# therealadityashankar/hey-buddy

Measured on AMD Instinct MI355X. Metric: audio clips/sec featurized+trained, 1.5 s @16 kHz, 1/2/4/8 GPU, higher is better.
Workload: dtype f32

## Files before the change

### hey-buddy_amd/csrc/hbk_augment_plan.h

```cpp
#pragma once

#include <algorithm>
#include <cmath>
#include <cstdarg>
#include <cstdint>
#include <cstdio>
#include <numeric>
#include <string>
#include <vector>

namespace hbk {
namespace {

constexpr int kPlanOk = 0, kPlanErrArg = -1, kPlanErrUnsupported = -3;

inline std::string strf(const char* fmt, ...) {
  char buf[512];
  va_list ap;
  va_start(ap, fmt);
  vsnprintf(buf, sizeof(buf), fmt, ap);
  va_end(ap);
  return buf;
}

inline int arg_fail(std::string& err, const char* what) {
  err = strf("hbk: invalid argument: %s", what);
  return kPlanErrArg;
}

inline int64_t up256(int64_t b) { return (b + 255) & ~int64_t(255); }

constexpr int kT = 23040;
constexpr int kM = kT / 2;
constexpr int kThreads = 1024;
constexpr int kN1 = 16000;
constexpr int kM1 = kN1 / 2;

constexpr int kTwLo = 128, kTwHi = kM / kTwLo;
static_assert(kTwLo * kTwHi == kM, "twiddle split");
constexpr int kTw8Lo = 100, kTw8Hi = kM1 / kTw8Lo;
static_assert(kTw8Lo * kTw8Hi == kM1, "twiddle split");

constexpr int kHRow = kM / 16 + 1;
constexpr int kHSlots = 16 * kHRow;

constexpr int kBsHalf = kT / 2;
constexpr int kBsPart = kT - kBsHalf + 1;
constexpr int kBsCirc = 512;
static_assert(2 * kBsCirc <= kThreads, "one edge sample per thread");

constexpr size_t kAugLds = (size_t(2 * kM + 32) * sizeof(float)) + (kTwHi + kTwLo) * 8;
constexpr size_t kBandStopLds = kAugLds + (5 * kBsCirc + 1) * sizeof(float);
constexpr size_t kColoredLds = (size_t(2 * kM1 + 32) * sizeof(float)) + (kTw8Hi + kTw8Lo) * 8;

constexpr int kPsFft = 250, kPsHop = 7, kPsBins = kPsFft / 2 + 1, kPsPad = kPsFft / 2;
constexpr int kPsTapMax = 144;
constexpr int kPsPhaseMax = 128;
constexpr int kPsResFrames = 32;
#ifndef HBK_PV_CLIPS
#define HBK_PV_CLIPS 2
#endif
constexpr int kPvClips = HBK_PV_CLIPS;
constexpr int kPvGroup = 8;
constexpr int kPvRows = 64;
constexpr int kPvGh = 64;
constexpr int kRsFrames = 64, kRsK = 160, kRsLd = kRsK + 8;
static_assert(kPsTapMax <= kRsK && kPsPhaseMax <= 128, "the MFMA resampler's K padding and 8 phase tiles");

struct PitchGeometry {
  int L = 0, f_in = 0, f_out = 0, l1 = 0, orig = 0, nw = 0, width = 0, target = 0;
  double rate = 0;
};

inline int pitch_geometry(int64_t L, int32_t sample_rate, int32_t num, int32_t den, PitchGeometry& a,
                          std::string& err) {
  if (sample_rate != 16000) {
    err = strf("hbk: pitch shift supports 16 kHz (n_fft 250, hop 7), got %d", sample_rate);
    return kPlanErrUnsupported;
  }
  if (num <= 0 || den <= 0) return arg_fail(err, "shift num / den must be positive");
  if (L <= kPsPad || L > (int64_t(1) << 24)) return arg_fail(err, "clip length must be in (125, 2^24]");
  a.L = static_cast<int>(L);
  a.rate = double(den) / double(num);
  a.f_in = 1 + a.L / kPsHop;
  a.f_out = static_cast<int>(std::ceil(double(a.f_in) / a.rate));
  a.l1 = kPsHop * (a.f_out - 1);
  const int64_t new_sr = int64_t(sample_rate) * den / num;
  const int64_t g = std::gcd(int64_t(sample_rate), new_sr);
  if (new_sr <= 0 || g <= 0) return arg_fail(err, "shift out of range");
  a.orig = static_cast<int>(sample_rate / g);
  a.nw = static_cast<int>(new_sr / g);
  a.width = static_cast<int>(std::ceil(6.0 * a.orig / (std::min(a.orig, a.nw) * 0.99)));
  a.target = static_cast<int>(std::ceil(double(a.nw) * a.l1 / a.orig));
  if (a.nw > kPsPhaseMax || 2 * a.width + a.orig > kPsTapMax || a.l1 <= 0 ||
      a.rate * kPvGroup + 3 > kPvRows) {
    err = strf("hbk: pitch shift %d/%d resamples %d -> %d (%d taps): the kernel holds <= %d phases of <= %d taps "
               "(torch_pitch_shift's fast shifts at 16 kHz)", num, den, a.orig, a.nw, 2 * a.width + a.orig,
               kPsPhaseMax, kPsTapMax);
    return kPlanErrUnsupported;
  }
  return kPlanOk;
}

struct PitchLayout {
  int64_t y = 0;
  int64_t taps = 0;
  int64_t yr = 0;
  int64_t sp = 0;
  int64_t key = 0;
  int64_t ord = 0;
  int64_t gord = 0;
  int64_t total = 0;
};

inline PitchLayout pitch_layout(const PitchGeometry& a, int64_t n) {
  PitchLayout w;
  w.y = 0;
  w.taps = up256(n * a.l1 * 4);
  w.yr = w.taps + up256(int64_t(kPsPhaseMax) * kPsTapMax * 4);
  w.sp = w.yr + up256(n * 8);
  w.key = w.sp + up256(n * 8);
  w.ord = w.key + up256(n * 8);
  w.gord = w.ord + up256(n * 4);
  w.total = w.gord + up256(n * 4);
  return w;
}

struct PitchKnobs {
  bool span = true;
  bool pair = true;
  bool resample_valu = false;
};

struct Grid {
  unsigned x = 1, y = 1, block = 0;
};

struct PitchLaunches {
  bool pair = false;
  int groups = 0;
  Grid taps, span, rank_clips, group, rank_groups, vocoder, resample;
  bool resample_mfma = true;
};

inline PitchLaunches pitch_launches(const PitchGeometry& a, int64_t n, const PitchKnobs& k) {
  PitchLaunches p;
  p.pair = k.span && k.pair;
  p.groups = static_cast<int>((n + kPvClips - 1) / kPvClips);
  p.taps = Grid{unsigned((a.nw * kPsTapMax + 255) / 256), 1, 256};
  p.span = Grid{unsigned((n + 3) / 4), 1, 256};
  p.rank_clips = Grid{unsigned((n + 63) / 64), 1, 1024};
  p.group = Grid{unsigned((p.groups + 255) / 256), 1, 256};
  p.rank_groups = Grid{unsigned((p.groups + 63) / 64), 1, 1024};
  p.vocoder = Grid{unsigned(p.groups), 1, unsigned(128 * kPvClips)};
  const int res_frames = (a.L + a.nw - 1) / a.nw;
  p.resample_mfma = !(k.resample_valu || a.nw > 128);
  p.resample = p.resample_mfma ? Grid{unsigned((res_frames + kRsFrames - 1) / kRsFrames), unsigned(n), 256}
                               : Grid{unsigned((res_frames + kPsResFrames - 1) / kPsResFrames), unsigned(n), 128};
  return p;
}

struct BandStopLayout {
  int64_t sums = 0;
  int64_t taps = 0;
  int64_t spectra = 0;
  int64_t scratch = 0;
  int64_t total = 0;
};

inline BandStopLayout band_stop_layout(int64_t n, int32_t n_filters, int32_t n_spectra, int64_t blocks) {
  BandStopLayout w;
  if (n <= 0) return w;
  w.taps = w.sums + up256(int64_t(n_filters) * 8);
  w.spectra = w.taps + up256(int64_t(n_filters) * (kBsCirc + 1) * 4);
  w.scratch = w.spectra + int64_t(n_spectra) * kHSlots * 8;
  w.total = w.scratch + blocks * kT * 4;
  return w;
}

struct ColoredLayout {
  int64_t groups = 0;
  int64_t gbuf = 0;
  int64_t grms = 0;
  int64_t total = 0;
};

inline ColoredLayout colored_layout(int64_t n_clips, int64_t clips_per_noise) {
  ColoredLayout w;
  w.groups = clips_per_noise > 1 && n_clips > 0 ? (n_clips + clips_per_noise - 1) / clips_per_noise : 0;
  if (!w.groups) return w;
  w.grms = w.groups * kN1 * int64_t(sizeof(float));
  w.total = w.grms + up256(w.groups * int64_t(sizeof(float)));
  return w;
}

enum ReverbTable { kTabHi, kTabLo, kTabN, kTabHi8, kTabLo8, kTabN16, kTabCount };

struct ReverbTables {
  std::vector<float> host;
  size_t off[kTabCount] = {};
  size_t pairs[kTabCount] = {};
  size_t bytes() const { return host.size() * sizeof(float); }
};

inline void twiddle_table(float* dst, int count, int step, int N, bool slotted) {
  for (int i = 0; i < count; ++i) {
    const double a = -2.0 * M_PI * (double(i) * step) / double(N);
    float* p = dst + 2 * size_t(slotted ? (i % 16) * kHRow + i / 16 : i);
    p[0] = float(cos(a));
    p[1] = float(sin(a));
  }
}

inline ReverbTables reverb_tables() {
  struct Spec {
    int count, step, N, pairs;
    bool slotted;
  };
  const Spec spec[kTabCount] = {
      {kTwHi, kTwLo, kM, kTwHi, false},        {kTwLo, 1, kM, kTwLo, false},      {kM + 1, 1, kT, kHSlots, true},
      {kTw8Hi, kTw8Lo, kM1, kTw8Hi, false},    {kTw8Lo, 1, kM1, kTw8Lo, false},   {kM1 / 2 + 1, 1, kN1, kM1 / 2 + 1, false},
  };
  ReverbTables t;
  size_t bytes = 0;
  for (int i = 0; i < kTabCount; ++i) {
    t.off[i] = bytes;
    t.pairs[i] = size_t(spec[i].pairs);
    bytes += size_t(up256(int64_t(spec[i].pairs) * 8));
  }
  t.host.assign(bytes / sizeof(float), 0.f);
  for (int i = 0; i < kTabCount; ++i)
    twiddle_table(t.host.data() + t.off[i] / sizeof(float), spec[i].count, spec[i].step, spec[i].N, spec[i].slotted);
  return t;
}

}
}
```

### hey-buddy_amd/csrc/hbk_clip_ops.hip

```cpp
#include <algorithm>

#include "hbk_aug_dev.h"

namespace hbk {
namespace {

struct TanhArgs {
  const float* x;
  int64_t x_stride;
  float* out;
  int64_t out_stride;
  int64_t n_clips;
  const float* amount;
  const int32_t* idx;
  int64_t n_entries;
  SrcView view;
};

__device__ __forceinline__ unsigned abs_bits(float v, int s) {
  return s < kT ? (__builtin_bit_cast(unsigned, v) & 0x7FFFFFFFu) : 0xFFFFFFFFu;
}

__global__ void __launch_bounds__(kThreads) __attribute__((amdgpu_waves_per_eu(8)))
tanh_distortion_kernel(TanhArgs a) {
  __shared__ unsigned hist[4096];
  __shared__ float red[32];
  __shared__ unsigned pick[2];
  constexpr int kPer = (kT + kThreads - 1) / kThreads;
  const int64_t n_iter = a.idx ? a.n_entries : a.n_clips;
  for (int64_t e = blockIdx.x; e < n_iter; e += gridDim.x) {
    const int64_t clip = a.idx ? a.idx[e] : e;
    const int tid = opaque_tid();
    const float* x = a.x + clip * a.x_stride;
    float* out = a.out + clip * a.out_stride;
    const float amt = a.amount[clip];
    if (amt != amt) {
      if (out != x) copy_clip(x, out, tid);
      continue;
    }
    float xr[kPer];
    const int pre = a.view.pre ? a.view.pre[clip] : -1, len = a.view.pre ? a.view.len[clip] : 0;
    if (pre >= 0) {
      const int n = min(len, kT);
      const float* row = n > 0 ? a.view.src + clip * a.view.stride : x;
      const int t = opaque_tid();
      const int w0 = __builtin_amdgcn_readfirstlane(t & ~63);
#pragma unroll
      for (int u = 0; u < kPer; ++u) xr[u] = load_placed_wave(row, pre, n, w0 + u * kThreads, t & 63);
    } else {
    const int t = opaque_tid();
#pragma unroll
    for (int u = 0; u < kPer; ++u) {
      const int s = t + u * kThreads;
      xr[u] = s < kT ? *reinterpret_cast<const float*>(reinterpret_cast<const char*>(x) + (static_cast<uint32_t>(s) << 2))
                     : 0.f;
    }
    }
    const double pos = (100.0 - 99.0 * static_cast<double>(amt)) / 100.0 * (kT - 1);
    const int lo = min(max(static_cast<int>(floor(pos)), 0), kT - 1);
    const double frac = pos - lo;
    unsigned prefix = 0, mask = 0, rank = static_cast<unsigned>(lo);
#pragma unroll 1
    for (int p = 0; p < 3; ++p) {
      const int shift = p == 0 ? 19 : (p == 1 ? 9 : 0), bins = p == 0 ? 4096 : (p == 1 ? 1024 : 512);
      const int per_lane = bins >> 6;
      for (int i = tid; i < bins; i += kThreads) hist[i] = 0;
      __syncthreads();
      const int t = opaque_tid();
#pragma unroll
      for (int u = 0; u < kPer; ++u) {
        const unsigned b = abs_bits(xr[u], t + u * kThreads);
        if ((b & mask) == prefix && b != 0xFFFFFFFFu) atomicAdd(&hist[(b >> shift) & (bins - 1)], 1u);
      }
      __syncthreads();
      if (tid < 64) {
        unsigned own = 0;
        for (int i = 0; i < per_lane; ++i) own += hist[per_lane * tid + i];
        unsigned inc = own;
#pragma unroll
        for (int d = 1; d < 64; d <<= 1) {
          const unsigned v = __shfl_up(inc, d, 64);
          if (tid >= d) inc += v;
        }
        const unsigned long long hit = __ballot(inc > rank);
        const int l = __ffsll(static_cast<long long>(hit)) - 1;
        if (tid == l) {
          unsigned r = rank - (inc - own), dsel = per_lane * l;
          for (int i = 0; i < per_lane - 1; ++i) {
            const unsigned h = hist[dsel];
            if (r < h) break;
            r -= h;
            ++dsel;
          }
          pick[0] = dsel;
          pick[1] = r;
        }
      }
      __syncthreads();
      prefix |= pick[0] << shift;
      mask |= static_cast<unsigned>(bins - 1) << shift;
      rank = pick[1];
    }
    float cnt = 0.f, mg = __builtin_inff();
    const int t2 = opaque_tid();
#pragma unroll
    for (int u = 0; u < kPer; ++u) {
      const unsigned b = abs_bits(xr[u], t2 + u * kThreads);
      if (b == 0xFFFFFFFFu) continue;
      if (b <= prefix) cnt += 1.f;
      else mg = fminf(mg, __builtin_bit_cast(float, b));
    }
    cnt = block_sum(cnt, red);
    {
      for (int d = 32; d >= 1; d >>= 1) mg = fminf(mg, __shfl_xor(mg, d, 64));
      __syncthreads();
      if ((tid & 63) == 0) red[tid >> 6] = mg;
      __syncthreads();
      mg = red[0];
      for (int w = 1; w < kThreads / 64; ++w) mg = fminf(mg, red[w]);
    }
    const double v_lo = __builtin_bit_cast(float, prefix);
    const double v_hi = (cnt >= lo + 2 || lo + 1 >= kT) ? v_lo : static_cast<double>(mg);
    const double d = v_hi - v_lo;
    const double th = frac >= 0.5 ? v_hi - d * (1.0 - frac) : v_lo + d * frac;
    const float g = static_cast<float>(0.5 / (th + 1e-6));
    float ex = 0.f, ey = 0.f;
#pragma unroll
    for (int u = 0; u < kPer; ++u) {
      ex += xr[u] * xr[u];
      xr[u] = 1.f - __fdividef(2.f, __expf(2.f * g * xr[u]) + 1.f);
      ey += xr[u] * xr[u];
    }
    block_sum2(ex, ey, red);
    const float rms_x = sqrtf(ex / kT);
    const float post = rms_x > 1e-9f ? rms_x / sqrtf(ey / kT) : 1.f;
    const int t3 = opaque_tid();
#pragma unroll
    for (int u = 0; u < kPer; ++u) {
      const int s = t3 + u * kThreads;
      if (s < kT) *reinterpret_cast<float*>(reinterpret_cast<char*>(out) + (static_cast<uint32_t>(s) << 2)) = xr[u] * post;
    }
    __syncthreads();
  }
}

constexpr int kPlaceSpan = 4096;
__global__ void __launch_bounds__(256) place_kernel(const float* __restrict__ src, int64_t src_stride,
                                                    const int32_t* __restrict__ src_len,
                                                    const int32_t* __restrict__ pre,
                                                    const int32_t* __restrict__ idx, float* __restrict__ out,
                                                    int64_t out_stride, int64_t n_clips, int T) {
  const int spans = (T + kPlaceSpan - 1) / kPlaceSpan;
  const int64_t items = n_clips * spans;
  constexpr int kR = kPlaceSpan / 1024;
  for (int64_t it = blockIdx.x; it < items; it += gridDim.x) {
    const int64_t e = it / spans;
    const int sp = static_cast<int>(it - e * spans);
    const int64_t clip = idx ? idx[e] : e;
    const int p = pre[clip];
    const int n = min(src_len[clip], T);
    const int last = max(n - 1, 0);
    const float* s = src + clip * src_stride;
    float* o = out + clip * out_stride;
    const int t0 = sp * kPlaceSpan + 4 * static_cast<int>(threadIdx.x);
    float v[kR][4];
#pragma unroll
    for (int r = 0; r < kR; ++r)
#pragma unroll
      for (int q = 0; q < 4; ++q) {
        const int u = t0 + r * 1024 + q - p;
        const float x = n > 0 ? s[min(max(u, 0), last)] : 0.f;
        v[r][q] = (u >= 0 && u < n) ? x : 0.f;
      }
#pragma unroll
    for (int r = 0; r < kR; ++r) {
      const int t = t0 + r * 1024;
      if (t < T) *reinterpret_cast<float4*>(o + t) = make_float4(v[r][0], v[r][1], v[r][2], v[r][3]);
    }
  }
}

constexpr int kEqTile = 64;
struct EqArgs {
  const float* x;
  int64_t x_stride;
  const double* coef;
  const int32_t* idx;
  float* out;
  int64_t out_stride;
  int64_t n;
  SrcView view;
};

constexpr int kEqClips = 8;
__global__ void __launch_bounds__(64) eq_kernel(EqArgs a) {
  constexpr int kRow = kEqTile + 4;
  __shared__ __attribute__((aligned(16))) float tin[kEqClips][kRow];
  __shared__ __attribute__((aligned(16))) float tout[kEqClips][kRow];
  const int lane = threadIdx.x, c = lane >> 3, sec = lane & 7;
  const int64_t j0 = static_cast<int64_t>(blockIdx.x) * kEqClips;
  const int64_t jc = min(j0 + c, a.n - 1);
  const double* cf0 = a.coef + jc * 35;
  const bool copy = cf0[0] != cf0[0];
  const int k = min(sec, 6);
  double b0 = cf0[5 * k], b1 = cf0[5 * k + 1], b2 = cf0[5 * k + 2], a1 = cf0[5 * k + 3], a2 = cf0[5 * k + 4];
  if (copy) b0 = 1.0, b1 = b2 = a1 = a2 = 0.0;
  double s1 = 0.0, s2 = 0.0;
  const int lc = lane >> 3, lq = lane & 7;
  const int64_t jl = min(j0 + lc, a.n - 1);
  const int64_t clip_l = a.idx ? static_cast<int64_t>(a.idx[jl]) : jl;
  const float* xl = a.x + clip_l * a.x_stride;
  float* ol = a.out + clip_l * a.out_stride;
  const bool store_l = j0 + lc < a.n;
  const int pre_l = a.view.pre ? a.view.pre[clip_l] : -1, len_l = a.view.pre ? a.view.len[clip_l] : 0;
  const int n_l = pre_l >= 0 ? min(len_l, kT) : 0;
  const float* sl = n_l > 0 ? a.view.src + clip_l * a.view.stride : xl;
  float4 p0, p1;
  auto load_tile = [&](int t) {
    const int u0 = t + 4 * lq - pre_l;
    if (pre_l >= 0 && u0 >= 0 && u0 + 35 < n_l) {
      const float* q = sl + u0;
      p0 = float4{q[0], q[1], q[2], q[3]};
      p1 = float4{q[32], q[33], q[34], q[35]};
    } else if (pre_l >= 0 && (u0 + 35 < 0 || u0 >= n_l)) {
      p0 = p1 = float4{0.f, 0.f, 0.f, 0.f};
    } else if (pre_l >= 0) {
      const int ta = t + 4 * lq, tb = ta + 32;
      p0 = float4{load_placed(sl, pre_l, n_l, ta), load_placed(sl, pre_l, n_l, ta + 1),
                  load_placed(sl, pre_l, n_l, ta + 2), load_placed(sl, pre_l, n_l, ta + 3)};
      p1 = float4{load_placed(sl, pre_l, n_l, tb), load_placed(sl, pre_l, n_l, tb + 1),
                  load_placed(sl, pre_l, n_l, tb + 2), load_placed(sl, pre_l, n_l, tb + 3)};
    } else {
      p0 = *reinterpret_cast<const float4*>(xl + t + 4 * lq);
      p1 = *reinterpret_cast<const float4*>(xl + t + 32 + 4 * lq);
    }
  };
  load_tile(0);
  float prev = 0.f;
  for (int t0 = 0; t0 <= kT; t0 += kEqTile) {
    tin[lc][4 * lq] = p0.x;
    tin[lc][4 * lq + 1] = p0.y;
    tin[lc][4 * lq + 2] = p0.z;
    tin[lc][4 * lq + 3] = p0.w;
    tin[lc][32 + 4 * lq] = p1.x;
    tin[lc][32 + 4 * lq + 1] = p1.y;
    tin[lc][32 + 4 * lq + 2] = p1.z;
    tin[lc][32 + 4 * lq + 3] = p1.w;
    __syncthreads();
    const int tn = min(t0 + kEqTile, kT - kEqTile);
    load_tile(tn);
    for (int st0 = 0; st0 < kEqTile; st0 += 8) {
      const float4 ia = *reinterpret_cast<const float4*>(&tin[c][st0]);
      const float4 ib = *reinterpret_cast<const float4*>(&tin[c][st0 + 4]);
      const float in8[8] = {ia.x, ia.y, ia.z, ia.w, ib.x, ib.y, ib.z, ib.w};
      float o8[8];
#pragma unroll
      for (int q = 0; q < 8; ++q) {
        const float u = sec == 0 ? in8[q] : prev;
        const double vd = u;
        const double y = fma(b0, vd, s1);
        s1 = fma(b1, vd, fma(-a1, y, s2));
        s2 = fma(b2, vd, -a2 * y);
        const float v = static_cast<float>(y);
        o8[q] = v;
        prev = __builtin_bit_cast(float, __builtin_amdgcn_update_dpp(__builtin_bit_cast(int, prev),
                                                                     __builtin_bit_cast(int, v), 0x111, 0xF, 0xF,
                                                                     false));
      }
      if (sec == 6) {
        *reinterpret_cast<float4*>(&tout[c][st0]) = float4{o8[0], o8[1], o8[2], o8[3]};
        *reinterpret_cast<float4*>(&tout[c][st0 + 4]) = float4{o8[4], o8[5], o8[6], o8[7]};
      }
    }
    __syncthreads();
    if (store_l) {
#pragma unroll
      for (int m = 0; m < 8; ++m) {
        const int kk = lq + 8 * m;
        const int n = t0 - 6 + kk;
        if (n >= 0 && n < kT) ol[n] = tout[lc][kk];
      }
    }
    __syncthreads();
  }
}

}
}

extern "C" {

int hbk_place_clips_idx(const float* src, int64_t n_clips, int64_t src_stride, const int32_t* src_len,
                        const int32_t* pre, const int32_t* idx, int64_t n_entries, float* out, int64_t out_stride,
                        int64_t T, void* stream) {
  using namespace hbk;
  if (n_clips < 0 || (idx && n_entries < 0)) return arg_error("negative count");
  const int64_t n_rows = idx ? n_entries : n_clips;
  if (n_rows == 0) return HBK_OK;
  if (!src || !src_len || !pre || !out) return arg_error("NULL pointer");
  if (T <= 0 || T % 4 || T > (int64_t(1) << 30)) return arg_error("T must be a positive multiple of 4");
  if (out_stride < T || out_stride % 4 || (reinterpret_cast<uintptr_t>(out) & 15))
    return arg_error("out rows must be 16-B aligned with stride >= T");
  const int64_t items = n_rows * ((T + kPlaceSpan - 1) / kPlaceSpan);
  if (items >= (int64_t(1) << 31)) return arg_error("too many clips for one launch");
  const int64_t blocks = items;
  hipLaunchKernelGGL(place_kernel, dim3(unsigned(blocks)), dim3(256), 0, as_stream(stream), src, src_stride, src_len,
                     pre, idx, out, out_stride, n_rows, int(T));
  HBK_LAUNCH_CHECK("place_kernel");
  return HBK_OK;
}

int hbk_place_clips(const float* src, int64_t n_clips, int64_t src_stride, const int32_t* src_len,
                    const int32_t* pre, float* out, int64_t out_stride, int64_t T, void* stream) {
  return hbk_place_clips_idx(src, n_clips, src_stride, src_len, pre, nullptr, 0, out, out_stride, T, stream);
}

int hbk_tanh_distortion_src(const float* x, int64_t n_clips, int64_t x_stride, const float* amount,
                            const int32_t* idx, int64_t n_entries, float* out, int64_t out_stride,
                            const float* src, int64_t src_stride, const int32_t* src_len, const int32_t* src_pre,
                            void* stream) {
  using namespace hbk;
  if (n_clips < 0) return arg_error("negative n_clips");
  if (n_clips == 0) return HBK_OK;
  if (!x || !out || !amount) return arg_error("NULL pointer");
  if (x_stride < kT || out_stride < kT) return arg_error("stride < 23040");
  TanhArgs a;
  a.x = x;
  a.x_stride = x_stride;
  a.out = out;
  a.out_stride = out_stride;
  a.n_clips = n_clips;
  a.amount = amount;
  a.idx = idx;
  a.n_entries = idx ? n_entries : n_clips;
  const int st = src_view(src, src_stride, src_len, src_pre, a.view);
  if (st != HBK_OK) return st;
  if (a.n_entries <= 0) return n_entries < 0 ? arg_error("negative n_entries") : HBK_OK;
  const int64_t blocks = std::min<int64_t>(a.n_entries, persistent_blocks(2, stream));
  hipLaunchKernelGGL(tanh_distortion_kernel, dim3(unsigned(blocks)), dim3(kThreads), 0, as_stream(stream), a);
  HBK_LAUNCH_CHECK("tanh_distortion_kernel");
  return HBK_OK;
}

int hbk_tanh_distortion(const float* x, int64_t n_clips, int64_t x_stride, const float* amount,
                        const int32_t* idx, int64_t n_entries, float* out, int64_t out_stride, void* stream) {
  return hbk_tanh_distortion_src(x, n_clips, x_stride, amount, idx, n_entries, out, out_stride, nullptr, 0, nullptr,
                                 nullptr, stream);
}

int hbk_seven_band_eq_src(const float* x, int64_t n_clips, int64_t x_stride, const double* coef, const int32_t* idx,
                          int64_t n_entries, float* out, int64_t out_stride, const float* src, int64_t src_stride,
                          const int32_t* src_len, const int32_t* src_pre, void* stream) {
  using namespace hbk;
  if (n_clips < 0 || n_entries < 0) return arg_error("negative count");
  if (!idx) n_entries = n_clips;
  if (n_entries == 0) return HBK_OK;
  if (!x || !out || !coef) return arg_error("NULL pointer");
  if (x_stride < kT || out_stride < kT) return arg_error("stride < 23040");
  if ((reinterpret_cast<uintptr_t>(x) | reinterpret_cast<uintptr_t>(out)) % 16 || x_stride % 4 || out_stride % 4)
    return arg_error("x / out rows must be 16-B aligned");
  EqArgs a;
  a.x = x;
  a.x_stride = x_stride;
  a.coef = coef;
  a.idx = idx;
  a.out = out;
  a.out_stride = out_stride;
  a.n = n_entries;
  const int st = src_view(src, src_stride, src_len, src_pre, a.view);
  if (st != HBK_OK) return st;
  hipLaunchKernelGGL(eq_kernel, dim3(unsigned((n_entries + kEqClips - 1) / kEqClips)), dim3(64), 0,
                     as_stream(stream), a);
  HBK_LAUNCH_CHECK("eq_kernel");
  return HBK_OK;
}

int hbk_seven_band_eq(const float* x, int64_t n_clips, int64_t x_stride, const double* coef, const int32_t* idx,
                      int64_t n_entries, float* out, int64_t out_stride, void* stream) {
  return hbk_seven_band_eq_src(x, n_clips, x_stride, coef, idx, n_entries, out, out_stride, nullptr, 0, nullptr,
                               nullptr, stream);
}

}
```

### hey-buddy_amd/csrc/hbk_mlp_fused.hip

```cpp
#include <hip/hip_runtime.h>

#include <algorithm>
#include <initializer_list>
#include <utility>
#include <cmath>
#include <cstdio>

#include "hbk_common.h"
#include "hbk_mlp_dev.h"
#include "hbk_mlp_gate.h"
#include "hbk_mlp_internal.h"
#include "hbk_mlp_plan.h"

namespace hbk {
namespace {

constexpr int kStats = 8;

#ifdef HBK_TRACE
constexpr int kTraceKerns = 6, kTraceWaves = 4;
static_assert(kTraceWaves * 64 >= 256, "every traced kernel runs <= 256 threads (4 waves)");
__device__ unsigned long long g_mlp_trace[kTraceKerns][kTraceWaves][128];
__device__ int g_mlp_trace_n[kTraceKerns][kTraceWaves];
#define HBK_MTB(kern, id, blk)                                                                       \
  do {                                                                                         \
    static_assert((kern) >= 0 && (kern) < kTraceKerns, "trace kernel slot out of range");     \
    if (blockIdx.x == (blk) && (threadIdx.x & 63) == 0 && (threadIdx.x >> 6) < kTraceWaves) {   \
      const int w_ = threadIdx.x >> 6;                                                          \
      const int n_ = g_mlp_trace_n[kern][w_];                                                   \
      if (n_ < 128) {                                                                           \
        g_mlp_trace[kern][w_][n_] = (static_cast<unsigned long long>(id) << 56) |               \
                                    (__builtin_amdgcn_s_memtime() & 0xFFFFFFFFFFFFFFull);       \
        g_mlp_trace_n[kern][w_] = n_ + 1;                                                       \
      }                                                                                         \
    }                                                                                           \
  } while (0)
#define HBK_MT(kern, id) HBK_MTB(kern, id, 0)
__device__ unsigned long long g_span[1024][3];
#define HBK_SPAN(slot, v)                                                               \
  do {                                                                                  \
    if (threadIdx.x == 0 && blockIdx.x < 1024) g_span[blockIdx.x][slot] = (v);           \
  } while (0)
#else
#define HBK_SPAN(slot, v) \
  do {                    \
  } while (0)
#define HBK_MT(kern, id) \
  do {                   \
  } while (0)
#define HBK_MTB(kern, id, blk) \
  do {                         \
  } while (0)
#endif

#ifdef HBK_BOUNDS
constexpr int kBMax = 16;
__device__ unsigned long long g_brange[kBMax][2];
__device__ int g_bn;
__device__ unsigned long long g_berr[4];
__device__ __attribute__((aligned(16))) char g_bsafe[1 << 16];
template <typename T>
__device__ __forceinline__ T* bck_(T* p, int nbytes, int line) {
  const unsigned long long c = reinterpret_cast<unsigned long long>(p);
  bool ok = false;
  for (int i = 0; i < kBMax; ++i) ok |= i < g_bn && c >= g_brange[i][0] && c + nbytes <= g_brange[i][1];
  if (ok) return p;
  if (atomicCAS(&g_berr[0], 0ull, static_cast<unsigned long long>(line)) == 0ull) {
    g_berr[1] = blockIdx.x;
    g_berr[2] = threadIdx.x;
    g_berr[3] = c;
  }
  return reinterpret_cast<T*>(g_bsafe);
}
#define BCK(p, n) bck_((p), (n), __LINE__)
#else
#define BCK(p, n) (p)
#endif

__device__ __forceinline__ int step_of(const float* state, int parity) {
  return state ? static_cast<int>(state[parity * 8 + 3]) : 0;
}

struct GateWords {
  const float* st;
  const float* stats;
};
struct GateSeen {
  float acc_samples, n_sel;
};
__device__ __forceinline__ GateSeen gate_load(const GateWords& g) {
  GateSeen s{0.f, kGateSamples};
  if (g.st) {
    s.acc_samples = *BCK(&g.st[0], 4);
    s.n_sel = *BCK(&g.stats[0], 4);
  }
  return s;
}
__device__ __forceinline__ bool gate_drops(const GateSeen& s) {
  return step_gate(s.acc_samples, 1.f, 0.f, s.n_sel).fire == 0.f;
}

struct K1aArgs {
  const float* pool32;
  const _Float16* pool16;
  int64_t n32, n16;
  const int32_t* idx;
  int64_t idx_stride;
  int64_t idx_steps;
  const float* state;
  int parity;
  int B;
  float drop_p;
  uint64_t seed;
  float* xhat[2];
  int64_t Bp;
  uint4* rinfo[2];
  uint32_t* mask[2];
};

struct K1bArgs {
  const float* P;
  int64_t g_in, b_in, w0;
  int B;
  const float* xhat;
  int64_t Bp;
  float* hg_part;
  float* stats;
};

constexpr int kSlabLd = 516;
template <bool kIdx, bool kV2 = false>
__device__ __forceinline__ void k1a_tile(const K1aArgs& a, int rt, int step, float* __restrict__ xout,
                                         float* slab, int dpar = 0) {
  const int tid = threadIdx.x, lane = tid & 63, wave = tid >> 6;
  const uint64_t seed = a.seed + static_cast<uint64_t>(step) +
                        (a.state ? static_cast<uint64_t>(a.state[a.parity * 8 + 4]) << 24 : 0);
  const uint32_t s0 = static_cast<uint32_t>(seed), s1 = static_cast<uint32_t>(seed >> 32) * 0x27D4EB2Fu;
  const char* fallback = a.pool32 ? reinterpret_cast<const char*>(a.pool32) : reinterpret_cast<const char*>(a.pool16);
  int ixs[4];
#pragma unroll
  for (int i = 0; i < 4; ++i) {
    ixs[i] = min(rt * kR + wave * 4 + i, a.B - 1);
    if (kIdx) ixs[i] = *BCK(&a.idx[static_cast<int64_t>(step) * a.idx_stride + ixs[i]], 4);
  }
  uint4 raw[4][6];
  bool is16[4], ok[4];
  const char* rowptr[4];
#pragma unroll
  for (int i = 0; i < 4; ++i) {
    const int r = rt * kR + wave * 4 + i;
    const int ix = __builtin_amdgcn_readfirstlane(ixs[i]);
    is16[i] = ix < 0;
    const int64_t row16 = -static_cast<int64_t>(ix) - 1;
    ok[i] = r < a.B && (is16[i] ? row16 < a.n16 : ix < a.n32);
    const char* bp = !ok[i] ? fallback
                     : is16[i] ? reinterpret_cast<const char*>(a.pool16 + row16 * kD)
                               : reinterpret_cast<const char*>(a.pool32 + static_cast<int64_t>(ix) * kD);
    rowptr[i] = bp;
#pragma unroll
    for (int u = 0; u < 6; ++u) {
      const int slot = is16[i] ? u % 3 : u;
      raw[i][u] = *BCK(reinterpret_cast<const uint4*>(bp + 16 * (lane + 64 * slot)), 16);
    }
  }
  const float keep = a.drop_p > 0.f ? 1.f / (1.f - a.drop_p) : 1.f;
  const uint32_t thr = static_cast<uint32_t>(a.drop_p * 65536.f + 0.5f);
  float xh[4][kV2 ? 1 : 24];
  unsigned char* mimg = reinterpret_cast<unsigned char*>(slab) + (wave * 4) * kD;
#pragma unroll
  for (int i = 0; i < 4; ++i) {
    const int r = rt * kR + wave * 4 + i;
    float v[24];
    int c[24];
    bool dr[24];
#pragma unroll
    for (int j = 0; j < 24; ++j) {
      const uint4 w16 = raw[i][j >> 3];
      const uint32_t word16 = (&w16.x)[(j & 7) >> 1];
      const _Float16 h = __builtin_bit_cast(_Float16, static_cast<uint16_t>((j & 1) ? word16 >> 16 : word16));
      const uint4 w32 = raw[i][j >> 2];
      const float f = __builtin_bit_cast(float, (&w32.x)[j & 3]);
      v[j] = ok[i] ? (is16[i] ? static_cast<float>(h) : f) : 0.f;
      c[j] = is16[i] ? 8 * (lane + 64 * (j >> 3)) + (j & 7) : 4 * (lane + 64 * (j >> 2)) + (j & 3);
      dr[j] = !ok[i];
    }
    if (a.drop_p > 0.f) {
      const uint32_t base = static_cast<uint32_t>(r) * (kD / 2);
#pragma unroll
      for (int j = 0; j < 24; j += 2) {
        const uint32_t hsh = drop_hash(s0, s1, base + (c[j] >> 1));
        const bool d0 = (hsh & 0xFFFFu) < thr, d1 = (hsh >> 16) < thr;
        v[j] = d0 ? 0.f : v[j] * keep;
        v[j + 1] = d1 ? 0.f : v[j + 1] * keep;
        dr[j] = dr[j] || d0;
        dr[j + 1] = dr[j + 1] || d1;
      }
    }
    float sm = 0.f;
#pragma unroll
    for (int j = 0; j < 24; ++j) sm += v[j];
    const float mu = wsum(sm) * (1.f / kD);
    float sq = 0.f;
#pragma unroll
    for (int j = 0; j < 24; ++j) sq += (v[j] - mu) * (v[j] - mu);
// ... 287 lines not shown
    acc[t] = f4{0.f, 0.f, 0.f, 0.f};
    if (t < RT) {
#pragma unroll
      for (int i = 0; i < kNI; ++i) {
        const h8 ah = *reinterpret_cast<const h8*>(&ahS[(16 * t + m) * kLdA + 32 * i + 8 * kq]);
        const h8 al = *reinterpret_cast<const h8*>(&alS[(16 * t + m) * kLdA + 32 * i + 8 * kq]);
        acc[t] = mma3(ah, al, whi[i], wlo[i], acc[t]);
      }
    }
  }
  float* out = a.hg_part + static_cast<int64_t>(ks) * a.B * kH2 + 16 * wave + m;
#pragma unroll
  for (int t = 0; t < kRTM; ++t)
    if (t < RT) {
#pragma unroll
      for (int e = 0; e < 4; ++e) {
        const int r = r0 + 16 * t + 4 * kq + e;
        if (r < a.B) *BCK(&out[static_cast<int64_t>(r) * kH2], 4) = acc[t][e] * (1.f / 16.f);
      }
    }
  HBK_MT(3, 3);
}

__device__ __forceinline__ void wsplit_store4(const WSplit& w, _Float16* __restrict__ base, int64_t i4, f4 p) {
#pragma unroll
  for (int sg = 0; sg < kMaxSeg; ++sg) {
    if (sg >= w.n) break;
    const WSeg g = w.s[sg];
    const int64_t rc = int64_t(g.rows) * g.cols, off = i4 - g.src;
    if (off < 0 || off >= rc) continue;
    uint32_t h[2], l[2];
    split_pair(16.f * p[0], 16.f * p[1], h[0], l[0]);
    split_pair(16.f * p[2], 16.f * p[3], h[1], l[1]);
    _Float16* d = base + g.dst;
    *reinterpret_cast<uint2*>(d + off) = uint2{h[0], h[1]};
    *reinterpret_cast<uint2*>(d + rc + off) = uint2{l[0], l[1]};
    const int r = static_cast<int>(off / g.cols), c = static_cast<int>(off - int64_t(r) * g.cols);
#pragma unroll
    for (int e = 0; e < 4; ++e) {
      const uint32_t he = (e & 1) ? h[e >> 1] >> 16 : h[e >> 1] & 0xFFFFu;
      const uint32_t le = (e & 1) ? l[e >> 1] >> 16 : l[e >> 1] & 0xFFFFu;
      d[2 * rc + int64_t(c + e) * g.rows + r] = __builtin_bit_cast(_Float16, static_cast<uint16_t>(he));
      d[3 * rc + int64_t(c + e) * g.rows + r] = __builtin_bit_cast(_Float16, static_cast<uint16_t>(le));
    }
  }
}
__global__ void __launch_bounds__(256) k0_wsplit_kernel(WSplit w, const float* __restrict__ P,
                                                         _Float16* __restrict__ base, int64_t n4) {
  for (int64_t q = blockIdx.x * int64_t(256) + threadIdx.x; q < n4; q += int64_t(gridDim.x) * 256) {
    int sg = 0;
#pragma unroll
    for (int t = 1; t < kMaxSeg; ++t)
      if (t < w.n && q >= w.s[t].q0) sg = t;
    const int64_t i4 = w.s[sg].src + 4 * (q - w.s[sg].q0);
    wsplit_store4(w, base, i4, *reinterpret_cast<const f4*>(P + i4));
  }
}

struct K2Args {
  const float* P;
  int B, NG, KS;
  int64_t w_hg[kMaxG], b_hg[kMaxG], w_o[kMaxG], b_o[kMaxG];
  int64_t ln_g[kMaxG], ln_b[kMaxG];
  const float* hg_part;
  const float* y;
  int64_t y_stride;
  const float* state;
  int parity;
  const float* sched;
  int sched_len;
  float neg_weight, thr, act_thr;
  float* prob;
  float* logit;
  float* G;
  float* stats;
  int64_t Bp;
  float* U;
  float* Xn;
  float* dS;
  float* dHG;
  int n_rt, prefetch;
  K1aArgs pre;
  const _Float16* wc;
  int64_t c_o[kMaxG], c_hg[kMaxG], c_oT[kMaxG], c_hgT[kMaxG];
  float* counts;
  int count_label;
  int v2;
  float* maxS;
  int pre_tiles;
};

#ifdef HBK_TRACE
#define K2_MARK(id)                                                                \
  do {                                                                             \
    if (blockIdx.x == 0 && lane == 0 && wave < kTraceWaves && trn < 48)            \
      trS[wave][trn++] = (static_cast<unsigned long long>(id) << 56) |             \
                         (__builtin_amdgcn_s_memtime() & 0xFFFFFFFFFFFFFFull);     \
  } while (0)
#else
#define K2_MARK(id) \
  do {              \
  } while (0)
#endif

#ifndef HBK_K2_ABLATE
#define HBK_K2_ABLATE 0
#endif
template <bool kTrain, int NG>
__global__ void __launch_bounds__(64 * kK2Waves) k2_rows_kernel(K2Args a) {
  constexpr int kHgF = NG * kR * kLd > kR * kSlabLd ? NG * kR * kLd : kR * kSlabLd;
  __shared__ __attribute__((aligned(16))) float hgRaw[kHgF];
  float (*hgS)[kR][kLd] = reinterpret_cast<float (*)[kR][kLd]>(hgRaw);
  __shared__ __attribute__((aligned(16))) float xhS[NG - 1][kR][kL + 4];
  __shared__ __attribute__((aligned(16))) float bX[kR][kLd];
  __shared__ __attribute__((aligned(16))) float bU[kR][kLd];
  __shared__ __attribute__((aligned(16))) float bS[kR][kLd];
  __shared__ float rsS[NG][kR];
  __shared__ float zS[kR], dzS[kR];
  __shared__ float red[kStats];
  __shared__ float sBhg[NG][kH2], sWo[kH];
#ifdef HBK_TRACE
  __shared__ unsigned long long trS[4][48];
  int trn = 0;
#endif
  if (kTrain && static_cast<int>(blockIdx.x) >= a.n_rt) {
    const int step = step_of(a.pre.state, a.pre.parity) + 1;
    if (step < a.pre.idx_steps) {
      if (a.v2) {
        for (int t = 0; t < a.pre_tiles; ++t) {
          const int rt = (blockIdx.x - a.n_rt) * a.pre_tiles + t;
          if (rt >= a.n_rt) break;
          if (t) __syncthreads();
          k1a_tile<true, true>(a.pre, rt, step, nullptr, hgRaw, a.pre.parity ^ 1);
        }
      } else {
        for (int t = 0; t < kPreTiles; ++t) {
          const int rt = (blockIdx.x - a.n_rt) * kPreTiles + t;
          if (rt >= a.n_rt) break;
          if (t) __syncthreads();
          k1a_tile<true>(a.pre, rt, step, a.pre.xhat[a.pre.parity ^ 1], hgRaw);
        }
      }
    }
    return;
  }
  const int tid = threadIdx.x, lane = tid & 63, wave = tid >> 6;
  const int m = lane & 15, kq = lane >> 4;
  const int r0 = blockIdx.x * kR;
  const int nrow = min(kR, a.B - r0);
  const float* P = a.P;
  const int64_t B = a.B;
  const int64_t Bp = a.Bp;
  K2_MARK(1);
  const int step = step_of(a.state, a.parity);
  float y_pre = 0.f, nw_pre = a.neg_weight;
  if (kTrain) {
    y_pre = *BCK(&a.y[static_cast<int64_t>(step) * a.y_stride + min(r0 + (tid & 15), a.B - 1)], 4);
    if (a.sched) nw_pre = *BCK(&a.sched[2 * min(step, a.sched_len - 1) + 1], 4);
  }
  WFrag<kH, 2> wa;
  WFrag<kL, 2> wb;
  load_wf<kH, kL, 2>(wa, a.wc + a.c_o[0], wave, lane);
  const int lc0 = 6 * (lane & 15);
  float bo0[NG], bo1[NG], lg[NG][6], lb[NG][6];
  {
    const int c2 = tid & (kH2 - 1);
    float vbhg[NG];
#pragma unroll
    for (int k = 0; k < NG; ++k) {
      vbhg[k] = P[a.b_hg[k] + c2];
      bo0[k] = P[a.b_o[k] + (k + 1 < NG ? 16 * wave + m : 0)];
      bo1[k] = P[a.b_o[k] + (k + 1 < NG ? min(16 * (wave + 4) + m, kL - 1) : 0)];
#pragma unroll
      for (int e = 0; e < 6; ++e) {
        lg[k][e] = k + 1 < NG ? P[a.ln_g[k] + lc0 + e] : 0.f;
        lb[k][e] = k + 1 < NG ? P[a.ln_b[k] + lc0 + e] : 0.f;
      }
    }
    const float vwo = P[a.w_o[NG - 1] + (tid & (kH - 1))];
#pragma unroll
    for (int k = 0; k < NG; ++k)
      if (tid < kH2) sBhg[k][tid] = vbhg[k];
    if (tid < kH) sWo[tid] = vwo;
  }
  {
    float h[4] = {0.f, 0.f, 0.f, 0.f}, g[4] = {0.f, 0.f, 0.f, 0.f};
    auto sum_slabs = [&](auto U_) {
      constexpr int U = decltype(U_)::value;
      for (int s0 = 0; s0 < a.KS; s0 += U) {
        float lh[U][4], lg[U][4];
#pragma unroll
        for (int u = 0; u < U; ++u) {
          const int sl = (HBK_K2_ABLATE & 2) ? 0 : min(s0 + u, a.KS - 1);
#pragma unroll
          for (int q = 0; q < 4; ++q) {
            const int e = tid + 256 * q, r = min(e >> 6, nrow - 1), j = e & 63;
            const float* src = a.hg_part + (sl * B + r0 + r) * kH2;
            lh[u][q] = *BCK(&src[j], 4);
            lg[u][q] = *BCK(&src[kH + j], 4);
          }
        }
#pragma unroll
        for (int u = 0; u < U; ++u) {
          const float on = s0 + u < a.KS ? 1.f : 0.f;
#pragma unroll
          for (int q = 0; q < 4; ++q) {
            h[q] += on * lh[u][q];
            g[q] += on * lg[u][q];
          }
        }
      }
    };
    if (a.KS % 12 == 0)
      sum_slabs(std::integral_constant<int, 12>{});
    else
      sum_slabs(std::integral_constant<int, 8>{});
    const float bh = P[a.b_hg[0] + (tid & 63)], bg = P[a.b_hg[0] + kH + (tid & 63)];
#pragma unroll
    for (int q = 0; q < 4; ++q) {
      const int e = tid + 256 * q, r = e >> 6, j = e & 63;
      const float hh = h[q] + bh, gg = g[q] + bg;
      hgS[0][r][j] = hh;
      hgS[0][r][kH + j] = gg;
      bU[r][j] = hh * sigm_fast(hh) * gg;
    }
  }
  __syncthreads();
  K2_MARK(2);
  auto st4 = [&](float* base, int col, int row4, f4 v) {
#pragma unroll
    for (int e = 0; e < 4; ++e)
      if (r0 + row4 + e >= a.B) v[e] = 0.f;
    *BCK(reinterpret_cast<f4*>(base + col * Bp + r0 + row4), 16) = v;
  };
  auto amax4 = [&](f4 v, int row4) {
    float x = 0.f;
#pragma unroll
    for (int e = 0; e < 4; ++e) x = fmaxf(x, r0 + row4 + e < a.B ? fabsf(v[e]) : 0.f);
    return x;
  };
  auto store_t = [&](float* base, const float* src, int ncols) {
    float mx = 0.f;
    for (int e = tid; e < 4 * ncols; e += 256) {
      const int col = e >> 2, r4 = 4 * (e & 3);
      const f4 v = f4{src[r4 * kLd + col], src[(r4 + 1) * kLd + col], src[(r4 + 2) * kLd + col],
                      src[(r4 + 3) * kLd + col]};
      mx = fmaxf(mx, amax4(v, r4));
      st4(base, col, r4, v);
    }
    return mx;
  };
  auto pub_max = [&](int mat, float mx) {
    if (a.maxS) {
      mx = wmax(mx);
      if (lane == 0) *BCK(&a.maxS[(static_cast<int64_t>(mat) * a.n_rt + blockIdx.x) * kK2Waves + wave], 4) = mx;
    }
  };
  if (kTrain) {
    const int j = tid & 63, rg = 4 * (tid >> 6);
    st4(a.U, j, rg, f4{bU[rg][j], bU[rg + 1][j], bU[rg + 2][j], bU[rg + 3][j]});
  }
#pragma unroll
  for (int k = 0; k + 1 < NG; ++k) {
    if (!(HBK_K2_ABLATE & 1) || k == 0) load_wf<kL, kH2, 2>(wb, a.wc + a.c_hg[k + 1], wave, lane);
    {
      f4 c0, c1;
      gemm2<kH>(wa, load_a<kH>(&bU[0][0], lane), c0, c1);
      const int n0 = 16 * wave + m, n1 = 16 * (wave + 4) + m;
      const float bo0_ = bo0[k], bo1_ = bo1[k];
#pragma unroll
      for (int e = 0; e < 4; ++e) bS[4 * kq + e][n0] = c0[e] + bo0_;
      if (n1 < kL) {
#pragma unroll
        for (int e = 0; e < 4; ++e) bS[4 * kq + e][n1] = c1[e] + bo1_;
      }
    }
    __syncthreads();
    K2_MARK(10 + k);
    if (!(HBK_K2_ABLATE & 1) && k + 2 < NG) load_wf<kH, kL, 2>(wa, a.wc + a.c_o[k + 1], wave, lane);
    {
      const int r = wave * 4 + (lane >> 4), c0 = 6 * (lane & 15);
      float v[6];
#pragma unroll
      for (int e = 0; e < 6; ++e) v[e] = bS[r][c0 + e];
      const float mu = rsum16(((v[0] + v[1]) + (v[2] + v[3])) + (v[4] + v[5])) * (1.f / kL);
      float sq = 0.f;
#pragma unroll
      for (int e = 0; e < 6; ++e) sq += (v[e] - mu) * (v[e] - mu);
      const float rs = __builtin_amdgcn_rsqf(rsum16(sq) * (1.f / kL) + kLnEps);
#pragma unroll
      for (int e = 0; e < 6; ++e) {
        const float x = (v[e] - mu) * rs;
        xhS[k][r][c0 + e] = x;
        bX[r][c0 + e] = x * lg[k][e] + lb[k][e];
      }
      if ((lane & 15) == 0) rsS[k][r] = rs;
    }
    __syncthreads();
    K2_MARK(20 + k);
    if (kTrain) store_t(a.Xn + (k + 1) * kL * Bp, &bX[0][0], kL);
    {
      f4 ch, cg;
      gemm2<kL>(wb, load_a<kL>(&bX[0][0], lane), ch, cg);
      const int j = 16 * wave + m;
      const float bh = sBhg[k + 1][j], bg = sBhg[k + 1][kH + j];
      f4 uo;
#pragma unroll
      for (int e = 0; e < 4; ++e) {
        const int r = 4 * kq + e;
        const float h = ch[e] + bh, g = cg[e] + bg;
        hgS[k + 1][r][j] = h;
        hgS[k + 1][r][kH + j] = g;
        const float u = h * sigm_fast(h) * g;
        bU[r][j] = u;
        uo[e] = u;
      }
      if (kTrain) st4(a.U + (k + 1) * kH * Bp, j, 4 * kq, uo);
    }
    __syncthreads();
    K2_MARK(30 + k);
  }
  WFrag<kH2, 2> fx;
  WFrag<kL, 1> fy;
  if (kTrain) {
    load_wf<kH2, kL, 2>(fx, a.wc + a.c_hgT[NG - 1], wave, lane);
    load_wf<kL, kH, 1>(fy, a.wc + a.c_oT[NG - 2], wave, lane);
  }
  {
    const float bo = bo0[NG - 1];
    const float wl = sWo[lane];
#pragma unroll
    for (int i = 0; i < 4; ++i) {
      const int r = wave * 4 + i;
      const float z = wsum(bU[r][lane] * wl) + bo;
      if (lane == 0) zS[r] = z;
    }
  }
  __syncthreads();
  K2_MARK(40);
  if (tid < kR) {
    const int r = tid;
    float loc[kStats] = {0.f, 0.f, 0.f, 0.f, 0.f, 0.f, 0.f, 0.f};
    float dz = 0.f;
    if (r < nrow) {
      const float z = zS[r], p = sigm(z);
      if (a.prob) *BCK(&a.prob[r0 + r], 4) = p;
      if (a.logit) *BCK(&a.logit[r0 + r], 4) = z;
      if (kTrain) {
        const float nw = nw_pre;
        const float yy = y_pre;
        const bool pos = yy == 1.f;
        const bool sel = pos ? (p < 1.f - a.thr) : (p >= a.thr);
        if (sel) {
          const float w = pos ? 1.f : nw;
          const float lp = fmaxf(logf(p), -100.f), l1p = fmaxf(logf(1.f - p), -100.f);
          loc[0] = 1.f;
          loc[1] = -w * (yy * lp + (1.f - yy) * l1p);
          dz = w * (p - yy) / fmaxf((1.f - p) * p, 1e-12f) * ((1.f - p) * p);
          if (pos) {
            loc[4] = 1.f;
            loc[5] = p > a.act_thr ? 1.f : 0.f;
          } else {
            loc[2] = 1.f;
            loc[3] = (yy - p <= -a.act_thr) ? 1.f : 0.f;
          }
        }
        loc[6] = 1.f;
      }
    }
    dzS[r] = dz;
    if (!kTrain && a.counts) {
      float pge = 0.f, pgt = 0.f;
      if (r < nrow) {
        const float p = sigm(zS[r]);
        pge = p >= a.act_thr ? 1.f : 0.f;
        pgt = p > a.act_thr ? 1.f : 0.f;
      }
      pge = rsum16(pge);
      pgt = rsum16(pgt);
      if (tid == 0) {
        if (pge != 0.f) atomicAdd(BCK(a.counts + 2 * a.count_label, 4), pge);
        if (pgt != 0.f) atomicAdd(BCK(a.counts + 2 * a.count_label + 1, 4), pgt);
      }
    }
    if (kTrain) {
#pragma unroll
      for (int s = 0; s < kStats; ++s) {
        const float v = rsum16(loc[s]);
        if (tid == 0) red[s] = v;
      }
    }
  }
  if constexpr (!kTrain) return;
  __syncthreads();
  K2_MARK(41);
  if (tid < kStats && red[tid] != 0.f) atomicAdd(BCK(a.stats + tid, 4), red[tid]);
  if (!HBK_K2_ABLATE && red[0] == 0.f) {
    const f4 z4 = {0.f, 0.f, 0.f, 0.f};
#pragma unroll
    for (int k = 0; k < NG; ++k) {
      for (int e = tid; e < 4 * kH2; e += 256) st4(a.dHG + k * kH2 * Bp, e >> 2, 4 * (e & 3), z4);
      if (k + 1 < NG) {
        for (int e = tid; e < 4 * kL; e += 256) st4(a.dS + k * kL * Bp, e >> 2, 4 * (e & 3), z4);
      } else if (tid < 4) {
        st4(a.dS + k * kL * Bp, 0, 4 * tid, z4);
      }
    }
    if (a.maxS && lane == 0) {
#pragma unroll
      for (int mat = 0; mat < 2 * NG; ++mat)
        *BCK(&a.maxS[(static_cast<int64_t>(mat) * a.n_rt + blockIdx.x) * kK2Waves + wave], 4) = 0.f;
    }
    return;
  }
  float* G = a.G;
  {
    const f4 dz4 = f4{dzS[4 * (tid & 3)], dzS[4 * (tid & 3) + 1], dzS[4 * (tid & 3) + 2], dzS[4 * (tid & 3) + 3]};
    if (tid < 4) st4(a.dS + (NG - 1) * kL * Bp, 0, 4 * tid, dz4);
    pub_max(2 * NG - 1, tid < 4 ? amax4(dz4, 4 * tid) : 0.f);
  }
  if (tid == 64) {
    float s = 0.f;
    for (int r = 0; r < kR; ++r) s += dzS[r];
    if (s != 0.f) atomicAdd(BCK(G + a.b_o[NG - 1], 4), s);
  }
  {
    const int k = NG - 1;
    const int j = tid & 63, rg = 4 * (tid >> 6);
    const float wj = sWo[j];
    f4 dho, dgo;
#pragma unroll
    for (int e = 0; e < 4; ++e) {
      const int r = rg + e;
      const float h = hgS[k][r][j], gg = hgS[k][r][kH + j], du = dzS[r] * wj;
      const float sg = sigm_fast(h);
      const float dh = du * gg * (sg * (1.f + h * (1.f - sg))), dg = du * h * sg;
      bX[r][j] = dh;
      bX[r][kH + j] = dg;
      dho[e] = dh;
      dgo[e] = dg;
    }
    st4(a.dHG + k * kH2 * Bp, j, rg, dho);
    st4(a.dHG + k * kH2 * Bp, kH + j, rg, dgo);
    pub_max(k, fmaxf(amax4(dho, rg), amax4(dgo, rg)));
  }
  __syncthreads();
  K2_MARK(42);
#pragma unroll
  for (int k = NG - 1; k >= 1; --k) {
    if (tid < kH2) {
      float s = 0.f;
      for (int r = 0; r < kR; ++r) s += bX[r][tid];
      atomicAdd(BCK(G + a.b_hg[k] + tid, 4), s);
    }
    {
      f4 c0, c1;
      gemm2<kH2>(fx, load_a<kH2>(&bX[0][0], lane), c0, c1);
      if (!(HBK_K2_ABLATE & 1) && k - 1 >= 1) load_wf<kH2, kL, 2>(fx, a.wc + a.c_hgT[k - 1], wave, lane);
      const int n0 = 16 * wave + m, n1 = 16 * (wave + 4) + m;
#pragma unroll
      for (int e = 0; e < 4; ++e) bU[4 * kq + e][n0] = c0[e];
      if (n1 < kL) {
#pragma unroll
        for (int e = 0; e < 4; ++e) bU[4 * kq + e][n1] = c1[e];
      }
    }
    __syncthreads();
    K2_MARK(50 + k);
    {
      const int l = k - 1;
      if (tid < kL) {
        float sg = 0.f, sb = 0.f;
        for (int r = 0; r < kR; ++r) {
          sg += bU[r][tid] * xhS[l][r][tid];
          sb += bU[r][tid];
        }
        atomicAdd(BCK(G + a.ln_g[l] + tid, 4), sg);
        atomicAdd(BCK(G + a.ln_b[l] + tid, 4), sb);
      }
      const int r = wave * 4 + (lane >> 4), c0 = 6 * (lane & 15);
      float t[6], x[6];
      float p1 = 0.f, p2 = 0.f;
#pragma unroll
      for (int e = 0; e < 6; ++e) {
        t[e] = bU[r][c0 + e] * lg[l][e];
        x[e] = xhS[l][r][c0 + e];
        p1 += t[e];
        p2 += t[e] * x[e];
      }
      const float s1 = rsum16(p1) * (1.f / kL), s2 = rsum16(p2) * (1.f / kL);
      const float rs = rsS[l][r];
#pragma unroll
      for (int e = 0; e < 6; ++e) bS[r][c0 + e] = rs * (t[e] - s1 - x[e] * s2);
    }
    __syncthreads();
    K2_MARK(60 + k);
    {
      const int kk = k - 1;
      pub_max(NG + kk, store_t(a.dS + kk * kL * Bp, &bS[0][0], kL));
      if (tid < kL) {
        float s = 0.f;
        for (int r = 0; r < kR; ++r) s += bS[r][tid];
        atomicAdd(BCK(G + a.b_o[kk] + tid, 4), s);
      }
      const f4 du = gemm1<kL>(fy, load_a<kL>(&bS[0][0], lane));
      if (!(HBK_K2_ABLATE & 1) && k - 2 >= 0) load_wf<kL, kH, 1>(fy, a.wc + a.c_oT[k - 2], wave, lane);
      const int j = 16 * wave + m;
      f4 dho, dgo;
#pragma unroll
      for (int e = 0; e < 4; ++e) {
        const int r = 4 * kq + e;
        const float h = hgS[kk][r][j], gg = hgS[kk][r][kH + j];
        const float sg = sigm_fast(h);
        const float dh = du[e] * gg * (sg * (1.f + h * (1.f - sg))), dg = du[e] * h * sg;
        bX[r][j] = dh;
        bX[r][kH + j] = dg;
        dho[e] = dh;
        dgo[e] = dg;
      }
      st4(a.dHG + kk * kH2 * Bp, j, 4 * kq, dho);
      st4(a.dHG + kk * kH2 * Bp, kH + j, 4 * kq, dgo);
      pub_max(kk, fmaxf(amax4(dho, 4 * kq), amax4(dgo, 4 * kq)));
    }
    __syncthreads();
    K2_MARK(70 + k);
  }
  if (tid < kH2) {
    float s = 0.f;
    for (int r = 0; r < kR; ++r) s += bX[r][tid];
    atomicAdd(BCK(G + a.b_hg[0] + tid, 4), s);
  }
  K2_MARK(99);
#ifdef HBK_TRACE
  if (blockIdx.x == 0 && lane == 0 && wave < kTraceWaves) {
    for (int i = 0; i < trn; ++i) g_mlp_trace[1][wave][i] = trS[wave][i];
    g_mlp_trace_n[1][wave] = trn;
  }
#endif
}

struct WJob {
  const float* X;
  const float* Y;
  int64_t c_off;
  int ldc, M, N, tn;
};
constexpr int kMaxRng = 2 + 2 * kMaxG;
struct Ranges {
// ... 1250 lines not shown
  HBK_LAUNCH_CHECK("k0_wsplit_kernel");
  return HBK_OK;
}

int mlp_fused_run(const hbk_mlp_plan& p, const float* params, const float* pool32, int64_t n32,
                  const void* pool16, int64_t n16, const int32_t* idx, int64_t idx_stride, int64_t idx_steps,
                  const float* y, int64_t y_stride, int B, const float* state, int parity, const float* sched,
                  int sched_len, float neg_weight, float thr, float act_thr, float drop_p, uint64_t seed,
                  float* bucket, float* prob, float* logit, float* ws, bool train, int flags, hipStream_t s) {
  const StepKnobs kn = read_step_knobs();
  const int64_t cus = persistent_blocks(1, s);
  const StepPlan pl = plan_step(B, static_cast<int>(p.g.size()), p.n_params, cus, kn);
  const FusedWs& w = pl.ws;
#ifdef HBK_BOUNDS
  bounds_set({{params, p.n_params * 4},
              {pool32, n32 * kD * 4},
              {pool16, n16 * kD * 2},
              {idx, (std::max<int64_t>(idx_steps, 1) * idx_stride + B) * 4},
              {y, (std::max<int64_t>(idx_steps, 1) * y_stride + B) * 4},
              {state, 64},
              {sched, int64_t(sched_len) * 8},
              {bucket, (p.n_params + kStats) * 4},
              {prob, int64_t(B) * 4},
              {logit, int64_t(B) * 4},
              {ws, w.total * 4}});
#endif
  if (kn.plan_log && train && pl.variant == 2) {
    static int64_t logged = -1;
    if (logged != pl.Bp) {
      logged = pl.Bp;
      fprintf(stderr, "hbk k3s plan: Bp %lld, CUs %lld, S0 %d x %d steps, S1 %d x %d steps\n",
              static_cast<long long>(pl.Bp), static_cast<long long>(cus), pl.S0, kK3sPairs[pl.k3s_pair][0], pl.S1,
              kK3sPairs[pl.k3s_pair][1]);
    }
  }
  const float keep = drop_p > 0.f ? 1.f / (1.f - drop_p) : 1.f;
  if (kn.gate_skip == 0) flags &= ~HBK_STEP_GATE_SKIP;
  StepRun r{p, pl, params, pool32, static_cast<const _Float16*>(pool16), y, y_stride, B, state, parity, sched,
            sched_len, neg_weight, thr, act_thr, keep, bucket, prob, logit, ws, train, flags, s, K1aArgs{},
            kn.gate_skip};
  K1aArgs& ka = r.ka;
  ka.pool32 = pool32;
  ka.pool16 = r.pool16;
  ka.n32 = pool32 ? n32 : 0;
  ka.n16 = pool16 ? n16 : 0;
  ka.idx = idx;
  ka.idx_stride = idx_stride;
  ka.idx_steps = idx ? idx_steps : 0;
  ka.state = state;
  ka.parity = parity;
  ka.B = B;
  ka.drop_p = drop_p;
  ka.seed = seed;
  ka.Bp = pl.Bp;
  for (int i = 0; i < 2; ++i) {
    ka.xhat[i] = ws + w.xhat[i];
    ka.rinfo[i] = reinterpret_cast<uint4*>(ws + w.rinfo[i]);
    ka.mask[i] = reinterpret_cast<uint32_t*>(ws + w.mask[i]);
  }
  int rc = HBK_OK;
  if (!(flags & HBK_STEP_WEIGHTS_READY)) rc = mlp_wcache_fill(p, params, ws + w.wsplit, s);
  if (rc == HBK_OK && !(flags & HBK_STEP_XHAT_READY)) rc = launch_rows(r);
  if (rc == HBK_OK) rc = launch_input_gemm(r);
  if (rc == HBK_OK) rc = launch_k2(r);
  if (rc != HBK_OK || !train) return rc;
  rc = launch_wgrad(r);
  return rc == HBK_OK ? finish_partials(r) : rc;
}

int mlp_fused_update(const hbk_mlp_plan& p, float* params, float* bucket, float* m, float* v, float* state,
                     int parity, const float* sched, int sched_len, float lr, float b1, float b2, float eps,
                     float* hist, int hist_cap, float* ws, hipStream_t s) {
  if (p.deferred_ws && p.deferred_ws != ws) {
    set_error("hbk: the previous hbk_mlp_step_fwd_bwd deferred its weight-gradient partials to its workspace: "
              "pass that workspace to hbk_mlp_step_update");
    return HBK_ERR_ARG;
  }
  K4Args k;
  k.w = make_wsplit(p);
  const FusedFixed fl = fused_fixed(static_cast<int>(p.g.size()), p.n_params);
  k.wc = ws ? reinterpret_cast<_Float16*>(ws + fl.wsplit) : nullptr;
  k.part = p.deferred_ws ? ws + fl.part : nullptr;
  k.pstride = fl.pstride;
  k.ns = p.deferred_ws ? p.deferred_ks : 0;
  if (p.n_params >= (int64_t(1) << 31) - 4) {
    set_error("hbk: hbk_mlp_step_update: parameter count >= 2^31");
    return HBK_ERR_ARG;
  }
  const Ranges rg = make_ranges(p);
  k.n_cov = rg.n;
  for (int i = 0; i < kMaxRng; ++i) {
    k.cov_lo[i] = i < rg.n ? static_cast<int32_t>(rg.lo[i]) : 0;
    k.cov_hi[i] = i < rg.n ? static_cast<int32_t>(rg.hi[i]) : 0;
  }
  k.n_skip = k.w.n;
  for (int sg = 0; sg < kMaxSeg; ++sg) {
    const int64_t lo = sg < k.w.n ? k.w.s[sg].src : 0, hi = sg < k.w.n ? lo + int64_t(k.w.s[sg].rows) * k.w.s[sg].cols : 0;
    k.skip_lo[sg] = static_cast<int32_t>((lo + 3) / 4);
    k.skip_hi[sg] = static_cast<int32_t>((hi + 3) / 4);
  }
  const bool gate_first = p.deferred_ws && k.ns > 0 && p.deferred_gate == 1;
  p.deferred_ws = nullptr;
  p.deferred_gate = 0;
  k.n_tiles = 0;
  for (int sg = 0; sg < k.w.n; ++sg)
    for (int r0 = 0; r0 < k.w.s[sg].rows && k.n_tiles < kMaxTiles; r0 += kTileR) {
      k.tile_seg[k.n_tiles] = sg;
      k.tile_r0[k.n_tiles++] = r0;
    }
  k.P = params;
  k.G = bucket;
  k.m = m;
  k.v = v;
  k.n = p.n_params;
  k.state = state;
  k.parity = parity;
  k.sched = sched;
  k.sched_len = sched_len;
  k.lr = lr;
  k.b1 = b1;
  k.b2 = b2;
  k.eps = eps;
  k.hist = hist;
  k.hist_cap = hist_cap;
  const int64_t blocks = (k.wc ? k.n_tiles : 0) + std::min<int64_t>((p.n_params / 4 + 255) / 256, 1024);
  hipLaunchKernelGGL(gate_first ? k4_update_kernel<true> : k4_update_kernel<false>, dim3(unsigned(blocks)), dim3(256),
                     0, s, k);
  HBK_LAUNCH_CHECK("k4_update_kernel");
  return HBK_OK;
}

}

#ifdef HBK_BOUNDS
extern "C" int hbk_debug_bounds(unsigned long long* out) {
  if (hipDeviceSynchronize() != hipSuccess) return -1;
  if (hipMemcpyFromSymbol(out, HIP_SYMBOL(hbk::g_berr), 4 * sizeof(unsigned long long)) != hipSuccess) return -2;
  unsigned long long z[4] = {};
  (void)hipMemcpyToSymbol(HIP_SYMBOL(hbk::g_berr), z, sizeof(z));
  return 0;
}
#endif

#ifdef HBK_TRACE
extern "C" int hbk_debug_mlp_trace(unsigned long long* out, int* counts) {
  static_assert(sizeof(hbk::g_mlp_trace) == sizeof(unsigned long long) * 6 * 4 * 128, "probe_mlp.py's buffer");
  if (hipMemcpyFromSymbol(out, HIP_SYMBOL(hbk::g_mlp_trace), sizeof(hbk::g_mlp_trace)) != hipSuccess) return -2;
  if (hipMemcpyFromSymbol(counts, HIP_SYMBOL(hbk::g_mlp_trace_n), sizeof(hbk::g_mlp_trace_n)) != hipSuccess)
    return -2;
  int z[hbk::kTraceKerns * hbk::kTraceWaves] = {};
  (void)hipMemcpyToSymbol(HIP_SYMBOL(hbk::g_mlp_trace_n), z, sizeof(z));
  return 0;
}
extern "C" int hbk_debug_spans(unsigned long long* out) {
  return hipMemcpyFromSymbol(out, HIP_SYMBOL(hbk::g_span), sizeof(hbk::g_span)) == hipSuccess ? 0 : -2;
}
#endif
```

### hey-buddy_amd/csrc/hbk_pitch.hip

```cpp
#include <atomic>
#include <cstdlib>

#include "hbk_augment_plan.h"
#include "hbk_common.h"

namespace hbk {
namespace {

static_assert(kPsTapMax == HBK_PITCH_SHIFT_MAX_TAPS, "the resampler's tap rows");
static_assert(kPlanOk == HBK_OK && kPlanErrArg == HBK_ERR_ARG && kPlanErrUnsupported == HBK_ERR_UNSUPPORTED,
              "the planner's status values");
#ifndef HBK_PV_ABLATE
#define HBK_PV_ABLATE 0
#endif
#ifndef HBK_PV_F32STATE
#define HBK_PV_F32STATE 0
#endif
#ifndef HBK_PV_RESTART
#if HBK_PV_F32STATE
#define HBK_PV_RESTART 128
#else
#define HBK_PV_RESTART 1024
#endif
#endif
constexpr int kPvRestart = HBK_PV_RESTART;
#if HBK_PV_F32STATE
typedef float pv_t;
#else
typedef double pv_t;
#endif

struct PitchArgs {
  const float* x;
  int64_t x_stride;
  const int32_t* idx;
  int n;
  float* out;
  int64_t out_stride;
  int L, f_in, f_out, l1, orig, nw, width, target;
  double rate;
  float* y;
  float* taps;
  int2* yr;
  int span;
  int2* sp;
  uint64_t* key;
  int32_t* ord;
  int32_t* gord;
};

__device__ __forceinline__ int ps_i0(const PitchArgs& a, int t, float& alpha) {
  const float ts = static_cast<float>(static_cast<double>(t) * a.rate);
  const float fl = floorf(ts);
  alpha = ts - fl;
  return static_cast<int>(fl);
}

struct PvClip {
  float d[kPvRows][8];
  float xs[256];
  float gh[2][kPvGh][8];
  int cnt0;
  int lo, hi;
};
struct PvShared {
  cf tw[256];
  double tw64[256][2];
  float4 wt[3][128];
  PvClip c[kPvClips];
};

__device__ __forceinline__ int pv_g(int b) { return (b & 3) ^ ((b & 4) ? 7 : 0); }

template <int kCtrl>
__device__ __forceinline__ float pv_dpp(float v) {
  return __builtin_bit_cast(float, __builtin_amdgcn_update_dpp(0, __builtin_bit_cast(int, v), kCtrl, 0xF, 0xF, true));
}

template <bool kSwap16>
__device__ __forceinline__ float pv_swap_add(float x, float y) {
  if (kSwap16)
    asm volatile("s_nop 1\n\tv_permlane16_swap_b32 %0, %1\n\ts_nop 1" : "+v"(x), "+v"(y));
  else
    asm volatile("s_nop 1\n\tv_permlane32_swap_b32 %0, %1\n\ts_nop 1" : "+v"(x), "+v"(y));
  return x + y;
}

__device__ __forceinline__ cf pv_cmul(cf a, cf b) {
  cf t, r;
  asm("v_pk_mul_f32 %0, %1, %2 op_sel_hi:[0,1]" : "=v"(t) : "v"(a), "v"(b));
  asm("v_pk_fma_f32 %0, %1, %2, %3 op_sel:[1,1,0] op_sel_hi:[1,0,1] neg_lo:[0,1,0]" : "=v"(r) : "v"(a), "v"(b), "v"(t));
  return r;
}
__device__ __forceinline__ cf pv_cmul_conj(cf a, cf b) {
  cf t, r;
  asm("v_pk_mul_f32 %0, %1, %2 op_sel_hi:[0,1] neg_hi:[0,1]" : "=v"(t) : "v"(a), "v"(b));
  asm("v_pk_fma_f32 %0, %1, %2, %3 op_sel:[1,1,0] op_sel_hi:[1,0,1]" : "=v"(r) : "v"(a), "v"(b), "v"(t));
  return r;
}

typedef float pv_v4 __attribute__((ext_vector_type(4)));
typedef __attribute__((address_space(3))) const pv_v4 pv_lds_v4;
__device__ __forceinline__ float4 pv_f4(pv_v4 v) { return float4{v.x, v.y, v.z, v.w}; }

__device__ __forceinline__ cf pv_inc(float4 da, float4 db, float4 w12, float4 w34, float4 w56) {
  const cf dxy = {da.x, da.y}, dzw = {da.z, da.w}, exy = {db.x, db.y}, ez = {db.z, db.w};
  const cf w1 = {w12.x, w12.y}, w2 = {w12.z, w12.w}, w3 = {w34.x, w34.y}, w4 = {w34.z, w34.w};
  const cf w5 = {w56.x, w56.y}, w6 = {w56.z, w56.w};
  cf acc;
  asm("v_pk_mul_f32 %0, %1, %2 op_sel:[1,0] op_sel_hi:[1,1]" : "=v"(acc) : "v"(dxy), "v"(w1));
  asm("v_pk_fma_f32 %0, %1, %2, %0 op_sel:[0,0,0] op_sel_hi:[0,1,1]" : "+v"(acc) : "v"(dzw), "v"(w2));
  asm("v_pk_fma_f32 %0, %1, %2, %0 op_sel:[1,0,0] op_sel_hi:[1,1,1]" : "+v"(acc) : "v"(dzw), "v"(w3));
  asm("v_pk_fma_f32 %0, %1, %2, %0 op_sel:[0,0,0] op_sel_hi:[0,1,1]" : "+v"(acc) : "v"(exy), "v"(w4));
  asm("v_pk_fma_f32 %0, %1, %2, %0 op_sel:[1,0,0] op_sel_hi:[1,1,1]" : "+v"(acc) : "v"(exy), "v"(w5));
  asm("v_pk_fma_f32 %0, %1, %2, %0 op_sel:[0,0,0] op_sel_hi:[0,1,1]" : "+v"(acc) : "v"(ez), "v"(w6));
  return acc;
}

__device__ __forceinline__ float ps_xp(const float* xr, int L, int p) {
  int i = p - kPsPad;
  i = i < 0 ? -i : i;
  i = i >= L ? 2 * (L - 1) - i : i;
  return xr[i];
}

__device__ __forceinline__ void pv_load_rows(const PitchArgs& a, PvShared& sh, const float* xr, int cl, int lane,
                                             int fb) {
  for (int q = lane; q < 2 * kPvRows; q += 128) {
    const int row = q >> 1, h = q & 1, f = fb + row;
    float* dr = sh.c[cl].d[row];
    if (f >= a.f_in) {
      for (int j = 4 * h; j < 4 * h + 4; ++j) dr[j] = 0.f;
      continue;
    }
    if (h == 0) {
      for (int j = 0; j < 4; ++j) dr[j] = ps_xp(xr, a.L, 7 * f + 243 + j) - ps_xp(xr, a.L, 7 * f - 7 + j);
    } else {
      int delta = 0;
      for (int j = 0; j < 7; ++j) {
        const float vin = ps_xp(xr, a.L, 7 * f + 243 + j), vout = ps_xp(xr, a.L, 7 * f - 7 + j);
        delta += (vin != 0.f) - (vout != 0.f);
        if (j >= 4) dr[j] = vin - vout;
      }
      dr[7] = __builtin_bit_cast(float, delta);
    }
  }
}

__device__ __forceinline__ void pv_scan_span(PvClip& C, const float* xr, int L, int lane) {
  int lo = INT_MAX, hi = -1;
  int done = 0;
  if ((reinterpret_cast<uintptr_t>(xr) & 15) == 0) {
    const float4* x4 = reinterpret_cast<const float4*>(xr);
    const int n4 = L >> 2;
    for (int q0 = 0; q0 < n4; q0 += 128 * 8) {
      float4 v[8];
#pragma unroll
      for (int j = 0; j < 8; ++j) {
        const int q = q0 + 128 * j + lane;
        v[j] = q < n4 ? x4[q] : float4{0.f, 0.f, 0.f, 0.f};
      }
#pragma unroll
      for (int j = 0; j < 8; ++j) {
        const int p = 4 * (q0 + 128 * j + lane);
        const bool b0 = v[j].x != 0.f, b1 = v[j].y != 0.f, b2 = v[j].z != 0.f, b3 = v[j].w != 0.f;
        if (b0 || b1 || b2 || b3) {
          lo = min(lo, p + (b0 ? 0 : b1 ? 1 : b2 ? 2 : 3));
          hi = max(hi, p + (b3 ? 3 : b2 ? 2 : b1 ? 1 : 0));
        }
      }
    }
    done = 4 * n4;
  }
  for (int p = done + lane; p < L; p += 128) {
    if (xr[p] != 0.f) {
      lo = min(lo, p);
      hi = max(hi, p);
    }
  }
  if (hi >= 0) {
    atomicMin(&C.lo, lo);
    atomicMax(&C.hi, hi);
  }
}

__device__ __forceinline__ void pv_frames_of(const PitchArgs& a, int lo, int hi, int& tb, int& tl) {
  const int jmax = (a.l1 + kPsPad - 1) / kPsHop;
  tb = 0;
  tl = jmax;
  float al;
  if (lo > hi) {
    tl = -1;
    return;
  }
  if (lo > 2 * kPsPad && a.rate < 2.0) {
    const int fz = (lo - kPsPad) / kPsHop - 1;
    int tg = min(static_cast<int>((fz - 2) / a.rate), a.f_out - 1) & ~(kPvGroup - 1);
    while (tg > 0 && ps_i0(a, tg - 1, al) + 2 > fz) tg -= kPvGroup;
    tb = max(tg, 0);
  }
  if (hi < a.L - 1 - 2 * kPsPad) {
    const int fn = min((hi + kPsPad) / kPsHop, a.f_in - 1);
    int t = max(min(a.f_out - 1, static_cast<int>((fn + 1) / a.rate) + 1), 0);
    while (t > 0 && ps_i0(a, t, al) > fn) --t;
    while (t + 1 < a.f_out && ps_i0(a, t + 1, al) <= fn) ++t;
    tl = min(jmax, t + 36);
  }
}

constexpr int kPsQuant = 360;

__global__ void __launch_bounds__(256) ps_span_kernel(PitchArgs a) {
  const int lane = threadIdx.x & 63, e = blockIdx.x * 4 + (threadIdx.x >> 6);
  if (e >= a.n) return;
  const float* xr = a.x + static_cast<int64_t>(a.idx[e]) * a.x_stride;
  constexpr int kChunk = 64 * 8;
  int lo = INT_MAX, hi = -1;
  for (int p0 = 0; p0 < a.L; p0 += kChunk) {
    float v[8];
#pragma unroll
    for (int j = 0; j < 8; ++j) {
      const int p = p0 + 64 * j + lane;
      v[j] = p < a.L ? xr[p] : 0.f;
    }
#pragma unroll
    for (int j = 0; j < 8; ++j)
      if (v[j] != 0.f) {
        lo = min(lo, p0 + 64 * j + lane);
        hi = max(hi, p0 + 64 * j + lane);
      }
    if (__any(hi >= 0)) break;
  }
  for (int o = 32; o >= 1; o >>= 1) {
    lo = min(lo, __shfl_xor(lo, o, 64));
    hi = max(hi, __shfl_xor(hi, o, 64));
  }
  if (hi >= 0) {
    for (int p1 = a.L; p1 > hi + 1; p1 -= kChunk) {
      float v[8];
      int h = -1;
#pragma unroll
      for (int j = 0; j < 8; ++j) {
        const int p = p1 - kChunk + 64 * j + lane;
        v[j] = (p > hi && p < a.L) ? xr[max(p, 0)] : 0.f;
      }
#pragma unroll
      for (int j = 0; j < 8; ++j)
        if (v[j] != 0.f) h = max(h, p1 - kChunk + 64 * j + lane);
      if (__any(h >= 0)) {
        for (int o = 32; o >= 1; o >>= 1) h = max(h, __shfl_xor(h, o, 64));
        hi = h;
        break;
      }
    }
  }
  if (lane == 0) {
    a.sp[e] = int2{lo, hi};
    const uint64_t q = hi < 0 ? 0 : 1 + static_cast<uint64_t>(hi / kPsQuant), f = hi < 0 ? 0 : static_cast<uint64_t>(lo);
    a.key[e] = (q << 40) | (f << 16) | static_cast<uint64_t>(e);
  }
}

__global__ void __launch_bounds__(1024) ps_rank_kernel(const uint64_t* __restrict__ key, int n,
                                                       int32_t* __restrict__ ord) {
  __shared__ int part[16][64];
  const int lane = threadIdx.x & 63, w = threadIdx.x >> 6, i = blockIdx.x * 64 + lane;
  const uint64_t mine = key[min(i, n - 1)];
  const int per = (n + 15) / 16, j0 = min(w * per, n), j1 = min(j0 + per, n);
  int below = 0;
  for (int jb = j0; jb < j1; jb += 64) {
    const uint64_t kl = jb + lane < j1 ? key[jb + lane] : ~uint64_t(0);
#pragma unroll
    for (int q = 0; q < 64; ++q) {
      const uint32_t hi = __builtin_amdgcn_readlane(static_cast<int>(kl >> 32), q);
      const uint32_t lo = __builtin_amdgcn_readlane(static_cast<int>(kl), q);
      below += ((static_cast<uint64_t>(hi) << 32) | lo) < mine;
    }
  }
  part[w][lane] = below;
  __syncthreads();
  if (w == 0 && i < n) {
    int r = 0;
#pragma unroll
    for (int q = 0; q < 16; ++q) r += part[q][lane];
    ord[r] = i;
  }
}

__global__ void __launch_bounds__(256) ps_group_kernel(PitchArgs a, int groups) {
  const int g = blockIdx.x * 256 + threadIdx.x;
  if (g >= groups) return;
  int lo = INT_MAX, hi = -1;
  for (int c = 0; c < kPvClips; ++c) {
    const int2 s = a.sp[a.ord[min(kPvClips * g + c, a.n - 1)]];
    lo = min(lo, s.x);
    hi = max(hi, s.y);
  }
  int tb, tl;
  pv_frames_of(a, lo, hi, tb, tl);
  const int steps = tl < tb ? 0 : (tl - tb) / kPvGroup + 1;
  a.key[g] = (static_cast<uint64_t>((1 << 24) - steps) << 16) | static_cast<uint64_t>(g);
}

#ifdef HBK_PHASE_TIMING
__device__ unsigned long long g_pv_phase[5];
#define HBK_PVT(i)                                    \
  do {                                                 \
    const unsigned long long t_ = __builtin_amdgcn_s_memtime(); \
    pvt[i] += t_ - pvt_t0;                             \
    pvt_t0 = t_;                                       \
  } while (0)
#else
#define HBK_PVT(i) \
  do {             \
  } while (0)
#endif

#ifndef HBK_PV_UNROLL_TAIL
#define HBK_PV_UNROLL_TAIL 1
#endif
#ifndef HBK_PV_WAVES
#define HBK_PV_WAVES 4
#endif
__global__ void __launch_bounds__(128 * kPvClips) __attribute__((amdgpu_waves_per_eu(HBK_PV_WAVES)))
ps_vocoder_kernel(PitchArgs a) {
#ifdef HBK_PHASE_TIMING
  unsigned long long pvt[5] = {0, 0, 0, 0, 0}, pvt_t0 = __builtin_amdgcn_s_memtime();
#endif
  extern __shared__ __attribute__((aligned(16))) unsigned char pv_smem[];
  PvShared& sh = *reinterpret_cast<PvShared*>(pv_smem);
  const int tid = threadIdx.x, cl = tid >> 7, lane = tid & 127;
  const int slot = (a.sp ? a.gord[blockIdx.x] : static_cast<int>(blockIdx.x)) * kPvClips + cl;
  const int e = a.sp ? a.ord[min(slot, a.n - 1)] : min(slot, a.n - 1);
  const bool live = slot < a.n;
  const float* xr = a.x + static_cast<int64_t>(a.idx[e]) * a.x_stride;
  PvClip& C = sh.c[cl];
  for (int q = tid; q < 256; q += blockDim.x) {
    double sn, cs;
    sincospi(2.0 * q / kPsFft, &sn, &cs);
    sh.tw[q] = cf{static_cast<float>(cs), static_cast<float>(sn)};
    sh.tw64[q][0] = cs;
    sh.tw64[q][1] = -sn;
  }
  if (lane == 0) C.cnt0 = 0;
  if (lane == 0) {
    const int2 s = a.sp ? a.sp[e] : int2{INT_MAX, -1};
    C.lo = s.x;
    C.hi = s.y;
  }
  __syncthreads();
  if (a.span && !a.sp) pv_scan_span(C, xr, a.L, lane);
  int nz = 0;
  for (int q = lane; q < kPsFft; q += 128) {
    const float v = ps_xp(xr, a.L, q);
    C.xs[q] = v;
    nz += v != 0.f;
  }
  if (nz) atomicAdd(&C.cnt0, nz);
  for (int q = tid; q < 3 * 128; q += blockDim.x) {
    const int j = 2 * (q / 128) + 1, kk = min(q % 128, kPsBins - 1), q1 = (kk * j) % kPsFft,
              q2 = (kk * (j + 1)) % kPsFft;
    sh.wt[q / 128][q % 128] = float4{static_cast<float>(sh.tw64[q1][0]), static_cast<float>(sh.tw64[q1][1]),
                                     static_cast<float>(sh.tw64[q2][0]), static_cast<float>(sh.tw64[q2][1])};
  }
  int fb = 1;
  pv_load_rows(a, sh, xr, cl, lane, fb);
  __syncthreads();

  const int k = min(lane, kPsBins - 1);
  const int q7 = (7 * k) % kPsFft;
  const pv_t rr = static_cast<pv_t>(sh.tw64[q7][0]), ri = static_cast<pv_t>(-sh.tw64[q7][1]);
  const float ck = lane < kPsBins ? ((lane == 0 || lane == kPsBins - 1) ? 1.f : 2.f) : 0.f;
  const int gb = pv_g(lane & 7), w = lane >> 6, ou = (lane >> 3) & 7;
  cf esr[4], esi[4];
#pragma unroll
  for (int r = 0; r < 8; ++r) {
    const int sr = r ^ gb;
    const cf ev = sr < kPsHop ? ck * sh.tw[(k * sr) % kPsFft] : cf{0.f, 0.f};
    esr[r >> 1][r & 1] = ev.x;
    esi[r >> 1][r & 1] = -ev.y;
  }
  const bool b3 = lane & 8;
  auto direct = [&](double& re, double& im) {
    re = im = 0.0;
    int q = 0;
    for (int n = 0; n < kPsFft; ++n) {
      const double v = static_cast<double>(C.xs[n]);
      re = fma(v, sh.tw64[q][0], re);
      im = fma(v, sh.tw64[q][1], im);
      q += k;
      q -= q >= kPsFft ? kPsFft : 0;
    }
  };
  pv_t xre = pv_t(0), xim = pv_t(0);
  int cnt = __builtin_amdgcn_readfirstlane(C.cnt0);
  if (cnt != 0) {
    double dre, dim;
// ... 288 lines not shown
    v = static_cast<float>((t == 0.0 ? 1.0 : sin(t) / t) * c * c * (base / a.orig));
  }
  a.taps[i] = v;
}

__device__ __forceinline__ bool ps_window_silent(const PitchArgs& a, int2 yr, int e, int j0, int f0, int frames,
                                                 int tid, int threads) {
  if (j0 < yr.y && j0 + (frames - 1) * a.orig + kPsTapMax > yr.x) return false;
  float* out = a.out + static_cast<int64_t>(a.idx[e]) * a.out_stride;
  const int i1 = static_cast<int>(min(static_cast<int64_t>(f0 + frames) * a.nw, static_cast<int64_t>(a.L)));
  for (int i = f0 * a.nw + tid; i < i1; i += threads) out[i] = 0.f;
  return true;
}

__global__ void __launch_bounds__(128) ps_resample_kernel(PitchArgs a) {
  static_assert(kPsTapMax % 2 == 0 && kPsResFrames % 2 == 0, "resampler pairs");
  constexpr int kPairs = kPsResFrames / 2;
  __shared__ __attribute__((aligned(16))) float ys2[kPairs][2 * kPsTapMax];
  const int ph = threadIdx.x, e = blockIdx.y;
  const int f0 = blockIdx.x * kPsResFrames;
  const float* y = a.y + static_cast<int64_t>(e) * a.l1;
  const int j0 = f0 * a.orig - a.width;
  const int2 yr = a.yr[e];
  if (ps_window_silent(a, yr, e, j0, f0, kPsResFrames, ph, 128)) return;
  for (int el = ph; el < kPsResFrames * kPsTapMax; el += 128) {
    const int fr = el / kPsTapMax, q = el - fr * kPsTapMax;
    const int src = j0 + fr * a.orig + q;
    ys2[fr >> 1][2 * q + (fr & 1)] = (src >= yr.x && src < yr.y) ? y[src] : 0.f;
  }
  float tp[kPsTapMax];
  const float* tr = a.taps + min(ph, a.nw - 1) * kPsTapMax;
#pragma unroll
  for (int q = 0; q < kPsTapMax; ++q) tp[q] = tr[q];
  __syncthreads();
  if (ph >= a.nw) return;
  float* out = a.out + static_cast<int64_t>(a.idx[e]) * a.out_stride;
  for (int p = 0; p < kPairs; ++p) {
    const int i = (f0 + 2 * p) * a.nw + ph, i1 = i + a.nw;
    if (i >= a.L) break;
    cf v = {0.f, 0.f};
    if (i < a.target) {
      const float4* w = reinterpret_cast<const float4*>(ys2[p]);
#pragma unroll
      for (int q2 = 0; q2 < kPsTapMax / 2; ++q2) {
        const float4 ww = w[q2];
        v = __builtin_elementwise_fma(cf{tp[2 * q2], tp[2 * q2]}, cf{ww.x, ww.y}, v);
        v = __builtin_elementwise_fma(cf{tp[2 * q2 + 1], tp[2 * q2 + 1]}, cf{ww.z, ww.w}, v);
      }
    }
    out[i] = v.x;
    if (i1 < a.L) out[i1] = i1 < a.target ? v.y : 0.f;
  }
}


typedef _Float16 rs_h8 __attribute__((ext_vector_type(8)));
typedef float rs_f4 __attribute__((ext_vector_type(4)));
__device__ __forceinline__ void rs_split(float v, _Float16& h, _Float16& l) {
  h = static_cast<_Float16>(v);
  l = static_cast<_Float16>(v - static_cast<float>(h));
}
__global__ void __launch_bounds__(256) ps_resample_mfma_kernel(PitchArgs a) {
  __shared__ __attribute__((aligned(16))) _Float16 wh[kRsFrames][kRsLd];
  __shared__ __attribute__((aligned(16))) _Float16 wl[kRsFrames][kRsLd];
  __shared__ float red[4];
  const int tid = threadIdx.x, lane = tid & 63, wave = tid >> 6;
  const int e = blockIdx.y, f0 = blockIdx.x * kRsFrames;
  const float* y = a.y + static_cast<int64_t>(e) * a.l1;
  const int2 yr = a.yr[e];
  if (ps_window_silent(a, yr, e, f0 * a.orig - a.width, f0, kRsFrames, tid, 256)) return;
  constexpr int kPairs = kRsFrames * kRsK / 2, kPer = kPairs / 256;
  float v0[kPer], v1[kPer];
  float mx = 0.f;
#pragma unroll
  for (int u = 0; u < kPer; ++u) {
    const int p = tid + 256 * u, fr = p / (kRsK / 2), q = 2 * (p - fr * (kRsK / 2));
    const int src = (f0 + fr) * a.orig - a.width + q;
    const int s0 = min(max(src, 0), a.l1 - 1), s1 = min(max(src + 1, 0), a.l1 - 1);
    const float x0 = y[s0], x1 = y[s1];
    v0[u] = (src >= yr.x && src < yr.y && q < kPsTapMax) ? x0 : 0.f;
    v1[u] = (src + 1 >= yr.x && src + 1 < yr.y && q + 1 < kPsTapMax) ? x1 : 0.f;
    mx = fmaxf(mx, fmaxf(fabsf(v0[u]), fabsf(v1[u])));
  }
  const int n = lane & 15, kq = lane >> 4;
  rs_h8 bh[2][5], bl[2][5];
#pragma unroll
  for (int t = 0; t < 2; ++t) {
    const int ph = min(16 * (2 * wave + t) + n, a.nw - 1);
    const float* tr = a.taps + ph * kPsTapMax;
#pragma unroll
    for (int ks = 0; ks < 5; ++ks)
#pragma unroll
      for (int j = 0; j < 8; ++j) {
        const int q = 32 * ks + 8 * kq + j;
        const float tv = tr[min(q, kPsTapMax - 1)];
        _Float16 h, l;
        rs_split(q < kPsTapMax ? tv * 1024.f : 0.f, h, l);
        bh[t][ks][j] = h;
        bl[t][ks][j] = l;
      }
  }
  for (int o = 32; o >= 1; o >>= 1) mx = fmaxf(mx, __shfl_xor(mx, o, 64));
  if (lane == 0) red[wave] = mx;
  __syncthreads();
  mx = fmaxf(fmaxf(red[0], red[1]), fmaxf(red[2], red[3]));
  const int ex = mx > 0.f ? min(14 - ilogbf(mx), 100) : 0;
  const float scale = ldexpf(1.f, ex), unscale = ldexpf(1.f, -ex - 10);
#pragma unroll
  for (int u = 0; u < kPer; ++u) {
    const int p = tid + 256 * u, fr = p / (kRsK / 2), q = 2 * (p - fr * (kRsK / 2));
    _Float16 h0, l0, h1, l1;
    rs_split(v0[u] * scale, h0, l0);
    rs_split(v1[u] * scale, h1, l1);
    wh[fr][q] = h0;
    wh[fr][q + 1] = h1;
    wl[fr][q] = l0;
    wl[fr][q + 1] = l1;
  }
  __syncthreads();
  float* out = a.out + static_cast<int64_t>(a.idx[e]) * a.out_stride;
#pragma unroll
  for (int ft = 0; ft < kRsFrames / 16; ++ft) {
    rs_f4 acc[2] = {{0.f, 0.f, 0.f, 0.f}, {0.f, 0.f, 0.f, 0.f}};
#pragma unroll
    for (int ks = 0; ks < 5; ++ks) {
      const rs_h8 ah = *reinterpret_cast<const rs_h8*>(&wh[16 * ft + n][32 * ks + 8 * kq]);
      const rs_h8 al = *reinterpret_cast<const rs_h8*>(&wl[16 * ft + n][32 * ks + 8 * kq]);
#pragma unroll
      for (int t = 0; t < 2; ++t) {
        acc[t] = __builtin_amdgcn_mfma_f32_16x16x32_f16(ah, bh[t][ks], acc[t], 0, 0, 0);
        acc[t] = __builtin_amdgcn_mfma_f32_16x16x32_f16(ah, bl[t][ks], acc[t], 0, 0, 0);
        acc[t] = __builtin_amdgcn_mfma_f32_16x16x32_f16(al, bh[t][ks], acc[t], 0, 0, 0);
      }
    }
#pragma unroll
    for (int t = 0; t < 2; ++t) {
      const int ph = 16 * (2 * wave + t) + n;
#pragma unroll
      for (int j = 0; j < 4; ++j) {
        const int i = (f0 + 16 * ft + 4 * kq + j) * a.nw + ph;
        if (ph < a.nw && i < a.L) out[i] = i < a.target ? acc[t][j] * unscale : 0.f;
      }
    }
  }
}

PitchKnobs read_pitch_knobs() {
  PitchKnobs k;
  const char* s = getenv("HBK_PS_SPAN");
  k.span = !(s && s[0] == '0');
  s = getenv("HBK_PS_PAIR");
  k.pair = !(s && s[0] == '0');
  k.resample_valu = getenv("HBK_PS_RESAMPLE_VALU") != nullptr;
  return k;
}

int vocoder_lds_opt_in() {
  constexpr int kDevices = 64;
  static std::atomic<bool> done[kDevices];
  int dev = -1;
  HBK_HIP(hipGetDevice(&dev));
  const bool tracked = dev >= 0 && dev < kDevices;
  if (tracked && done[dev].load(std::memory_order_acquire)) return HBK_OK;
  HBK_HIP(hipFuncSetAttribute(reinterpret_cast<const void*>(ps_vocoder_kernel),
                              hipFuncAttributeMaxDynamicSharedMemorySize, int(sizeof(PvShared))));
  if (tracked) done[dev].store(true, std::memory_order_release);
  return HBK_OK;
}

template <typename... Params, typename... Args>
void launch(void (*kernel)(Params...), const Grid& g, size_t lds, hipStream_t st, Args... args) {
  hipLaunchKernelGGL(kernel, dim3(g.x, g.y), dim3(g.block), lds, st, args...);
}

}

#ifdef HBK_PHASE_TIMING
int pv_phase_take(unsigned long long* out) {
  if (hipMemcpyFromSymbol(out, HIP_SYMBOL(g_pv_phase), sizeof(unsigned long long) * 5) != hipSuccess) return -2;
  unsigned long long z[5] = {};
  (void)hipMemcpyToSymbol(HIP_SYMBOL(g_pv_phase), z, sizeof(z));
  return 0;
}
#endif

}

extern "C" {

int64_t hbk_pitch_shift_workspace_size(int64_t n, int64_t T, int32_t sample_rate, int32_t num, int32_t den) {
  hbk::PitchGeometry g;
  std::string err;
  if (n <= 0 || hbk::pitch_geometry(T, sample_rate, num, den, g, err) != HBK_OK) return 0;
  return hbk::pitch_layout(g, n).total;
}

int hbk_pitch_shift(const float* x, int64_t x_stride, int64_t n, const int32_t* idx, int64_t T, int32_t sample_rate,
                    int32_t num, int32_t den, float* out, int64_t out_stride, void* workspace,
                    int64_t workspace_bytes, void* stream) {
  using namespace hbk;
  if (n < 0) return arg_error("negative n");
  if (n == 0) return HBK_OK;
  if (n > 65535) return arg_error("n > 65535 per call");
  if (!x || !idx || !out || !workspace) return arg_error("NULL pointer");
  PitchGeometry g;
  std::string err;
  const int rc = pitch_geometry(T, sample_rate, num, den, g, err);
  if (rc != HBK_OK) {
    set_error("%s", err.c_str());
    return rc;
  }
  if (x_stride < T || out_stride < T) return arg_error("stride < T");
  const PitchLayout off = pitch_layout(g, n);
  if (workspace_bytes < off.total) return arg_error("workspace too small (hbk_pitch_shift_workspace_size)");
  const PitchKnobs knobs = read_pitch_knobs();
  const PitchLaunches L = pitch_launches(g, n, knobs);
  unsigned char* w = static_cast<unsigned char*>(workspace);
  PitchArgs a{};
  a.x = x;
  a.x_stride = x_stride;
  a.idx = idx;
  a.n = static_cast<int>(n);
  a.out = out;
  a.out_stride = out_stride;
  a.L = g.L, a.f_in = g.f_in, a.f_out = g.f_out, a.l1 = g.l1;
  a.orig = g.orig, a.nw = g.nw, a.width = g.width, a.target = g.target;
  a.rate = g.rate;
  a.y = reinterpret_cast<float*>(w + off.y);
  a.taps = reinterpret_cast<float*>(w + off.taps);
  a.yr = reinterpret_cast<int2*>(w + off.yr);
  a.span = knobs.span ? 1 : 0;
  if (L.pair) {
    a.sp = reinterpret_cast<int2*>(w + off.sp);
    a.key = reinterpret_cast<uint64_t*>(w + off.key);
    a.ord = reinterpret_cast<int32_t*>(w + off.ord);
    a.gord = reinterpret_cast<int32_t*>(w + off.gord);
  }
  const int lds_rc = vocoder_lds_opt_in();
  if (lds_rc != HBK_OK) return lds_rc;
  hipStream_t st = as_stream(stream);
  launch(ps_taps_kernel, L.taps, 0, st, a);
  HBK_LAUNCH_CHECK("ps_taps_kernel");
  if (L.pair) {
    launch(ps_span_kernel, L.span, 0, st, a);
    HBK_LAUNCH_CHECK("ps_span_kernel");
    launch(ps_rank_kernel, L.rank_clips, 0, st, static_cast<const uint64_t*>(a.key), a.n, a.ord);
    HBK_LAUNCH_CHECK("ps_rank_kernel");
    launch(ps_group_kernel, L.group, 0, st, a, L.groups);
    HBK_LAUNCH_CHECK("ps_group_kernel");
    launch(ps_rank_kernel, L.rank_groups, 0, st, static_cast<const uint64_t*>(a.key), L.groups, a.gord);
    HBK_LAUNCH_CHECK("ps_rank_kernel");
  }
  launch(ps_vocoder_kernel, L.vocoder, sizeof(PvShared), st, a);
  HBK_LAUNCH_CHECK("ps_vocoder_kernel");
  launch(L.resample_mfma ? ps_resample_mfma_kernel : ps_resample_kernel, L.resample, 0, st, a);
  HBK_LAUNCH_CHECK(L.resample_mfma ? "ps_resample_mfma_kernel" : "ps_resample_kernel");
  return HBK_OK;
}

}
```

### hey-buddy_amd/heybuddy/_native.py

```python
from __future__ import annotations

import ctypes
import os
import threading
from typing import Optional

import torch

__all__ = ["HBKError", "HBKUnavailable", "lib", "check", "stream_ptr", "require_device",
           "LIB_PATH"]

LIB_PATH = os.environ.get(
    "HBK_LIB",
    os.path.join(os.path.dirname(os.path.dirname(os.path.abspath(__file__))), "lib", "libhbk.so"),
)


class HBKError(RuntimeError):
    """A libhbk.so entry point returned a non-zero status."""


class HBKUnavailable(HBKError):
    """libhbk.so (or a HIP device) is not available: the HIP path cannot run."""


_lock = threading.Lock()
_lib: Optional[ctypes.CDLL] = None

_c_int64 = ctypes.c_int64
_c_int = ctypes.c_int
_c_float = ctypes.c_float
_vp = ctypes.c_void_p

_PROTOS = {
    "hbk_version": (ctypes.c_char_p, []),
    "hbk_last_error": (ctypes.c_char_p, []),
    "hbk_device_count": (_c_int, [ctypes.POINTER(_c_int)]),
    "hbk_stream_create_cu_mask": (_c_int, [_vp, _c_int, ctypes.POINTER(_vp)]),
    "hbk_stream_destroy": (_c_int, [_vp]),
    "hbk_profile_mark": (_c_int, [ctypes.c_int32, _vp]),
    "hbk_mel_plan_create": (_c_int, [_vp, _vp, _c_int, _c_int, _c_int, _c_float, _c_float,
                                     _c_float, _c_float, ctypes.POINTER(_vp)]),
    "hbk_mel_plan_destroy": (_c_int, [_vp]),
    "hbk_mel_set_variant": (_c_int, [_vp, ctypes.c_int32]),
    "hbk_mel_plan_info": (_c_int, [_vp, ctypes.POINTER(ctypes.c_int32)]),
    "hbk_mel_frames": (_c_int, [_vp, _vp, _c_int64, _c_int64, _c_int64, _vp, _vp]),
    "hbk_embed_plan_create": (_c_int, [_vp, ctypes.c_int32, ctypes.c_int32, ctypes.c_int32, _vp,
                                       ctypes.c_int32, ctypes.POINTER(_vp)]),
    "hbk_embed_plan_create_ex": (_c_int, [_vp, ctypes.c_int32, ctypes.c_int32, ctypes.c_int32, _vp,
                                          ctypes.c_int32, ctypes.c_int32, ctypes.POINTER(_vp)]),
    "hbk_embed_plan_destroy": (_c_int, [_vp]),
    "hbk_embed_plan_info": (_c_int, [_vp, ctypes.POINTER(ctypes.c_int32),
                                     ctypes.POINTER(ctypes.c_int32), ctypes.POINTER(ctypes.c_int32),
                                     ctypes.POINTER(ctypes.c_double),
                                     ctypes.POINTER(ctypes.c_double),
                                     ctypes.POINTER(ctypes.c_int32)]),
    "hbk_embed_workspace_size": (_c_int, [_vp, _c_int64, ctypes.POINTER(_c_int64)]),
    "hbk_embed_clips": (_c_int, [_vp, _vp, _c_int64, _c_int64, _vp, _vp, _c_int64, _vp]),
    "hbk_embed_split_info": (_c_int, [_vp, ctypes.c_int32, ctypes.POINTER(_c_int64)]),
    "hbk_embed_clips_front": (_c_int, [_vp, _vp, _c_int64, _c_int64, ctypes.c_int32, _vp, _vp, _c_int64, _vp]),
    "hbk_embed_clips_back": (_c_int, [_vp, _vp, _c_int64, ctypes.c_int32, _vp, _vp, _c_int64, _vp]),
    "hbk_embed_windows": (_c_int, [_vp, _vp, _c_int64, _vp, _vp, _c_int64, _vp]),
    "hbk_nan_rows_workspace_size": (_c_int64, [_c_int64]),
    "hbk_nan_rows_fix": (_c_int, [_vp, _c_int64, _c_int64, ctypes.c_uint64, _vp, _c_int64, _vp]),
    "hbk_embed_range_status": (_c_int, [_vp, ctypes.POINTER(ctypes.c_int32), ctypes.c_int32, _vp]),
    "hbk_reverb_plan_create": (_c_int, [_c_int64, ctypes.POINTER(_vp)]),
    "hbk_reverb_plan_destroy": (_c_int, [_vp]),
    "hbk_reverb_spectrum": (_c_int, [_vp, _vp, _c_int64, _c_int64, _vp, _vp]),
    "hbk_augment": (_c_int, [_vp, _vp, _c_int64, _c_int64, _vp, _c_int64, _vp, _vp, _vp, _vp, _vp,
                             _vp, _c_int64, _vp]),
    "hbk_colored_noise": (_c_int, [_vp, _vp, _c_int64, _c_int64, _vp, _c_int64, ctypes.c_uint64, _c_int64, _vp,
                                   _vp, _c_float, _vp, _c_int64, _vp, _c_int64, _vp]),
    "hbk_augment_colored": (_c_int, [_vp, _vp, _c_int64, _c_int64, _vp, _c_int64, _vp, _vp, _vp, _vp, _vp,
                                     _vp, _c_int64, ctypes.c_uint64, _c_int64, _vp, _vp, _c_float, _vp, _c_int64,
                                     _vp, _c_int64, _vp, _c_int64, _vp]),
    "hbk_colored_noise_workspace_size": (_c_int64, [_c_int64, _c_int64]),
    "hbk_colored_noise_ws": (_c_int, [_vp, _vp, _c_int64, _c_int64, _vp, _c_int64, ctypes.c_uint64, _c_int64, _vp,
                                      _vp, _c_float, _vp, _c_int64, _vp, _c_int64, _vp, _c_int64, _vp]),
    "hbk_tanh_distortion": (_c_int, [_vp, _c_int64, _c_int64, _vp, _vp, _c_int64, _vp, _c_int64, _vp]),
    "hbk_band_stop_workspace_size": (_c_int64, [_c_int64, ctypes.c_int32, ctypes.c_int32, _vp]),
    "hbk_band_stop": (_c_int, [_vp, _vp, _c_int64, _c_int64, _vp, _vp, ctypes.c_int32, _vp, _vp, _vp, _vp,
                               ctypes.c_int32, _vp, _vp, _vp, _c_int64, _vp, _c_int64, _vp]),
    "hbk_pitch_shift_workspace_size": (_c_int64, [_c_int64, _c_int64, ctypes.c_int32, ctypes.c_int32,
                                                  ctypes.c_int32]),
    "hbk_pitch_shift": (_c_int, [_vp, _c_int64, _c_int64, _vp, _c_int64, ctypes.c_int32, ctypes.c_int32,
                                 ctypes.c_int32, _vp, _c_int64, _vp, _c_int64, _vp]),
    "hbk_seven_band_eq": (_c_int, [_vp, _c_int64, _c_int64, _vp, _vp, _c_int64, _vp, _c_int64, _vp]),
    "hbk_place_clips": (_c_int, [_vp, _c_int64, _c_int64, _vp, _vp, _vp, _c_int64, _c_int64, _vp]),
    "hbk_place_clips_idx": (_c_int, [_vp, _c_int64, _c_int64, _vp, _vp, _vp, _c_int64, _vp, _c_int64, _c_int64,
                                     _vp]),
    "hbk_seven_band_eq_src": (_c_int, [_vp, _c_int64, _c_int64, _vp, _vp, _c_int64, _vp, _c_int64,
                                       _vp, _c_int64, _vp, _vp, _vp]),
    "hbk_tanh_distortion_src": (_c_int, [_vp, _c_int64, _c_int64, _vp, _vp, _c_int64, _vp, _c_int64,
                                         _vp, _c_int64, _vp, _vp, _vp]),
    "hbk_reverb_plan_set_source": (_c_int, [_vp, _vp, _c_int64, _vp, _vp]),
    "hbk_mlp_set_step_scalars": (_c_int, [_vp, _vp]),
    "hbk_mlp_plan_create": (_c_int, [ctypes.c_int32] * 4 + [ctypes.POINTER(_vp)]),
    "hbk_mlp_plan_destroy": (_c_int, [_vp]),
    "hbk_mlp_layout": (_c_int, [_vp, ctypes.POINTER(_c_int64), _vp, ctypes.c_int32]),
    "hbk_mlp_workspace_size": (_c_int, [_vp, _c_int64, ctypes.POINTER(_c_int64)]),
    "hbk_mlp_forward": (_c_int, [_vp, _vp, _vp, _c_int64, _vp, _vp, _c_float, ctypes.c_uint64,
                                 _vp, _c_int64, _vp]),
    "hbk_mlp_train_fwd_bwd": (_c_int, [_vp, _vp, _vp, _vp, _c_int64, _c_float, _c_float, _c_float,
                                       _c_float, ctypes.c_uint64, _vp, _vp, _vp, _c_int64, _vp]),
    "hbk_mlp_gate_adam": (_c_int, [_vp, _vp, _vp, _vp, _vp, _vp, _vp, _vp, ctypes.c_int32,
                                   _c_float, _c_float, _c_float, _c_float, _vp]),
    "hbk_mlp_fused_supported": (_c_int, [_vp, ctypes.POINTER(ctypes.c_int32)]),
    "hbk_mlp_step_variant": (_c_int, [_vp, _c_int64, _vp, ctypes.POINTER(ctypes.c_int32)]),
    "hbk_mlp_step_plan_info": (_c_int, [_vp, _c_int64, _vp, ctypes.POINTER(ctypes.c_int32), ctypes.c_int32]),
    "hbk_mlp_step_fwd_bwd": (_c_int, [_vp, _vp, _vp, _c_int64, _vp, _c_int64, _vp, _c_int64, _vp, _c_int64,
                                      _c_int64, _vp, ctypes.c_int32, _vp, _c_int64, _c_float, _c_float,
                                      _c_float, _c_float, ctypes.c_uint64, _vp, _vp, _c_int64, ctypes.c_int32,
                                      _vp, _c_int64, _vp]),
    "hbk_mlp_step_update": (_c_int, [_vp, _vp, _vp, _vp, _vp, _vp, ctypes.c_int32, _vp, _c_int64, _c_float,
                                     _c_float, _c_float, _c_float, _vp, ctypes.c_int32, _vp, _c_int64, _vp]),
    "hbk_mlp_eval_workspace_size": (_c_int, [_vp, _c_int64, ctypes.POINTER(_c_int64)]),
    "hbk_mlp_eval_prepare": (_c_int, [_vp, _vp, _vp, _c_int64, _vp]),
    "hbk_mlp_eval_count_multi": (_c_int, [_vp, _vp, ctypes.c_int32, _vp, ctypes.c_int32, _vp, _vp, _vp, _vp, _vp,
                                          _vp, _c_float, _c_float, _vp, _c_int64, _vp]),
    "hbk_mlp_eval_count": (_c_int, [_vp, _vp, _vp, ctypes.c_int32, _c_int64, _vp, _c_int64, _c_int64,
                                    ctypes.c_int32, _c_float, _c_float, ctypes.c_uint64, _vp, _vp, _vp, _c_int64,
                                    _vp]),
    "hbk_mlp_eval_laps": (_c_int, [_c_int64, _c_int64, ctypes.c_int32, ctypes.c_int32,
                                   ctypes.POINTER(_c_int64)]),
    "hbk_mlp_eval_finish": (_c_int, [_vp, _vp, ctypes.POINTER(ctypes.c_double), _c_float, _c_float, _vp,
                                     _c_int64, _c_int64, _vp, _vp]),
}


class GraphOp(ctypes.Structure):
    _fields_ = [
        ("kind", ctypes.c_int32), ("kh", ctypes.c_int32), ("kw", ctypes.c_int32),
        ("cin", ctypes.c_int32), ("cout", ctypes.c_int32), ("act", ctypes.c_int32),
        ("alpha", ctypes.c_float), ("weight", _vp), ("bias", _vp),
    ]


def exported_symbols() -> list[str]:
    return list(_PROTOS)


def lib() -> ctypes.CDLL:
    global _lib
    if _lib is not None:
        return _lib
    with _lock:
        if _lib is not None:
            return _lib
        if not os.path.exists(LIB_PATH):
            raise HBKUnavailable(
                f"libhbk.so not found at {LIB_PATH}; build it with "
                "`python hey-buddy_amd/build.py` (the HIP path has no fallback)")
        try:
            handle = ctypes.CDLL(LIB_PATH, mode=ctypes.RTLD_GLOBAL)
        except OSError as e:
            raise HBKUnavailable(f"cannot load {LIB_PATH}: {e}") from e
        for name, (res, args) in _PROTOS.items():
            fn = getattr(handle, name)
            fn.restype = res
            fn.argtypes = args
        _lib = handle
        return _lib


def check(rc: int, what: str = "") -> None:
    if rc != 0:
        msg = lib().hbk_last_error().decode(errors="replace")
        raise HBKError(f"{what}: status {rc}: {msg}")


def require_device(device: Optional[torch.device | int] = None) -> torch.device:
    lib()
    if not torch.cuda.is_available():
        raise HBKUnavailable("no HIP device visible: the hey-buddy MI355X path needs a GPU")
    if device is None:
        return torch.device("cuda", torch.cuda.current_device())
    if isinstance(device, int):
        return torch.device("cuda", device)
    device = torch.device(device)
    if device.type != "cuda":
        raise HBKUnavailable(f"device {device} is not a HIP device")
    return device if device.index is not None else torch.device("cuda", torch.cuda.current_device())


def stream_ptr(device: Optional[torch.device] = None) -> int:
    return torch.cuda.current_stream(device).cuda_stream


def ptr(t: torch.Tensor) -> int:
    return t.data_ptr()
```

### hey-buddy_amd/heybuddy/dataset/augmented.py

```python
from __future__ import annotations

from typing import Any, Dict, Iterator, List, Optional, Sequence

import os
import numpy as np
import torch

from heybuddy.constants import (DEFAULT_AUGMENT_BACKGROUND_NOISE_MAX_SNR_DB,
                                DEFAULT_AUGMENT_BACKGROUND_NOISE_MIN_SNR_DB, DEFAULT_AUGMENT_BAND_STOP_PROB,
                                DEFAULT_AUGMENT_COLORED_NOISE_MAX_F_DECAY,
                                DEFAULT_AUGMENT_COLORED_NOISE_MAX_SNR_DB,
                                DEFAULT_AUGMENT_COLORED_NOISE_MIN_F_DECAY,
                                DEFAULT_AUGMENT_COLORED_NOISE_MIN_SNR_DB, DEFAULT_AUGMENT_COLORED_NOISE_PROB,
                                DEFAULT_AUGMENT_PITCH_SHIFT_PROB, DEFAULT_AUGMENT_PITCH_SHIFT_SEMITONES,
                                DEFAULT_AUGMENT_TANH_DISTORTION_PROB, DEFAULT_AUGMENT_TANH_MAX_DISTORTION,
                                DEFAULT_AUGMENT_TANH_MIN_DISTORTION,
                                DEFAULT_AUGMENT_BACKGROUND_NOISE_PROB, DEFAULT_AUGMENT_GAIN_MAX_DB,
                                DEFAULT_AUGMENT_GAIN_MIN_DB, DEFAULT_AUGMENT_GAIN_PROB,
                                DEFAULT_AUGMENT_REVERB_PROB, DEFAULT_AUGMENT_SEVEN_BAND_GAIN_DB,
                                DEFAULT_AUGMENT_SEVEN_BAND_PROB)
from heybuddy.kernels import ReverbPlan, SourceView, pitch_shift, place_clips, seven_band_eq, tanh_distortion

__all__ = ["AugmentedAudioGenerator", "BatchAugmenter", "SourceOrder", "bandstop_cutoffs", "eq_coefficients",
           "eq_parameters", "hf_shuffle_permutation", "source_plan", "target_length_offset", "target_length_offsets",
           "to_target_length"]

T = 23040



def _u(shape, lo: float = 0.0, hi: float = 1.0) -> np.ndarray:
    return (torch.rand(shape, dtype=torch.float64) * (hi - lo) + lo).numpy()


def hf_shuffle_permutation(n: int) -> np.ndarray:
    _, keys, pos, *_ = np.random.get_state()
    seed = keys[pos] if pos < 624 else keys[0]
    np.random.random()
    return np.random.default_rng(seed).permutation(n)


class SourceOrder:

    def __init__(self, n: int) -> None:
        if n <= 0:
            raise ValueError("source dataset is empty")
        self.n = int(n)
        self.perm = np.arange(self.n)
        self.pos = 0

    def take(self, m: int) -> np.ndarray:
        out = np.empty(int(m), dtype=np.int64)
        for i in range(int(m)):
            if self.pos == self.n:
                self.perm = hf_shuffle_permutation(self.n)
                self.pos = 0
            out[i] = self.perm[self.pos]
            self.pos += 1
        return out

EQ_BANDS = ((42.0, 95.0), (91.0, 204.0), (196.0, 441.0), (421.0, 948.0), (909.0, 2045.0),
            (1957.0, 4404.0), (4216.0, 9486.0))
EQ_Q_RANGE = (0.5, 1.33)


def eq_parameters(n: int, gain_db: float, sample_rate: int = 16000) -> np.ndarray:
    mel = lambda f: 2595.0 * np.log10(1.0 + np.asarray(f) / 700.0)
    lo, hi = mel([b[0] for b in EQ_BANDS]), mel([b[1] for b in EQ_BANDS])
    f0 = 700.0 * (10.0 ** ((lo + _u((n, 7)) * (hi - lo)) / 2595.0) - 1.0)
    f0[:, 6] = np.minimum(f0[:, 6], (sample_rate // 2) * 0.95)
    g = _u((n, 7), -gain_db, gain_db)
    q = _u((n, 7), *EQ_Q_RANGE)
    return np.stack([f0, g, q], axis=-1)


def eq_coefficients(params: np.ndarray, sample_rate: int = 16000) -> np.ndarray:
    p = np.asarray(params, dtype=np.float64)
    A = 10.0 ** (p[..., 1] / 40.0)
    w0 = 2.0 * np.pi * p[..., 0] / sample_rate
    c, al = np.cos(w0), np.sin(w0) / (2.0 * p[..., 2])
    r = 2.0 * np.sqrt(A) * al
    Ap, Am = A + 1.0, A - 1.0
    peak = (1 + al * A, -2 * c, 1 - al * A, 1 + al / A, -2 * c, 1 - al / A)
    low = (A * (Ap - Am * c + r), 2 * A * (Am - Ap * c), A * (Ap - Am * c - r),
           Ap + Am * c + r, -2 * (Am + Ap * c), Ap + Am * c - r)
    high = (A * (Ap + Am * c + r), -2 * A * (Am + Ap * c), A * (Ap + Am * c - r),
            Ap - Am * c + r, 2 * (Am - Ap * c), Ap - Am * c - r)
    kind = np.arange(7)
    b0, b1, b2, a0, a1, a2 = (np.where(kind == 0, lo_, np.where(kind == 6, hi_, pk_))
                              for lo_, hi_, pk_ in zip(low, high, peak))
    return np.stack([b0 / a0, b1 / a0, b2 / a0, a1 / a0, a2 / a0], axis=-1)


def bandstop_cutoffs(n: int, sample_rate: int = 16000):
    def mel(f):
        return 2595.0 * np.log10(1.0 + f / 700.0)
    m = _u(n, mel(200.0), mel(4000.0)).astype(np.float32)
    fc = (np.float32(700.0) * (np.float32(10.0) ** (m / np.float32(2595.0)) - np.float32(1.0))).astype(np.float32)
    bw = _u(n, 0.5, 1.99).astype(np.float32)
    sr = np.float32(sample_rate)
    lo = (fc * (np.float32(1.0) - bw / np.float32(2.0)) / sr).astype(np.float32)
    hi = (fc * (np.float32(1.0) + bw / np.float32(2.0)) / sr).astype(np.float32)
    return lo, hi


def _pinned(t: torch.Tensor) -> torch.Tensor:
    return t.pin_memory() if torch.cuda.is_available() else t


def fast_shifts(sample_rate: int = 16000, semitones: float = DEFAULT_AUGMENT_PITCH_SHIFT_SEMITONES) -> list:
    from fractions import Fraction
    from itertools import combinations
    from math import prod
    fac, n, d = [], int(sample_rate), 2
    while n > 1:
        while n % d == 0:
            fac.append(d)
            n //= d
        d += 1
    products = {prod(c) for r in range(1, len(fac) + 1) for c in combinations(fac, r)}
    lo, hi = Fraction(2.0 ** (-semitones / 12.0)), Fraction(2.0 ** (semitones / 12.0))
    return sorted({Fraction(i, j) for i in products for j in products if lo <= Fraction(i, j) <= hi} - {1})


ROUTE_PLACE, ROUTE_EQ, ROUTE_TANH, ROUTE_AUGMENT = 0, 1, 2, 3


def first_touch_enabled() -> bool:
    return os.environ.get("HBK_PLACE_FIRST_TOUCH", "1") != "0"


def first_touch_routes(eq_on: np.ndarray, tanh_on: np.ndarray, placed_first: np.ndarray) -> np.ndarray:
    eq_on, tanh_on, placed_first = (np.asarray(a, dtype=bool) for a in (eq_on, tanh_on, placed_first))
    route = np.where(placed_first, ROUTE_PLACE, ROUTE_AUGMENT).astype(np.int8)
    route[tanh_on] = ROUTE_TANH
    route[eq_on] = ROUTE_EQ
    return route


class BatchAugmenter:
    def __init__(self, noise: Optional[Sequence[torch.Tensor]] = None,
                 impulse_responses: Optional[Sequence[torch.Tensor]] = None,
                 device: Optional[torch.device] = None, batch_size: int = 128,
                 background_noise_prob: float = DEFAULT_AUGMENT_BACKGROUND_NOISE_PROB,
                 background_noise_min_snr_db: float = DEFAULT_AUGMENT_BACKGROUND_NOISE_MIN_SNR_DB,
                 background_noise_max_snr_db: float = DEFAULT_AUGMENT_BACKGROUND_NOISE_MAX_SNR_DB,
                 reverb_prob: float = DEFAULT_AUGMENT_REVERB_PROB,
                 gain_prob: float = DEFAULT_AUGMENT_GAIN_PROB,
                 min_gain_in_db: float = DEFAULT_AUGMENT_GAIN_MIN_DB,
                 max_gain_in_db: float = DEFAULT_AUGMENT_GAIN_MAX_DB,
                 colored_noise_prob: float = DEFAULT_AUGMENT_COLORED_NOISE_PROB,
                 colored_noise_min_snr_db: float = DEFAULT_AUGMENT_COLORED_NOISE_MIN_SNR_DB,
                 colored_noise_max_snr_db: float = DEFAULT_AUGMENT_COLORED_NOISE_MAX_SNR_DB,
                 colored_noise_min_f_decay: float = DEFAULT_AUGMENT_COLORED_NOISE_MIN_F_DECAY,
                 colored_noise_max_f_decay: float = DEFAULT_AUGMENT_COLORED_NOISE_MAX_F_DECAY,
                 tanh_distortion_prob: float = DEFAULT_AUGMENT_TANH_DISTORTION_PROB,
                 tanh_min_distortion: float = DEFAULT_AUGMENT_TANH_MIN_DISTORTION,
                 tanh_max_distortion: float = DEFAULT_AUGMENT_TANH_MAX_DISTORTION,
                 seven_band_prob: float = DEFAULT_AUGMENT_SEVEN_BAND_PROB,
                 seven_band_gain_db: float = DEFAULT_AUGMENT_SEVEN_BAND_GAIN_DB,
                 band_stop_prob: float = DEFAULT_AUGMENT_BAND_STOP_PROB,
                 sample_rate: int = 16000,
                 pitch_shift_prob: float = DEFAULT_AUGMENT_PITCH_SHIFT_PROB,
                 pitch_shift_semitones: float = DEFAULT_AUGMENT_PITCH_SHIFT_SEMITONES) -> None:
        self.plan = ReverbPlan(device)
        self.device = self.plan.device
        if background_noise_prob > 0 and not noise:
            raise ValueError("Background noise is enabled but no augmentation dataset is provided")
        if reverb_prob > 0 and not impulse_responses:
            raise ValueError("Reverb is enabled but no impulse response dataset is provided")
        self.batch_size = int(batch_size)
        self.p_noise = float(background_noise_prob)
        self.p_reverb = float(reverb_prob)
        self.snr_min = float(background_noise_min_snr_db)
        self.snr_max = float(background_noise_max_snr_db)
        self.p_gain = float(gain_prob)
        self.gain_min_db = float(min_gain_in_db)
        self.gain_max_db = float(max_gain_in_db)
        self.p_colored = float(colored_noise_prob)
        self.colored_snr = (float(colored_noise_min_snr_db), float(colored_noise_max_snr_db))
        self.colored_decay = (float(colored_noise_min_f_decay), float(colored_noise_max_f_decay))
        self.sample_rate = int(sample_rate)
        self.p_tanh = float(tanh_distortion_prob)
        self.tanh_range = (float(tanh_min_distortion), float(tanh_max_distortion))
        self.p_eq = float(seven_band_prob)
        self.eq_gain_db = float(seven_band_gain_db)
        self.p_bandstop = float(band_stop_prob)
        self.p_pitch = float(pitch_shift_prob)
        self.pitch_shifts = fast_shifts(self.sample_rate, pitch_shift_semitones) if self.p_pitch > 0 else []
        if self.p_pitch > 0 and not self.pitch_shifts:
            raise ValueError(f"no fast pitch shift within +-{pitch_shift_semitones} semitones at {sample_rate} Hz")
        self.ring = None
        self.lengths: List[int] = []
        self.starts: List[int] = []
        if noise:
            parts = [n.reshape(-1).to(self.device, torch.float32) for n in noise]
            self.ring = torch.cat(parts)
            self.lengths = [p.numel() for p in parts]
            self.starts = list(np.cumsum([0] + self.lengths[:-1]))
        self.spectra = None
        if impulse_responses:
            ks = torch.stack([ReverbPlan.rotated_kernel(ir.to(self.device), T) for ir in impulse_responses])
            self.spectra = self.plan.spectra(ks)
        self.noise_idx = 0
        self.ir_idx = 0
        self._advance = {}
        self.timing: Optional[list] = None

    def _tick(self, name: str, start: Optional[Any]) -> Optional[Any]:
        if self.timing is None:
            return None
        ev = torch.cuda.Event(enable_timing=True)
        ev.record()
        if start is not None and name:
            self.timing.append((name, start, ev))
        return ev

    def _noise_advance(self, idx: int, nb: int) -> int:
        key = (idx, nb)
        nxt = self._advance.get(key)
        if nxt is None:
            need, covered, nxt = nb * T, 0, idx
            while covered < need:
                covered += self.lengths[nxt]
                nxt = (nxt + 1) % len(self.lengths)
            self._advance[key] = nxt
        return nxt

    def plan_batches(self, n: int, coins: Optional[np.ndarray] = None):
        bs = self.batch_size
        nbat = (n + bs - 1) // bs
        sizes = np.full(nbat, bs, dtype=np.int64)
        sizes[-1] = n - bs * (nbat - 1)
        batch = np.repeat(np.arange(nbat), sizes)
        pos = np.arange(n) - batch * bs
        if coins is None:
            coins = np.random.rand(nbat, 2)
        coins = np.asarray(coins, dtype=np.float64).reshape(nbat, 2)
        gain_db = np.zeros(n, dtype=np.float32)
        if self.p_gain > 0:
            g_on = _u(nbat) < self.p_gain
            g_db = _u(nbat, self.gain_min_db, self.gain_max_db)
            gain_db = np.where(g_on, g_db, 0.0).astype(np.float32)[batch]
        colored_snr = np.full(n, np.nan, dtype=np.float32)
        colored_fd = np.zeros(n, dtype=np.float32)
        if self.p_colored > 0:
            c_on = _u(nbat) < self.p_colored
            c_snr = _u(nbat, *self.colored_snr)
            c_fd = _u(nbat, *self.colored_decay)
            colored_snr = np.where(c_on, c_snr, np.nan).astype(np.float32)[batch]
            colored_fd = c_fd.astype(np.float32)[batch]
        noise_off = np.full(n, -1, dtype=np.int64)
        n_on = (coins[:, 0] < self.p_noise) if self.ring is not None else np.zeros(nbat, bool)
        if n_on.any():
            start = np.full(nbat, -1, dtype=np.int64)
            for b in np.flatnonzero(n_on):
                start[b] = self.starts[self.noise_idx]
                self.noise_idx = self._noise_advance(self.noise_idx, int(sizes[b]))
            sel = start[batch] >= 0
            noise_off[sel] = start[batch][sel] + pos[sel] * T
        spec_idx = np.full(n, -1, dtype=np.int32)
        r_on = (coins[:, 1] < self.p_reverb) if self.spectra is not None else np.zeros(nbat, bool)
        if r_on.any():
            n_spec = self.spectra.shape[0]
            ir = (self.ir_idx + np.cumsum(r_on) - 1) % n_spec
            self.ir_idx = int((self.ir_idx + r_on.sum()) % n_spec)
            per_clip = np.where(r_on, ir, -1).astype(np.int32)[batch]
            spec_idx[:] = per_clip
        self._colored = (colored_snr, colored_fd)
        p_bs = getattr(self, "p_bandstop", 0.0)
        b_on = (_u(nbat) < p_bs) if p_bs > 0 else np.zeros(nbat, bool)
        lo, hi = bandstop_cutoffs(int(b_on.sum()), getattr(self, "sample_rate", 16000))
        sel = b_on[batch]
        per = np.full(nbat, -1, dtype=np.int64)
        per[b_on] = np.arange(int(b_on.sum()))
        self._bandstop = (np.flatnonzero(sel).astype(np.int32), lo[per[batch][sel]], hi[per[batch][sel]])
        self._pitch = []
        if getattr(self, "p_pitch", 0.0) > 0:
            p_on = _u(nbat) < self.p_pitch
            p_pick = torch.randint(0, len(self.pitch_shifts), (nbat,)).numpy()
            for j, f in enumerate(self.pitch_shifts):
                clips = np.flatnonzero((p_on & (p_pick == j))[batch]).astype(np.int32)
                if clips.size:
                    self._pitch.append((f.numerator, f.denominator, clips))
        p_eq = getattr(self, "p_eq", 0.0)
        e_on = (_u(n) < p_eq) if p_eq > 0 else np.zeros(n, bool)
        sr = getattr(self, "sample_rate", 16000)
        eq_idx = np.nonzero(e_on)[0].astype(np.int32)
        self._eq = (eq_idx, eq_coefficients(eq_parameters(eq_idx.size, getattr(self, "eq_gain_db", 0.0), sr), sr))
        p_tanh = getattr(self, "p_tanh", 0.0)
        self._tanh = np.full(n, np.nan, dtype=np.float32)
        if p_tanh > 0:
            t_on = _u(n) < p_tanh
            t_amt = _u(n, *getattr(self, "tanh_range", (0.0, 0.0)))
            self._tanh = np.where(t_on, t_amt, np.nan).astype(np.float32)
        return noise_off, spec_idx, gain_db

    def prepare(self, n: int, coins: Optional[np.ndarray] = None) -> Dict[str, Any]:
        noise_off, spec_idx, gain_db = self.plan_batches(n, coins)
        ring_len = 0 if self.ring is None else self.ring.numel()
        if ring_len:
            noise_off = np.where(noise_off >= 0, noise_off % ring_len, -1)
        snr = torch.zeros(n, dtype=torch.float32)
        if (noise_off >= 0).any():
            snr = torch.from_numpy(_u(n, self.snr_min, self.snr_max).astype(np.float32))
        gain = None
        if self.p_gain > 0:
            gain = torch.pow(10.0, torch.from_numpy(gain_db) / 20.0)
        eq_idx, eq_coef = self._eq
        eq = None
        if eq_idx.size:
            eq = (_pinned(torch.from_numpy(eq_coef)), _pinned(torch.from_numpy(eq_idx)))
        tanh = None if np.isnan(self._tanh).all() else torch.from_numpy(self._tanh)
        bs_idx, bs_lo, bs_hi = self._bandstop
        bandstop = None
        if bs_idx.size:
            bandstop = (torch.from_numpy(bs_idx), torch.from_numpy(bs_lo), torch.from_numpy(bs_hi))
        colored_snr, colored_fd = self._colored
        colored = None
        if not np.isnan(colored_snr).all():
            colored = (torch.from_numpy(colored_fd), torch.from_numpy(colored_snr),
                       int(torch.randint(0, 2 ** 62, (1,)).item()))
        pr = {"n": n, "noise_off": torch.from_numpy(noise_off), "spec_idx": torch.from_numpy(spec_idx),
              "snr": snr, "gain": gain, "eq": eq, "tanh": tanh, "bandstop": bandstop, "colored": colored,
              "pitch": [(a, b, _pinned(torch.from_numpy(c))) for a, b, c in getattr(self, "_pitch", [])]}
        pr["route"] = self.routes(pr)
        return pr

    def _colored_fold(self) -> bool:
        return self.sample_rate == 16000 and os.environ.get("HBK_AUG_COLORED_FOLD", "1") != "0"

    def routes(self, pr: Dict[str, Any]) -> np.ndarray:
        n = pr["n"]
        placed_first = np.zeros(n, dtype=bool)
        for _, _, clips in pr.get("pitch") or []:
            placed_first[clips.numpy()] = True
        if pr.get("bandstop") is not None:
            placed_first[pr["bandstop"][0].numpy()] = True
        if pr.get("colored") is not None:
            fd, csnr = pr["colored"][0], pr["colored"][1]
            if self._colored_fold():
                rows = ReverbPlan.colored_fallback_rows(csnr, fd, self.batch_size,
                                                        self.plan.colored_group_path(n, self.batch_size))
                placed_first[rows.numpy()] = True
            else:
                placed_first |= ~torch.isnan(csnr).numpy()
        eq_on = np.zeros(n, dtype=bool)
        if pr.get("eq") is not None:
            eq_on[pr["eq"][1].numpy()] = True
        tanh_on = np.zeros(n, dtype=bool) if pr.get("tanh") is None else ~torch.isnan(pr["tanh"]).numpy()
        return first_touch_routes(eq_on, tanh_on, placed_first)

    def __call__(self, x: torch.Tensor, out: Optional[torch.Tensor] = None,
                 prepared: Optional[Dict[str, Any]] = None, source: Optional[Dict[int, SourceView]] = None
                 ) -> torch.Tensor:
        n = x.shape[0]
        pr = self.prepare(n) if prepared is None else prepared
        if pr["n"] != n:
            raise ValueError(f"prepared for {pr['n']} clips, called with {n}")
        source = source or {}
        if source and (out is None or out.data_ptr() != x.data_ptr()):
            raise ValueError("a source view needs the chain in place (out is x)")
        ev = self._tick("", None)
        if pr["eq"] is not None:
            if out is None:
                out = torch.empty((n, T), dtype=torch.float32, device=x.device)
            if out.data_ptr() != x.data_ptr():
                out.copy_(x[:, :T])
            x = seven_band_eq(out, pr["eq"][0], idx=pr["eq"][1], source=source.get(ROUTE_EQ))
            ev = self._tick("eq", ev)
        if pr["tanh"] is not None:
            x = tanh_distortion(x, pr["tanh"], out=out, source=source.get(ROUTE_TANH))
            out = x
            ev = self._tick("tanh", ev)
        for num, den, clips in pr.get("pitch") or []:
            if out is None:
                out = torch.empty((n, T), dtype=torch.float32, device=x.device)
            x = pitch_shift(x, clips, num, den, out=out, sample_rate=self.sample_rate)
            ev = self._tick("pitch", ev)
        if pr.get("bandstop") is not None:
            if out is None:
                out = x[:, :T].clone()
            elif out.data_ptr() != x.data_ptr():
                out.copy_(x[:, :T])
            x = self.plan.band_stop(out, *pr["bandstop"], out=out)
            ev = self._tick("bandstop", ev)
        colored = None
        if pr["colored"] is not None:
            fd, csnr, seed = pr["colored"]
            if self._colored_fold():
                colored = (fd, csnr, seed, self.batch_size)
            else:
                x = self.plan.colored_noise(x, fd, csnr, seed=seed, out=out, sample_rate=self.sample_rate,
                                            clips_per_noise=self.batch_size)
                out = x
                ev = self._tick("colored", ev)
        y = self.plan.augment(x, self.ring, pr["noise_off"], pr["snr"], self.spectra, pr["spec_idx"],
                              out=out, gain=pr["gain"], colored=colored, source=source.get(ROUTE_AUGMENT))
        self._tick("mix_reverb", ev)
        return y


def source_plan(source_lengths: Sequence[int], num_samples: int, batch_size: int, target_num_samples: int):
    src = np.asarray(source_lengths, dtype=np.int64)
    order = SourceOrder(src.shape[0])
    rows, pres, coins = [], [], []
    for b0 in range(0, int(num_samples), int(batch_size)):
        r = order.take(min(int(batch_size), int(num_samples) - b0))
        rows.append(r)
        pres.append(target_length_offsets(src[r], target_num_samples))
        coins.append(np.random.rand(2))
    if not rows:
        return np.zeros(0, np.int64), np.zeros(0, np.int32), np.zeros((0, 2))
    return (np.concatenate(rows), np.concatenate(pres).astype(np.int32),
            np.array(coins, dtype=np.float64).reshape(-1, 2))


def target_length_offset(num_samples: int, target_num_samples: int) -> int:
    total = target_num_samples - num_samples
    if total <= 1:
        return 0
    return int(np.random.randint(int(total / 4), int(3 * total / 4)))


def target_length_offsets(lengths: Sequence[int], target_num_samples: int) -> np.ndarray:
    lengths = np.asarray(lengths, dtype=np.int64)
    total = target_num_samples - lengths
    pre = np.zeros(lengths.shape[0], dtype=np.int32)
    pad = total > 1
    if pad.any():
        t = total[pad]
        pre[pad] = np.random.randint((t / 4).astype(np.int64), (3 * t / 4).astype(np.int64))
    return pre


def to_target_length(audio: np.ndarray, target_num_samples: int) -> np.ndarray:
    if audio.dtype == np.int16:
        audio = audio.astype(np.float32) / 32768.0
    n = audio.shape[0]
    if n >= target_num_samples:
        return audio[:target_num_samples]
    pre = target_length_offset(n, target_num_samples)
    out = np.zeros(target_num_samples, dtype=np.float32)
    out[pre:pre + n] = audio
    return out


def _audio_arrays(dataset: Any) -> List[Dict[str, Any]]:
    out = []
    for row in dataset:
        if isinstance(row, dict) and "audio" in row:
            row = row["audio"]
        if isinstance(row, dict):
            out.append({"array": row["array"], "sampling_rate": int(row.get("sampling_rate", 16000))})
        else:
            out.append({"array": row, "sampling_rate": 16000})
    return out


def _as_float_array(a: Any) -> np.ndarray:
    if torch.is_tensor(a):
        a = a.detach().cpu().numpy()
    a = np.asarray(a)
    if a.dtype == np.int16:
        return a.astype(np.float32) / 32768.0
    return a.astype(np.float32, copy=False)


class AugmentedAudioGenerator:

    def __init__(self, source_dataset: Any, device_id: Optional[int] = None,
                 augmentation_dataset: Any = None, impulse_response_dataset: Any = None,
                 target_length: float = 1.44, sample_rate: int = 16000, batch_size: int = 128,
                 seven_band_aug_prob: float = DEFAULT_AUGMENT_SEVEN_BAND_PROB,
                 seven_band_aug_gain_db: float = DEFAULT_AUGMENT_SEVEN_BAND_GAIN_DB,
                 tanh_distortion_prob: float = DEFAULT_AUGMENT_TANH_DISTORTION_PROB,
                 tanh_min_distortion: float = DEFAULT_AUGMENT_TANH_MIN_DISTORTION,
                 tanh_max_distortion: float = DEFAULT_AUGMENT_TANH_MAX_DISTORTION,
                 pitch_shift_prob: float = 0.25, pitch_shift_semitones: int = 3,
                 band_stop_prob: float = 0.25,
                 colored_noise_prob: float = DEFAULT_AUGMENT_COLORED_NOISE_PROB,
                 colored_noise_min_snr_db: float = DEFAULT_AUGMENT_COLORED_NOISE_MIN_SNR_DB,
                 colored_noise_max_snr_db: float = DEFAULT_AUGMENT_COLORED_NOISE_MAX_SNR_DB,
                 colored_noise_min_f_decay: float = DEFAULT_AUGMENT_COLORED_NOISE_MIN_F_DECAY,
                 colored_noise_max_f_decay: float = DEFAULT_AUGMENT_COLORED_NOISE_MAX_F_DECAY,
                 background_noise_prob: float = DEFAULT_AUGMENT_BACKGROUND_NOISE_PROB,
                 background_noise_min_snr_db: float = DEFAULT_AUGMENT_BACKGROUND_NOISE_MIN_SNR_DB,
                 background_noise_max_snr_db: float = DEFAULT_AUGMENT_BACKGROUND_NOISE_MAX_SNR_DB,
                 gain_prob: float = DEFAULT_AUGMENT_GAIN_PROB,
                 reverb_prob: float = DEFAULT_AUGMENT_REVERB_PROB) -> None:
        if background_noise_prob > 0 and not augmentation_dataset:
            raise ValueError("Background noise is enabled but no augmentation dataset is provided")
        if reverb_prob > 0 and not impulse_response_dataset:
            raise ValueError("Reverb is enabled but no impulse response dataset is provided")
        self.device_id = device_id
        self.source_dataset = source_dataset
        self.augmentation_dataset = augmentation_dataset
        self.impulse_response_dataset = impulse_response_dataset
        self.target_length = target_length
        self.sample_rate = int(sample_rate)
        self.batch_size = int(batch_size)
        self.reverb_prob = reverb_prob
        self.background_noise_prob = background_noise_prob
        self.background_noise_min_snr_db = background_noise_min_snr_db
        self.background_noise_max_snr_db = background_noise_max_snr_db
        dev = None if device_id is None else torch.device("cuda", device_id)

        def bank(ds):
            if not ds:
                return None
            from heybuddy.util import resample
            rows = _audio_arrays(ds)
            return [resample(torch.from_numpy(_as_float_array(r["array"]).reshape(-1)), int(r["sampling_rate"]),
                             self.sample_rate) for r in rows]

        self.augmenter = BatchAugmenter(
            bank(augmentation_dataset), bank(impulse_response_dataset), device=dev,
            batch_size=self.batch_size, background_noise_prob=background_noise_prob,
            background_noise_min_snr_db=background_noise_min_snr_db,
            background_noise_max_snr_db=background_noise_max_snr_db, reverb_prob=reverb_prob,
            gain_prob=gain_prob, colored_noise_prob=colored_noise_prob,
            colored_noise_min_snr_db=colored_noise_min_snr_db, colored_noise_max_snr_db=colored_noise_max_snr_db,
            colored_noise_min_f_decay=colored_noise_min_f_decay, colored_noise_max_f_decay=colored_noise_max_f_decay,
            tanh_distortion_prob=tanh_distortion_prob, tanh_min_distortion=tanh_min_distortion,
            tanh_max_distortion=tanh_max_distortion, seven_band_prob=seven_band_aug_prob,
            seven_band_gain_db=seven_band_aug_gain_db, band_stop_prob=band_stop_prob, sample_rate=self.sample_rate,
            pitch_shift_prob=pitch_shift_prob, pitch_shift_semitones=pitch_shift_semitones)
        self.device = self.augmenter.device
        self._source: Optional[List[Dict[str, Any]]] = None
        self._order: Optional[SourceOrder] = None

    @property
    def target_num_samples(self) -> int:
        return int(self.target_length * self.sample_rate)

    def to_target_length(self, audio: np.ndarray) -> np.ndarray:
        return to_target_length(np.asarray(audio), self.target_num_samples)

    def to_audio_array(self, audio: Any) -> np.ndarray:
        if isinstance(audio, list):
            if not audio:
                raise ValueError("Audio list is empty")
            first = audio[0][0] if isinstance(audio[0], list) else audio[0]
            return np.array(audio, dtype=np.float32 if isinstance(first, float) else np.int16)
        return audio

    def get_next_audio_sample_dict(self) -> Dict[str, Any]:
        if self._source is None:
            self._source = list(self.source_dataset)
            self._order = SourceOrder(len(self._source))
        row = self._source[int(self._order.take(1)[0])]
        return row if isinstance(row, dict) and "audio" in row else {"audio": _audio_arrays([row])[0]}

    def place_batch(self, batch: Sequence[Any]) -> torch.Tensor:
        from heybuddy.util import resample
        T = self.target_num_samples
        arrays = []
        for audio in batch:
            a = audio["array"] if isinstance(audio, dict) else audio
            sr = audio.get("sampling_rate", self.sample_rate) if isinstance(audio, dict) else self.sample_rate
            a = _as_float_array(self.to_audio_array(a)).reshape(-1)
            if sr != self.sample_rate:
                a = resample(torch.from_numpy(a), int(sr), self.sample_rate).numpy()
            arrays.append(a)
        lens = np.array([a.shape[0] for a in arrays], dtype=np.int32)
        pre = target_length_offsets(lens, T)
        width = max(int(lens.max()), 1)
        host = torch.zeros((len(arrays), width), dtype=torch.float32).pin_memory()
        for i, a in enumerate(arrays):
            host[i, :a.shape[0]] = torch.from_numpy(a)
        return place_batch_device(host.to(self.device, non_blocking=True), lens, pre, T)

    def execute_augment_batch(self, batch: Sequence[Any]) -> torch.Tensor:
        placed = self.place_batch(batch)
        return self.augmenter(placed, out=placed)

    def plan_batches(self, lens: Sequence[int]):
        lens = np.asarray(lens, dtype=np.int64)
        pres, coins = [], []
        for b0 in range(0, lens.shape[0], self.batch_size):
            pres.append(target_length_offsets(lens[b0:b0 + self.batch_size], self.target_num_samples))
            coins.append(np.random.rand(2))
        pre = np.concatenate(pres).astype(np.int32) if pres else np.zeros(0, np.int32)
        return pre, np.array(coins, dtype=np.float64).reshape(-1, 2)

    def plan_source(self, source_lengths: Sequence[int], num_samples: int):
        return source_plan(source_lengths, num_samples, self.batch_size, self.target_num_samples)

    def prepare_device(self, clips: torch.Tensor, lengths: Optional[Sequence[int]] = None) -> Dict[str, Any]:
        n = clips.shape[0]
        lens = np.full(n, clips.shape[1], dtype=np.int32) if lengths is None else np.asarray(lengths, np.int32)
        pre, coins = self.plan_batches(lens)
        return {"lens": lens, "pre": pre, "chain": self.augmenter.prepare(n, coins)}

    def augment_device(self, clips: torch.Tensor, lengths: Optional[Sequence[int]] = None,
                       prepared: Optional[Dict[str, Any]] = None) -> torch.Tensor:
        pr = self.prepare_device(clips, lengths) if prepared is None else prepared
        T = self.target_num_samples
        route = pr["chain"].get("route")
        if route is None or not first_touch_enabled() or T != ReverbPlan.T or not clips.shape[1]:
            placed = place_clips(clips, pr["lens"], pr["pre"], T)
            return self.augmenter(placed, out=placed, prepared=pr["chain"])
        n = clips.shape[0]
        lens = np.asarray(pr["lens"], dtype=np.int32).reshape(n)
        pre = np.asarray(pr["pre"], dtype=np.int32).reshape(n)
        if lens.size and (int(lens.min()) < 0 or int(lens.max()) > clips.shape[1] or int(pre.min()) < 0
                          or int((pre + np.minimum(lens, T)).max()) > T):
            raise ValueError("lens / pre must place every clip inside [0, T)")
        routes = (ROUTE_EQ, ROUTE_TANH, ROUTE_AUGMENT)
        host = np.stack([lens, pre] + [np.where(route == r, pre, -1).astype(np.int32) for r in routes])
        dev = _pinned(torch.from_numpy(host)).to(clips.device, non_blocking=True)
        self.placed_rows = np.flatnonzero(route == ROUTE_PLACE).astype(np.int32)
        placed = place_clips(clips, dev[0], dev[1], T, idx=torch.from_numpy(self.placed_rows))
        source = {r: SourceView(clips, dev[0], dev[2 + i]) for i, r in enumerate(routes)}
        return self.augmenter(placed, out=placed, prepared=pr["chain"], source=source)

    def __call__(self, num_samples: int, **kwargs: Any) -> Iterator[Dict[str, Any]]:
        total_batches = int(np.ceil(num_samples / self.batch_size))
        for i in range(total_batches):
            nb = min(self.batch_size, num_samples - i * self.batch_size)
            items = [self.get_next_audio_sample_dict() for _ in range(nb)]
            out = self.execute_augment_batch([it["audio"] for it in items]).cpu().numpy()
            for audio, item in zip(out, items):
                yield {"audio": {"array": audio, "sampling_rate": self.sample_rate},
                       **{k: v for k, v in item.items() if k != "audio"}}


def place_batch_device(src: torch.Tensor, lengths: np.ndarray, pre: np.ndarray, T: int) -> torch.Tensor:
    if not pre.any() and src.shape[1] >= T and (lengths >= T).all():
        return src[:, :T]
    return place_clips(src, lengths, pre, T)
```

### hey-buddy_amd/heybuddy/dataset/features.py

```python
from __future__ import annotations

import math
import os
import random
import re
import zlib
from typing import Any, Callable, List, Optional, Sequence, Tuple, Union

import numpy as np
import torch

from heybuddy.constants import (DEFAULT_ADVERSARIAL_PHRASES, DEFAULT_AUGMENT_BACKGROUND_NOISE_MAX_SNR_DB,
                                DEFAULT_AUGMENT_BACKGROUND_NOISE_MIN_SNR_DB,
                                DEFAULT_AUGMENT_BACKGROUND_NOISE_PROB,
                                DEFAULT_AUGMENT_COLORED_NOISE_MAX_F_DECAY,
                                DEFAULT_AUGMENT_COLORED_NOISE_MAX_SNR_DB,
                                DEFAULT_AUGMENT_COLORED_NOISE_MIN_F_DECAY,
                                DEFAULT_AUGMENT_COLORED_NOISE_MIN_SNR_DB, DEFAULT_AUGMENT_COLORED_NOISE_PROB,
                                DEFAULT_AUGMENT_GAIN_PROB, DEFAULT_AUGMENT_REVERB_PROB,
                                DEFAULT_AUGMENT_TANH_DISTORTION_PROB, DEFAULT_AUGMENT_TANH_MAX_DISTORTION,
                                DEFAULT_AUGMENT_TANH_MIN_DISTORTION, DEFAULT_EMBEDDING_BATCH_SIZE,
                                DEFAULT_EMBEDDING_SPECTROGRAM_BATCH_SIZE, DEFAULT_FEATURE_BATCH_SIZE,
                                DEFAULT_AUGMENT_BATCH_SIZE, DEFAULT_AUGMENT_BAND_STOP_PROB,
                                DEFAULT_AUGMENT_PHRASE_PROB, DEFAULT_AUGMENT_PITCH_SHIFT_PROB,
# ... 131 lines not shown
class TrainingFeaturesGenerator:

    def __init__(self, device_id: Optional[int] = None, use_tqdm: bool = True, use_autoconfigure: bool = True,
                 sample_rate: int = 16000, sample_batch_size: int = DEFAULT_FEATURE_BATCH_SIZE,
                 tts_text: str = "Hello, world!", tts_additional_texts: List[str] = [],
                 tts_adversarial: bool = False, tts_adversarial_num_phrases: int = DEFAULT_ADVERSARIAL_PHRASES,
                 tts_adversarial_custom_phrases: List[str] = [], tts_batch_size: int = DEFAULT_TTS_BATCH_SIZE,
                 tts_phrase_augment_prob: float = DEFAULT_AUGMENT_PHRASE_PROB,
                 tts_phrase_augment_words: Sequence[str] = (),
                 augment_target_length: float = 1.44, augment_batch_size: int = DEFAULT_AUGMENT_BATCH_SIZE,
                 augment_sample_ratio: float = DEFAULT_AUGMENT_SAMPLE_RATIO,
                 augment_dataset_streaming: bool = False,
                 augment_background_dataset: SupplementalDatasetType = None,
                 augment_impulse_dataset: SupplementalDatasetType = None,
                 augment_seven_band_prob: float = DEFAULT_AUGMENT_SEVEN_BAND_PROB,
                 augment_seven_band_gain_db: float = DEFAULT_AUGMENT_SEVEN_BAND_GAIN_DB,
                 augment_tanh_distortion_prob: float = DEFAULT_AUGMENT_TANH_DISTORTION_PROB,
                 augment_tanh_min_distortion: float = DEFAULT_AUGMENT_TANH_MIN_DISTORTION,
                 augment_tanh_max_distortion: float = DEFAULT_AUGMENT_TANH_MAX_DISTORTION,
                 augment_pitch_shift_prob: float = DEFAULT_AUGMENT_PITCH_SHIFT_PROB,
                 augment_pitch_shift_semitones: int = DEFAULT_AUGMENT_PITCH_SHIFT_SEMITONES,
                 augment_band_stop_prob: float = DEFAULT_AUGMENT_BAND_STOP_PROB,
                 augment_colored_noise_prob: float = DEFAULT_AUGMENT_COLORED_NOISE_PROB,
                 augment_colored_noise_min_snr_db: float = DEFAULT_AUGMENT_COLORED_NOISE_MIN_SNR_DB,
                 augment_colored_noise_max_snr_db: float = DEFAULT_AUGMENT_COLORED_NOISE_MAX_SNR_DB,
                 augment_colored_noise_min_f_decay: float = DEFAULT_AUGMENT_COLORED_NOISE_MIN_F_DECAY,
                 augment_colored_noise_max_f_decay: float = DEFAULT_AUGMENT_COLORED_NOISE_MAX_F_DECAY,
                 augment_background_noise_prob: float = DEFAULT_AUGMENT_BACKGROUND_NOISE_PROB,
                 augment_background_noise_min_snr_db: float = DEFAULT_AUGMENT_BACKGROUND_NOISE_MIN_SNR_DB,
                 augment_background_noise_max_snr_db: float = DEFAULT_AUGMENT_BACKGROUND_NOISE_MAX_SNR_DB,
                 augment_gain_prob: float = DEFAULT_AUGMENT_GAIN_PROB,
                 augment_reverb_prob: float = DEFAULT_AUGMENT_REVERB_PROB,
                 embedding_spectrogram_batch_size: int = DEFAULT_EMBEDDING_SPECTROGRAM_BATCH_SIZE,
                 embedding_batch_size: int = DEFAULT_EMBEDDING_BATCH_SIZE) -> None:
        self.device_id = device_id
        self.use_autoconfigure = use_autoconfigure
        self.use_tqdm = use_tqdm
        self.sample_rate = sample_rate
        self.sample_batch_size = sample_batch_size
        self.tts_text = tts_text
        self.tts_additional_texts = list(tts_additional_texts)
        self.tts_adversarial = tts_adversarial
        self.tts_adversarial_num_phrases = tts_adversarial_num_phrases
        self.tts_adversarial_custom_phrases = list(tts_adversarial_custom_phrases)
        self.tts_batch_size = tts_batch_size
        self.tts_phrase_augment_prob = tts_phrase_augment_prob
        self.tts_phrase_augment_words = list(tts_phrase_augment_words)
        self.augment_target_length = augment_target_length
        self.augment_sample_ratio = augment_sample_ratio
        self.augment_batch_size = augment_batch_size
        self.augment_dataset_streaming = augment_dataset_streaming
        self.augment_background_dataset = augment_background_dataset
        self.augment_impulse_dataset = augment_impulse_dataset
        self.augment_seven_band_prob = augment_seven_band_prob
        self.augment_seven_band_gain_db = augment_seven_band_gain_db
        self.augment_tanh_distortion_prob = augment_tanh_distortion_prob
        self.augment_tanh_min_distortion = augment_tanh_min_distortion
        self.augment_tanh_max_distortion = augment_tanh_max_distortion
        self.augment_pitch_shift_prob = augment_pitch_shift_prob
        self.augment_pitch_shift_semitones = augment_pitch_shift_semitones
        self.augment_band_stop_prob = augment_band_stop_prob
        self.augment_colored_noise_prob = augment_colored_noise_prob
        self.augment_colored_noise_min_snr_db = augment_colored_noise_min_snr_db
        self.augment_colored_noise_max_snr_db = augment_colored_noise_max_snr_db
        self.augment_colored_noise_min_f_decay = augment_colored_noise_min_f_decay
        self.augment_colored_noise_max_f_decay = augment_colored_noise_max_f_decay
        self.augment_background_noise_prob = augment_background_noise_prob
        self.augment_background_noise_min_snr_db = augment_background_noise_min_snr_db
        self.augment_background_noise_max_snr_db = augment_background_noise_max_snr_db
        self.augment_gain_prob = augment_gain_prob
        self.augment_reverb_prob = augment_reverb_prob
        self.embedding_spectrogram_batch_size = embedding_spectrogram_batch_size
        self.embedding_batch_size = embedding_batch_size
        self._augmenters: dict = {}

    @property
    def device(self) -> torch.device:
        from heybuddy import _native
        return _native.require_device(self.device_id)

    def autoconfigure(self) -> None:
        from heybuddy import _native
        dev = _native.require_device(self.device_id)
        self.device_id = dev.index
        self.tts_batch_size = 64
        self.augment_batch_size = 128
        self.embedding_spectrogram_batch_size = 128
        self.embedding_batch_size = 128

    def get_speech_embeddings_model(self):
        from heybuddy.embeddings import get_speech_embeddings
        return get_speech_embeddings(device_id=self.device.index)

    def get_tts_generator(self) -> SyntheticSpeechGenerator:
        self._tts_calls = getattr(self, "_tts_calls", 0) + 1
        seed = (zlib.crc32(f"{self.tts_text}|{self.tts_adversarial}".encode()) + 7919 * self._tts_calls) % (2 ** 31 - 1)
        return SyntheticSpeechGenerator(self.tts_text, adversarial=self.tts_adversarial,
                                        num_adversarial_texts=self.tts_adversarial_num_phrases,
                                        device_id=self.device.index, target_sample_rate=self.sample_rate, seed=seed)

    def _bank(self, which: str, testing: bool) -> Any:
        ds = self.augment_background_dataset if which == "noise" else self.augment_impulse_dataset
        if ds is None or not _is_hub_name(ds):
            return ds
        from heybuddy.synthetic import impulse_responses, noise_bank
        logger.warning(f"{which} dataset {ds!r} is a Hugging Face repo (no network): using the synthetic "
                       f"{which} bank of heybuddy.synthetic")
        seed = 1000 + (7 if testing else 0)
        return noise_bank(64, seed=seed) if which == "noise" else impulse_responses(32, seed=seed + 1)

    def get_augmented_generator(self, dataset: Any = None, testing: bool = False) -> AugmentedAudioGenerator:
        key = (testing, self.augment_batch_size)
        if key not in self._augmenters:
            self._augmenters[key] = AugmentedAudioGenerator(
                dataset if dataset is not None else [], device_id=self.device.index,
                batch_size=self.augment_batch_size,
                target_length=self.augment_target_length, sample_rate=self.sample_rate,
                augmentation_dataset=self._bank("noise", testing),
                impulse_response_dataset=self._bank("ir", testing),
                seven_band_aug_prob=self.augment_seven_band_prob,
                seven_band_aug_gain_db=self.augment_seven_band_gain_db,
                tanh_distortion_prob=self.augment_tanh_distortion_prob,
                tanh_min_distortion=self.augment_tanh_min_distortion,
                tanh_max_distortion=self.augment_tanh_max_distortion,
                pitch_shift_prob=self.augment_pitch_shift_prob,
                pitch_shift_semitones=self.augment_pitch_shift_semitones,
                band_stop_prob=self.augment_band_stop_prob,
                colored_noise_prob=self.augment_colored_noise_prob,
                colored_noise_min_snr_db=self.augment_colored_noise_min_snr_db,
                colored_noise_max_snr_db=self.augment_colored_noise_max_snr_db,
                colored_noise_min_f_decay=self.augment_colored_noise_min_f_decay,
                colored_noise_max_f_decay=self.augment_colored_noise_max_f_decay,
                background_noise_prob=self.augment_background_noise_prob,
                background_noise_min_snr_db=self.augment_background_noise_min_snr_db,
                background_noise_max_snr_db=self.augment_background_noise_max_snr_db,
                gain_prob=self.augment_gain_prob, reverb_prob=self.augment_reverb_prob)
        return self._augmenters[key]

    def augment_device(self, clips: torch.Tensor, lengths: np.ndarray, num_samples: int,
                       testing: bool = False, validation: bool = False) -> torch.Tensor:
        T = int(self.sample_rate * self.augment_target_length)
        n_tts = clips.shape[0]
        if validation:
            from heybuddy.kernels import place_clips
            lens = np.minimum(lengths, T).astype(np.int32)
            pre = ((T - lens) // 2).astype(np.int32)
            return place_clips(clips, lens, pre, T)
        aug = self.get_augmented_generator(testing=testing)
        aug.augmenter.noise_idx = aug.augmenter.ir_idx = 0
        rows, pre, coins = aug.plan_source(lengths, num_samples)
        lens = np.asarray(lengths)[rows].astype(np.int32)
        same = num_samples == n_tts and np.array_equal(rows, np.arange(n_tts))
        src = clips if same else clips.index_select(0, torch.from_numpy(rows).to(clips.device))
        prepared = {"lens": lens, "pre": pre, "chain": aug.augmenter.prepare(num_samples, coins)}
        return aug.augment_device(src, lens, prepared=prepared)

    def generate_device(self, num_samples: int, testing: bool = False, validation: bool = False) -> torch.Tensor:
        if self.use_autoconfigure:
            self.autoconfigure()
        if validation:
            tts_num_samples = num_samples
        else:
            tts_num_samples = max(1, min(num_samples, int(num_samples // self.augment_sample_ratio)))
        clips, lengths = self.get_tts_generator().device_batch(tts_num_samples)
        audio = self.augment_device(clips, lengths, num_samples, testing=testing, validation=validation)
        del clips
        return self.get_speech_embeddings_model().featurize(audio)

    def generate(self, num_samples: int, sample_save_path: Optional[str] = None,
                 augmented_sample_save_path: Optional[str] = None, testing: bool = False,
                 validation: bool = False) -> np.ndarray:
        if sample_save_path or augmented_sample_save_path:
            logger.warning("sample wav export needs an audio writer; skipped")
        return self.generate_device(num_samples, testing=testing, validation=validation).cpu().numpy()

    def _chunks(self, num_samples: int, fn: Callable[[int], Any]) -> List[Any]:
        sizes = [self.sample_batch_size] * math.ceil(num_samples / self.sample_batch_size)
        if num_samples % self.sample_batch_size:
            sizes[-1] = num_samples % self.sample_batch_size
        states = (np.random.get_state(), torch.random.get_rng_state(), random.getstate())
        parts = []
        try:
            for size in sizes:
                np.random.set_state(states[0])
                torch.random.set_rng_state(states[1])
                random.setstate(states[2])
                parts.append(fn(size))
        finally:
            np.random.set_state(states[0])
            torch.random.set_rng_state(states[1])
            random.setstate(states[2])
        return parts

    def __call__(self, num_samples: int, sample_save_path: Optional[str] = None,
                 augmented_sample_save_path: Optional[str] = None, testing: bool = False,
                 validation: bool = False) -> np.ndarray:
        parts = self._chunks(num_samples, lambda s: self.generate(s, sample_save_path, augmented_sample_save_path,
                                                                 testing, validation))
        return parts[0] if len(parts) == 1 else np.concatenate(parts)

    def call_device(self, num_samples: int, testing: bool = False, validation: bool = False) -> torch.Tensor:
        parts = self._chunks(num_samples, lambda s: self.generate_device(s, testing=testing, validation=validation))
        if not parts:
            return torch.empty((0, 16, 96), dtype=torch.float32, device=self.device)
        return parts[0] if len(parts) == 1 else torch.cat(parts)

    @classmethod
    def default(cls, wake_phrase: str, adversarial: bool = False, num_adversarial_phrases: int = 10,
                additional_wake_phrases: List[str] = [], custom_adversarial_phrases: List[str] = [],
                dataset_streaming: bool = False, tts_batch_size: int = DEFAULT_TTS_BATCH_SIZE,
                phrase_augment_prob: float = DEFAULT_AUGMENT_PHRASE_PROB,
                phrase_augment_words: Sequence[str] = (), augment_target_length: float = 1.44,
                augment_background_dataset: SupplementalDatasetType = DEFAULT_BACKGROUND_DATASET,
                augment_impulse_dataset: SupplementalDatasetType = DEFAULT_IMPULSE_DATASET,
                **kwargs: Any) -> "TrainingFeaturesGenerator":
        kwargs.pop("use_cache", None)
        if augment_background_dataset is None:
            augment_background_dataset = DEFAULT_BACKGROUND_DATASET
        if augment_impulse_dataset is None:
            augment_impulse_dataset = DEFAULT_IMPULSE_DATASET
        return cls(use_autoconfigure=True, tts_text=wake_phrase, tts_adversarial=adversarial,
                   tts_batch_size=tts_batch_size, tts_adversarial_num_phrases=num_adversarial_phrases,
                   tts_adversarial_custom_phrases=custom_adversarial_phrases,
                   tts_additional_texts=additional_wake_phrases, tts_phrase_augment_prob=phrase_augment_prob,
                   tts_phrase_augment_words=phrase_augment_words,
                   augment_background_dataset=augment_background_dataset,
                   augment_impulse_dataset=augment_impulse_dataset, augment_target_length=augment_target_length,
                   **kwargs)

    @classmethod
    def get_wake_phrase_file_name(cls, wake_phrase: str, testing: bool = False) -> str:
        return safe_name(wake_phrase).strip("_") + ("_tst" if testing else "")

    @classmethod
    def get_training_features(cls, wake_phrase: str, num_positive_samples: int, num_adversarial_samples: int,
                              num_adversarial_phrases: int = 10, additional_wake_phrases: List[str] = [],
                              custom_adversarial_phrases: List[str] = [], testing: bool = False,
                              use_cache: bool = True, save_samples: bool = True, keep_in_memory: bool = False,
                              directory: Optional[str] = None, device_id: Optional[int] = None, **kwargs: Any
                              ) -> Tuple[PrecalculatedDatasetIterator, PrecalculatedDatasetIterator]:
        from heybuddy.dataset.precalculated import LOCAL_DIR
        directory = directory or LOCAL_DIR
        name = cls.get_wake_phrase_file_name(wake_phrase, testing=testing)
        out = []
        for suffix, adversarial, n in (("", False, num_positive_samples), ("_adv", True, num_adversarial_samples)):
            it_name = name + suffix
            existing = None
            if use_cache:
                try:
                    existing = PrecalculatedDatasetIterator(it_name, directory=directory)
                except FileNotFoundError:
                    existing = None
            have = len(existing) if existing is not None else 0
            if existing is not None and have >= n:
                out.append(existing)
                continue
            gen = cls.default(wake_phrase, adversarial=adversarial, num_adversarial_phrases=num_adversarial_phrases,
                              additional_wake_phrases=additional_wake_phrases,
                              custom_adversarial_phrases=custom_adversarial_phrases, device_id=device_id, **kwargs)
            feats = _sharded(lambda m: gen.call_device(m, testing=testing), n - have)
            if have:
                feats = np.concatenate([np.asarray(existing.precalculated), feats])
            out.append(_save_then_open(feats, it_name, directory, keep_in_memory=keep_in_memory))
        return out[0], out[1]

    @classmethod
    def get_validation_features(cls, wake_phrase: str, num_positive_samples: int, use_cache: bool = True,
                                keep_in_memory: bool = False, augment_target_length: float = 1.44,
                                directory: Optional[str] = None, device_id: Optional[int] = None,
                                **kwargs: Any) -> PrecalculatedDatasetIterator:
        from heybuddy.dataset.precalculated import LOCAL_DIR
        directory = directory or LOCAL_DIR
        name = cls.get_wake_phrase_file_name(wake_phrase) + "_val"
        existing = None
        if use_cache:
            try:
                existing = PrecalculatedDatasetIterator(name, directory=directory)
            except FileNotFoundError:
                existing = None
        have = len(existing) if existing is not None else 0
        if existing is not None and have >= num_positive_samples:
            return existing
        gen = cls.default(wake_phrase, augment_target_length=augment_target_length, device_id=device_id)
        feats = _sharded(lambda m: gen.call_device(m, validation=True), num_positive_samples - have)
        if have:
            feats = np.concatenate([np.asarray(existing.precalculated), feats])
        return _save_then_open(feats, name, directory, keep_in_memory=keep_in_memory)
```

### hey-buddy_amd/heybuddy/kernels.py

```python
from __future__ import annotations

import contextlib
import ctypes
import os
import itertools
import threading
from typing import Dict

import numpy as np
import torch

from heybuddy import _native
from heybuddy._native import check, lib, ptr, stream_ptr

__all__ = ["MelPlan", "mel_frames"]

_plans: Dict[int, object] = {}
_plan_ids = itertools.count(1)
_plans_lock = threading.Lock()


def _register(plan) -> int:
    with _plans_lock:
        pid = next(_plan_ids)
# ... 613 lines not shown
        arr(ctypes.c_void_p, [counts.data_ptr() + 16 * w for w in which]), activation_threshold, dropout_p,
        ptr(ws), ws.numel(), stream_ptr(params.device)), "hbk_mlp_eval_count_multi")


@torch.library.custom_op("hbk::mlp_eval_finish_", mutates_args=("sched", "out"))
def _mlp_eval_finish_op(counts_val: torch.Tensor | None, counts_test: torch.Tensor | None, sizes: list[float],
                        target: float, ratio: float, sched: torch.Tensor | None, next_step: int,
                        out: torch.Tensor) -> None:
    sz = (ctypes.c_double * 4)(*sizes[:4])
    check(lib().hbk_mlp_eval_finish(
        ptr(counts_val) if counts_val is not None else None, ptr(counts_test) if counts_test is not None else None,
        sz, target, ratio, ptr(sched) if sched is not None else None, sched.shape[0] if sched is not None else 0,
        next_step, ptr(out), stream_ptr(out.device)), "hbk_mlp_eval_finish")


@torch.library.custom_op("hbk::nan_rows_fix_", mutates_args=("rows", "ws"))
def _nan_rows_fix_op(rows: torch.Tensor, seed: int, ws: torch.Tensor) -> None:
    n = rows.shape[0]
    check(lib().hbk_nan_rows_fix(ptr(rows), n, rows.numel() // max(n, 1), seed & (2 ** 64 - 1), ptr(ws), ws.numel(),
                                 stream_ptr(rows.device)), "hbk_nan_rows_fix")


def nan_rows_fix(rows: torch.Tensor, seed: int = 0, ws: torch.Tensor | None = None) -> torch.Tensor:
    _native.require_device(rows.device)
    n = rows.shape[0]
    if rows.dtype != torch.float32 or not rows.is_contiguous() or (n and (rows.numel() // n) % 4):
        raise ValueError("rows must be a contiguous float32 [n, ...] tensor with a multiple of 4 values per row")
    if n == 0:
        return rows
    need = int(lib().hbk_nan_rows_workspace_size(n))
    if ws is None or ws.numel() < need:
        ws = torch.empty(need, dtype=torch.uint8, device=rows.device)
    torch.ops.hbk.nan_rows_fix_(rows, _u64_to_i64(seed), ws)
    return rows


@torch.library.custom_op("hbk::place_clips", mutates_args=())
def _place_clips_op(src: torch.Tensor, src_len: torch.Tensor, pre: torch.Tensor, T: int) -> torch.Tensor:
    n = src.shape[0]
    out = torch.empty((n, T), dtype=torch.float32, device=src.device)
    if n:
        check(lib().hbk_place_clips(ptr(src), n, src.stride(0), ptr(src_len), ptr(pre), ptr(out), T, T,
                                    stream_ptr(src.device)), "hbk_place_clips")
    return out


@_place_clips_op.register_fake
def _(src, src_len, pre, T):
    return src.new_empty((src.shape[0], T))


@torch.library.custom_op("hbk::place_clips_idx_", mutates_args=("out",))
def _place_clips_idx_op(src: torch.Tensor, src_len: torch.Tensor, pre: torch.Tensor, idx: torch.Tensor,
                        out: torch.Tensor) -> None:
    check(lib().hbk_place_clips_idx(ptr(src), src.shape[0], src.stride(0), ptr(src_len), ptr(pre), ptr(idx),
                                    idx.numel(), ptr(out), out.stride(0), out.shape[1], stream_ptr(src.device)),
          "hbk_place_clips_idx")


class SourceView:

    def __init__(self, src: torch.Tensor, lens: torch.Tensor, pre: torch.Tensor) -> None:
        n = src.shape[0]
        if src.dim() != 2 or src.dtype != torch.float32 or src.stride(1) != 1:
            raise ValueError("src must be [n, S] float32 rows on the device")
        for t in (lens, pre):
            if t.dtype != torch.int32 or t.shape != (n,) or t.device != src.device or not t.is_contiguous():
                raise ValueError("lens / pre must be [n] int32 on src's device")
        self.src, self.lens, self.pre = src, lens, pre

    def check(self, x: torch.Tensor) -> "SourceView":
        if self.src.shape[0] != x.shape[0] or self.src.device != x.device:
            raise ValueError("the source view must cover x's clips on x's device")
        return self


def place_clips(src: torch.Tensor, src_len, pre, T: int = 23040, idx: torch.Tensor | None = None,
                out: torch.Tensor | None = None) -> torch.Tensor:
    dev = _native.require_device(src.device)
    if src.dim() != 2 or src.dtype != torch.float32 or src.stride(1) != 1:
        raise ValueError("src must be [n, S] float32 rows on the device")
    n = src.shape[0]

    def per_clip(v) -> torch.Tensor:
        t = torch.as_tensor(v, dtype=torch.int32).reshape(-1).contiguous()
        if t.numel() != n:
            raise ValueError("src_len / pre must have n entries")
        if t.device.type == "cpu":
            if bool((t < 0).any()):
                raise ValueError("src_len / pre must be >= 0")
            return t.pin_memory().to(dev, non_blocking=True)
        return t.to(dev)

    if torch.is_tensor(src_len) and src_len.device.type != "cpu":
        src_len = src_len.clamp(0, src.shape[1])
    elif int(np.max(np.asarray(src_len), initial=0)) > src.shape[1]:
        raise ValueError(f"src_len exceeds the {src.shape[1]} source columns")
    src_len, pre = per_clip(src_len), per_clip(pre)
    if idx is None and out is None:
        return torch.ops.hbk.place_clips(src, src_len, pre, int(T))
    if out is None:
        out = torch.empty((n, int(T)), dtype=torch.float32, device=dev)
    elif out.shape != (n, int(T)) or out.dtype != torch.float32 or out.stride(1) != 1 or out.device != dev:
        raise ValueError("out must be [n, T] float32 rows on src's device")
    if idx is None:
        idx = torch.arange(n, dtype=torch.int32)
    idx = idx.to(dtype=torch.int32).reshape(-1).contiguous()
    if idx.device.type == "cpu":
        if idx.numel() and (int(idx.min()) < 0 or int(idx.max()) >= n):
            raise ValueError("idx out of range")
        idx = idx.pin_memory().to(dev, non_blocking=True)
    if idx.numel():
        torch.ops.hbk.place_clips_idx_(src, src_len, pre, idx, out)
    return out


def _active_rows(values: torch.Tensor) -> torch.Tensor | None:
    if values.device.type != "cpu":
        return None
    return torch.from_numpy(np.flatnonzero(~np.isnan(values.numpy())).astype(np.int32))


def tanh_distortion(x: torch.Tensor, amount: torch.Tensor, out: torch.Tensor | None = None,
                    source: SourceView | None = None) -> torch.Tensor:
    T = ReverbPlan.T
    dev = _native.require_device(x.device)
    n = x.shape[0]
    if x.dim() != 2 or x.shape[1] < T or x.stride(1) != 1 or x.dtype != torch.float32:
        raise ValueError(f"x must be [n, >= {T}] f32 rows on the device")
    amount = amount.to(dtype=torch.float32).reshape(-1).contiguous()
    if amount.numel() != n:
        raise ValueError("amount must have n entries")
    rows = _active_rows(amount)
    amount = amount.pin_memory().to(dev, non_blocking=True) if amount.device.type == "cpu" else amount.to(dev)
    if out is None:
        out = torch.empty((n, T), dtype=torch.float32, device=dev)
    if rows is not None:
        if out.data_ptr() != x.data_ptr():
            out.copy_(x[:, :T])
            x = out
        if rows.numel() == 0:
            return out
        rows = rows.pin_memory().to(dev, non_blocking=True)
    sv = (None, None, None) if source is None else (source.check(x).src, source.lens, source.pre)
    torch.ops.hbk.tanh_distortion_(x, amount, rows, out, *sv)
    return out


PITCH_SHIFT_CHUNK = 16384
_PS_WS: dict = {}


def pitch_shift(x: torch.Tensor, idx: torch.Tensor, num: int, den: int, out: torch.Tensor | None = None,
                sample_rate: int = 16000) -> torch.Tensor:
    T = ReverbPlan.T
    dev = _native.require_device(x.device)
    if x.dim() != 2 or x.shape[1] < T or x.stride(1) != 1 or x.dtype != torch.float32:
        raise ValueError(f"x must be [n, >= {T}] f32 rows on the device")
    n = x.shape[0]
    if out is None:
        out = torch.empty((n, T), dtype=torch.float32, device=dev)
    if out.data_ptr() != x.data_ptr():
        out.copy_(x[:, :T])
        x = out
    idx = idx.to(dtype=torch.int32).reshape(-1)
    if idx.numel() == 0:
        return out
    if idx.device.type == "cpu":
        if int(idx.min()) < 0 or int(idx.max()) >= n:
            raise ValueError("idx out of range")
        idx = idx.pin_memory().to(dev, non_blocking=True)
    chunk = min(PITCH_SHIFT_CHUNK, idx.numel())
    need = int(lib().hbk_pitch_shift_workspace_size(chunk, T, sample_rate, num, den))
    if need <= 0:
        raise ValueError(f"unsupported pitch shift {num}/{den} at {sample_rate} Hz")
    key = (dev, stream_ptr(dev))
    ws = _PS_WS.get(key)
    if ws is None or ws.numel() < need:
        ws = torch.empty(need, dtype=torch.uint8, device=dev)
        _PS_WS[key] = ws
    for c0 in range(0, idx.numel(), chunk):
        torch.ops.hbk.pitch_shift_(x, idx[c0:c0 + chunk], num, den, sample_rate, out, ws)
    return out


@torch.library.custom_op("hbk::pitch_shift_", mutates_args=("out", "workspace"))
def _pitch_shift_op(x: torch.Tensor, idx: torch.Tensor, num: int, den: int, sample_rate: int, out: torch.Tensor,
                    workspace: torch.Tensor) -> None:
    check(lib().hbk_pitch_shift(ptr(x), x.stride(0), idx.numel(), ptr(idx), ReverbPlan.T, sample_rate, num, den,
                                ptr(out), out.stride(0), ptr(workspace), workspace.numel(), stream_ptr(x.device)),
          "hbk_pitch_shift")


def _view_args(src: torch.Tensor | None, src_len: torch.Tensor | None, src_pre: torch.Tensor | None) -> tuple:
    if src is None:
        return None, 0, None, None
    return ptr(src), src.stride(0), ptr(src_len), ptr(src_pre)


def seven_band_eq(x: torch.Tensor, coef: torch.Tensor, out: torch.Tensor | None = None,
                  idx: torch.Tensor | None = None, source: SourceView | None = None) -> torch.Tensor:
    T = ReverbPlan.T
    dev = _native.require_device(x.device)
    n = x.shape[0]
    if x.dim() != 2 or x.shape[1] < T or x.stride(1) != 1 or x.dtype != torch.float32:
        raise ValueError(f"x must be [n, >= {T}] f32 rows on the device")
    if x.stride(0) % 4 or x.data_ptr() % 16:
        raise ValueError("x rows must be 16-B aligned")

    def to_dev(t: torch.Tensor) -> torch.Tensor:
        return (t if t.is_pinned() else t.pin_memory()).to(dev, non_blocking=True) if t.device.type == "cpu" else t.to(dev)

    m = n if idx is None else int(idx.numel())
    coef = to_dev(coef.to(dtype=torch.float64).reshape(m, 7, 5).contiguous())
    if idx is not None:
        idx = idx.to(dtype=torch.int32).reshape(-1).contiguous()
        if idx.device.type == "cpu" and m and (int(idx.min()) < 0 or int(idx.max()) >= n):
            raise ValueError("idx out of range")
        idx = to_dev(idx)
        if out is None:
            out = x
    elif out is None:
        out = torch.empty((n, T), dtype=torch.float32, device=dev)
    if m:
        sv = (None, None, None) if source is None else (source.check(x).src, source.lens, source.pre)
        torch.ops.hbk.seven_band_eq_(x, coef, idx, out, *sv)
    return out


@torch.library.custom_op("hbk::seven_band_eq_", mutates_args=("out",))
def _seven_band_eq_op(x: torch.Tensor, coef: torch.Tensor, idx: torch.Tensor | None, out: torch.Tensor,
                      src: torch.Tensor | None = None, src_len: torch.Tensor | None = None,
                      src_pre: torch.Tensor | None = None) -> None:
    check(lib().hbk_seven_band_eq_src(ptr(x), x.shape[0], x.stride(0), ptr(coef),
                                      ptr(idx) if idx is not None else None,
                                      idx.numel() if idx is not None else x.shape[0], ptr(out), out.stride(0),
                                      *_view_args(src, src_len, src_pre), stream_ptr(x.device)),
          "hbk_seven_band_eq_src")


@torch.library.custom_op("hbk::tanh_distortion_", mutates_args=("out",))
def _tanh_distortion_op(x: torch.Tensor, amount: torch.Tensor, rows: torch.Tensor | None, out: torch.Tensor,
                        src: torch.Tensor | None = None, src_len: torch.Tensor | None = None,
                        src_pre: torch.Tensor | None = None) -> None:
    check(lib().hbk_tanh_distortion_src(ptr(x), x.shape[0], x.stride(0), ptr(amount),
                                        ptr(rows) if rows is not None else None,
                                        rows.numel() if rows is not None else 0, ptr(out), out.stride(0),
                                        *_view_args(src, src_len, src_pre), stream_ptr(x.device)),
          "hbk_tanh_distortion_src")


BAND_STOP_CIRCULAR_MAX_HALF = 512
BAND_STOP_PARTITION_TAPS = 11521


class ReverbPlan:

    T = 23040
    COLORED_GROUP_MIN = 8

    def __init__(self, device: torch.device | int | None = None) -> None:
        self.device = _native.require_device(device)
        handle = ctypes.c_void_p()
        with torch.cuda.device(self.device):
            check(lib().hbk_reverb_plan_create(self.T, ctypes.byref(handle)), "hbk_reverb_plan_create")
        self._handle = handle
        self._bs_ws: torch.Tensor | None = None
        self._cn_ws: torch.Tensor | None = None
        self.id = _register(self)

    @staticmethod
    def rotated_kernel(ir: torch.Tensor, T: int = 23040) -> torch.Tensor:
        ir = ir.reshape(-1).to(torch.float32)
        d = int(torch.argmax(ir.abs()).item())
        if ir.shape[0] > T:
            ir = ir[:T]
        z = torch.zeros(T - ir.shape[0], dtype=ir.dtype, device=ir.device)
        return torch.cat([ir[d:], z, ir[:d]])

    SLOTS = 11536

    def spectra(self, kernels: torch.Tensor) -> torch.Tensor:
        kernels = kernels.to(self.device, torch.float32).contiguous()
        n = kernels.shape[0]
        out = torch.zeros((n, self.SLOTS, 2), dtype=torch.float32, device=self.device)
        torch.ops.hbk.reverb_spectrum_(kernels, out, self.id)
        return out

    @classmethod
    def natural_spectrum(cls, spectra: torch.Tensor) -> torch.Tensor:
        n = spectra.shape[0]
        rows = spectra.reshape(n, 16, cls.SLOTS // 16, 2)
        return rows.transpose(1, 2).reshape(n, cls.SLOTS, 2)[:, :cls.T // 2 + 1]

    def augment(self, x: torch.Tensor, ring: torch.Tensor | None, noise_off: torch.Tensor,
                snr_db: torch.Tensor, spectra: torch.Tensor | None, spec_idx: torch.Tensor,
                out: torch.Tensor | None = None, gain: torch.Tensor | None = None,
                colored: tuple | None = None, source: SourceView | None = None) -> torch.Tensor:
        n = x.shape[0]
        if x.dim() != 2 or x.shape[1] < self.T or x.stride(1) != 1 or x.device != self.device:
            raise ValueError(f"x must be [n, >= {self.T}] f32 rows on {self.device}")
        if out is None:
            out = torch.empty((n, self.T), dtype=torch.float32, device=self.device)
        def per_clip(t: torch.Tensor, dtype: torch.dtype) -> torch.Tensor:
            t = t.to(dtype=dtype).reshape(-1).contiguous()
            if t.numel() != n:
                raise ValueError("per-clip arrays must have n entries")
            return t

        noise_off = per_clip(noise_off, torch.int64)
        spec_idx = per_clip(spec_idx, torch.int32)
        snr_db = per_clip(snr_db, torch.float32)
        if gain is not None:
            gain = per_clip(gain, torch.float32)
        if spectra is not None and (spectra.dim() != 3 or spectra.shape[1:] != (self.SLOTS, 2)):
            raise ValueError(f"spectra must be [n, {self.SLOTS}, 2] (ReverbPlan.spectra's slot layout)")
        ring_n = 0 if ring is None else ring.numel()
        if bool((noise_off >= 0).any()) and ring_n == 0:
            raise ValueError("noise requested without a noise ring")
        if ring_n and bool((noise_off >= ring_n).any()):
            raise ValueError("noise_off must be < the ring length")
        if spectra is not None and bool((spec_idx >= spectra.shape[0]).any()):
            raise ValueError("spec_idx out of range")

        def to_dev(t: torch.Tensor) -> torch.Tensor:
            if t.device.type == "cpu":
                return t.pin_memory().to(self.device, non_blocking=True)
            return t.to(self.device)

        noise_off, spec_idx, snr_db = to_dev(noise_off), to_dev(spec_idx), to_dev(snr_db)
        if gain is not None:
            gain = to_dev(gain)
        sv = (None, None, None) if source is None else (source.check(x).src, source.lens, source.pre)
        if colored is None:
            torch.ops.hbk.augment_(x, ring, noise_off, snr_db, spectra, spec_idx, gain, out, self.id, *sv)
            return out
        f_decay, c_snr, seed, clips_per_noise = colored
        f_decay, c_snr = per_clip(f_decay, torch.float32), per_clip(c_snr, torch.float32)
        if clips_per_noise < 1:
            raise ValueError("clips_per_noise must be >= 1")
        if out.data_ptr() != x.data_ptr():
            lo_o, hi_o = out.data_ptr(), out.data_ptr() + out.stride(0) * 4 * n
            lo_x, hi_x = x.data_ptr(), x.data_ptr() + x.stride(0) * 4 * n
            if lo_o < hi_x and lo_x < hi_o:
# ... 212 lines not shown
```

### include/hbk.h

```cpp
#ifndef HBK_H
#define HBK_H

#include <stdint.h>

#ifdef __cplusplus
extern "C" {
#endif

typedef enum {
  HBK_OK = 0,
  HBK_ERR_ARG = -1,
  HBK_ERR_HIP = -2,
  HBK_ERR_UNSUPPORTED = -3
} hbk_status;

const char* hbk_version(void);
const char* hbk_last_error(void);
int hbk_device_count(int* count);
int hbk_stream_create_cu_mask(const uint32_t* cu_mask, int n_words, void** stream);
int hbk_stream_destroy(void* stream);

int hbk_profile_mark(int32_t tag, void* stream);

typedef struct hbk_mel_plan hbk_mel_plan;
// ... 42 lines not shown
int hbk_embed_clips(const hbk_embed_plan* plan, const float* mel, int64_t n_clips,
                    int64_t mel_clip_stride, float* out, void* workspace,
                    int64_t workspace_bytes, void* stream);

int hbk_embed_split_info(const hbk_embed_plan* plan, int32_t n_front, int64_t* mid_floats_per_clip);
int hbk_embed_clips_front(const hbk_embed_plan* plan, const float* mel, int64_t n_clips,
                          int64_t mel_clip_stride, int32_t n_front, float* mid, void* workspace,
                          int64_t workspace_bytes, void* stream);
int hbk_embed_clips_back(const hbk_embed_plan* plan, const float* mid, int64_t n_clips, int32_t n_front,
                         float* out, void* workspace, int64_t workspace_bytes, void* stream);

int hbk_embed_windows(const hbk_embed_plan* plan, const float* windows, int64_t n, float* out,
                      void* workspace, int64_t workspace_bytes, void* stream);

int64_t hbk_nan_rows_workspace_size(int64_t n);
int hbk_nan_rows_fix(float* rows, int64_t n, int64_t row_len, uint64_t seed, void* workspace,
                     int64_t workspace_bytes, void* stream);

int hbk_embed_range_status(const hbk_embed_plan* plan, int32_t* tripped, int32_t reset, void* stream);

typedef struct hbk_mlp_plan hbk_mlp_plan;

int hbk_mlp_plan_create(int32_t d_in, int32_t layer_dim, int32_t hidden, int32_t n_layers,
                        hbk_mlp_plan** plan);
int hbk_mlp_plan_destroy(hbk_mlp_plan* plan);
int hbk_mlp_layout(const hbk_mlp_plan* plan, int64_t* n_params, int64_t* offsets, int32_t n_offsets);
int hbk_mlp_workspace_size(const hbk_mlp_plan* plan, int64_t batch, int64_t* bytes);

int hbk_mlp_forward(const hbk_mlp_plan* plan, const float* params, const float* x, int64_t batch,
                    float* prob, float* logit, float dropout_p, uint64_t seed, void* workspace,
                    int64_t workspace_bytes, void* stream);

int hbk_mlp_train_fwd_bwd(const hbk_mlp_plan* plan, const float* params, const float* x,
                          const float* y, int64_t batch, float neg_weight,
                          float high_loss_threshold, float activation_threshold, float dropout_p,
                          uint64_t seed, float* bucket, float* prob, void* workspace,
                          int64_t workspace_bytes, void* stream);

int hbk_mlp_gate_adam(const hbk_mlp_plan* plan, float* params, const float* bucket, float* m,
                      float* v, float* state, float* ctrl, float* history, int32_t history_cap,
                      float lr, float beta1, float beta2, float eps, void* stream);

#define HBK_STEP_XHAT_READY 1
#define HBK_STEP_PREFETCH_NEXT 2
#define HBK_STEP_WEIGHTS_READY 4
#define HBK_STEP_DEFER_PARTIALS 8
#define HBK_STEP_GATE_SKIP 16
int hbk_mlp_fused_supported(const hbk_mlp_plan* plan, int32_t* supported);
int hbk_mlp_step_variant(const hbk_mlp_plan* plan, int64_t batch, void* stream, int32_t* variant);
int hbk_mlp_step_plan_info(const hbk_mlp_plan* plan, int64_t batch, void* stream, int32_t* info, int32_t n_info);
int hbk_mlp_step_fwd_bwd(const hbk_mlp_plan* plan, const float* params, const float* pool32, int64_t n32,
                         const void* pool16, int64_t n16, const int32_t* idx, int64_t idx_step_stride,
                         const float* y, int64_t y_step_stride, int64_t batch, const float* state,
                         int32_t parity, const float* sched, int64_t sched_len, float neg_weight,
                         float high_loss_threshold, float activation_threshold, float dropout_p,
                         uint64_t seed, float* bucket, float* prob, int64_t idx_steps, int32_t flags,
                         void* workspace, int64_t workspace_bytes, void* stream);
int hbk_mlp_step_update(const hbk_mlp_plan* plan, float* params, float* bucket, float* m, float* v,
                        float* state, int32_t parity, const float* sched, int64_t sched_len, float lr,
                        float beta1, float beta2, float eps, float* history, int32_t history_cap,
                        void* workspace, int64_t workspace_bytes, void* stream);

int hbk_mlp_set_step_scalars(hbk_mlp_plan* plan, const double* dev_scalars);

int hbk_mlp_eval_workspace_size(const hbk_mlp_plan* plan, int64_t rows, int64_t* bytes);
int hbk_mlp_eval_prepare(const hbk_mlp_plan* plan, const float* params, void* workspace, int64_t workspace_bytes,
                         void* stream);
int hbk_mlp_eval_count(const hbk_mlp_plan* plan, const float* params, const void* pool, int32_t pool_is_f16,
                       int64_t n_pool, const int32_t* idx, int64_t rows, int64_t row_offset, int32_t label,
                       float activation_threshold, float dropout_p, uint64_t seed, float* counts, float* prob,
                       void* workspace, int64_t workspace_bytes, void* stream);
int hbk_mlp_eval_laps(int64_t rows, int64_t n_pool, int32_t pool_is_f16, int32_t has_idx, int64_t* parts);
int hbk_mlp_eval_count_multi(const hbk_mlp_plan* plan, const float* params, int32_t n_pools,
                             const void* const* pools, int32_t pools_are_f16, const int64_t* n_pool,
                             const int64_t* rows, const int64_t* row_offsets, const int32_t* labels,
                             const uint64_t* seeds, float* const* counts, float activation_threshold,
                             float dropout_p, void* workspace, int64_t workspace_bytes, void* stream);
int hbk_mlp_eval_finish(const float* counts_val, const float* counts_test, const double* sizes,
                        float target_false_positives_per_hour, float adjust_ratio, float* sched, int64_t sched_len,
                        int64_t next_step, float* out, void* stream);

typedef struct hbk_reverb_plan hbk_reverb_plan;

int hbk_reverb_plan_create(int64_t T, hbk_reverb_plan** plan);
int hbk_reverb_plan_destroy(hbk_reverb_plan* plan);

#define HBK_REVERB_SPECTRUM_SLOTS 11536

int hbk_reverb_spectrum(const hbk_reverb_plan* plan, const float* kernels, int64_t n_kernels,
                        int64_t stride, float* spectra, void* stream);

int hbk_augment(const hbk_reverb_plan* plan, const float* x, int64_t n_clips, int64_t x_stride,
                const float* noise_ring, int64_t ring_len, const int64_t* noise_off,
                const float* snr_db, const float* spectra, const int32_t* spec_idx,
                const float* gain, float* out, int64_t out_stride, void* stream);

int hbk_colored_noise(const hbk_reverb_plan* plan, const float* x, int64_t n_clips, int64_t x_stride,
                      const float* white, int64_t white_stride, uint64_t seed, int64_t clips_per_noise,
                      const float* f_decay, const float* snr_db, float sample_rate, const int32_t* idx,
                      int64_t n_entries, float* out, int64_t out_stride, void* stream);
int64_t hbk_colored_noise_workspace_size(int64_t n_clips, int64_t clips_per_noise);
int hbk_colored_noise_ws(const hbk_reverb_plan* plan, const float* x, int64_t n_clips, int64_t x_stride,
                         const float* white, int64_t white_stride, uint64_t seed, int64_t clips_per_noise,
                         const float* f_decay, const float* snr_db, float sample_rate, const int32_t* idx,
                         int64_t n_entries, float* out, int64_t out_stride, void* workspace, int64_t workspace_bytes,
                         void* stream);

int hbk_augment_colored(const hbk_reverb_plan* plan, const float* x, int64_t n_clips, int64_t x_stride,
                        const float* noise_ring, int64_t ring_len, const int64_t* noise_off,
                        const float* snr_db, const float* spectra, const int32_t* spec_idx,
                        const float* gain, const float* white, int64_t white_stride, uint64_t seed,
                        int64_t clips_per_noise, const float* c_f_decay, const float* c_snr_db,
                        float sample_rate, const int32_t* c_idx, int64_t c_n_entries, float* out,
                        int64_t out_stride, void* workspace, int64_t workspace_bytes, void* stream);

#define HBK_BAND_STOP_CIRCULAR_MAX_HALF 512
#define HBK_BAND_STOP_PARTITION_TAPS 11521
int64_t hbk_band_stop_workspace_size(int64_t n, int32_t n_filters, int32_t n_spectra, void* stream);
int hbk_band_stop(const hbk_reverb_plan* plan, const float* x, int64_t x_stride, int64_t n, const int32_t* idx,
                  const int32_t* filt, int32_t n_filters, const float* f_lo, const float* f_hi,
                  const int32_t* f_half, const int32_t* f_spec0, int32_t n_spectra, const int32_t* s_filt,
                  const int32_t* s_part, float* out, int64_t out_stride, void* workspace, int64_t workspace_bytes,
                  void* stream);

#define HBK_PITCH_SHIFT_MAX_TAPS 144
int64_t hbk_pitch_shift_workspace_size(int64_t n, int64_t T, int32_t sample_rate, int32_t num, int32_t den);
int hbk_pitch_shift(const float* x, int64_t x_stride, int64_t n, const int32_t* idx, int64_t T, int32_t sample_rate,
                    int32_t num, int32_t den, float* out, int64_t out_stride, void* workspace,
                    int64_t workspace_bytes, void* stream);

int hbk_seven_band_eq(const float* x, int64_t n_clips, int64_t x_stride, const double* coef, const int32_t* idx,
                      int64_t n_entries, float* out, int64_t out_stride, void* stream);

int hbk_tanh_distortion(const float* x, int64_t n_clips, int64_t x_stride, const float* amount,
                        const int32_t* idx, int64_t n_entries, float* out, int64_t out_stride, void* stream);

int hbk_place_clips(const float* src, int64_t n_clips, int64_t src_stride, const int32_t* src_len,
                    const int32_t* pre, float* out, int64_t out_stride, int64_t T, void* stream);
int hbk_place_clips_idx(const float* src, int64_t n_clips, int64_t src_stride, const int32_t* src_len,
                        const int32_t* pre, const int32_t* idx, int64_t n_entries, float* out,
                        int64_t out_stride, int64_t T, void* stream);

int hbk_seven_band_eq_src(const float* x, int64_t n_clips, int64_t x_stride, const double* coef,
                          const int32_t* idx, int64_t n_entries, float* out, int64_t out_stride,
                          const float* src, int64_t src_stride, const int32_t* src_len,
                          const int32_t* src_pre, void* stream);
int hbk_tanh_distortion_src(const float* x, int64_t n_clips, int64_t x_stride, const float* amount,
                            const int32_t* idx, int64_t n_entries, float* out, int64_t out_stride,
                            const float* src, int64_t src_stride, const int32_t* src_len,
                            const int32_t* src_pre, void* stream);
int hbk_reverb_plan_set_source(hbk_reverb_plan* plan, const float* src, int64_t src_stride,
                               const int32_t* src_len, const int32_t* src_pre);

#ifdef __cplusplus
}
#endif

#endif
```

Measured before the change: 1.145 million.

## Exploit known zero padding of placed clips in tanh, EQ and pitch span

Uses the known placement (pre offset and length) of clips inside the zero-padded window to skip work on the silent regions. The tanh distortion histogram adds the known zero count directly instead of histogramming silent samples. The EQ kernel starts filtering at the first non-silent tile and writes zeros before it, with host-side sorting of EQ entries by offset so lanes share start points. The pitch-shift span scan is restricted to the placed region. This adds validation checks and plumbing, plus an env toggle and debug arrival tracing, and it risks subtle numerical differences such as signed zeros in the IIR state.

```diff
diff --git a/hey-buddy_amd/csrc/hbk_augment_plan.h b/hey-buddy_amd/csrc/hbk_augment_plan.h
--- a/hey-buddy_amd/csrc/hbk_augment_plan.h
+++ b/hey-buddy_amd/csrc/hbk_augment_plan.h
@@ -130,6 +130,7 @@
   bool span = true;
   bool pair = true;
   bool resample_valu = false;
+  bool known_silence = true;
 };
 
 struct Grid {
diff --git a/hey-buddy_amd/csrc/hbk_clip_ops.hip b/hey-buddy_amd/csrc/hbk_clip_ops.hip
--- a/hey-buddy_amd/csrc/hbk_clip_ops.hip
+++ b/hey-buddy_amd/csrc/hbk_clip_ops.hip
@@ -1,4 +1,5 @@
 #include <algorithm>
+#include <cstdlib>
 
 #include "hbk_aug_dev.h"
 
@@ -21,6 +22,7 @@
   return s < kT ? (__builtin_bit_cast(unsigned, v) & 0x7FFFFFFFu) : 0xFFFFFFFFu;
 }
 
+template <bool kKnown>
 __global__ void __launch_bounds__(kThreads) __attribute__((amdgpu_waves_per_eu(8)))
 tanh_distortion_kernel(TanhArgs a) {
   __shared__ unsigned hist[4096];
@@ -40,6 +42,7 @@
     }
     float xr[kPer];
     const int pre = a.view.pre ? a.view.pre[clip] : -1, len = a.view.pre ? a.view.len[clip] : 0;
+    unsigned skip = 0, zeros_out = 0;
     if (pre >= 0) {
       const int n = min(len, kT);
       const float* row = n > 0 ? a.view.src + clip * a.view.stride : x;
@@ -47,6 +50,11 @@
       const int w0 = __builtin_amdgcn_readfirstlane(t & ~63);
 #pragma unroll
       for (int u = 0; u < kPer; ++u) xr[u] = load_placed_wave(row, pre, n, w0 + u * kThreads, t & 63);
+      if (kKnown && n > 0) {
+#pragma unroll
+        for (int u = 0; u < kPer; ++u) skip |= placed_class(pre, n, w0 + u * kThreads) == 0 ? 1u << u : 0u;
+        zeros_out = 64u * static_cast<unsigned>((pre >> 6) + max(kT / 64 - ((pre + n + 63) >> 6), 0));
+      }
     } else {
     const int t = opaque_tid();
 #pragma unroll
@@ -65,11 +73,12 @@
       const int shift = p == 0 ? 19 : (p == 1 ? 9 : 0), bins = p == 0 ? 4096 : (p == 1 ? 1024 : 512);
       const int per_lane = bins >> 6;
       for (int i = tid; i < bins; i += kThreads) hist[i] = 0;
+      if (kKnown && tid == 0 && prefix == 0) hist[0] = zeros_out;
       __syncthreads();
       const int t = opaque_tid();
 #pragma unroll
       for (int u = 0; u < kPer; ++u) {
-        const unsigned b = abs_bits(xr[u], t + u * kThreads);
+        const unsigned b = (kKnown && (skip >> u & 1)) ? 0xFFFFFFFFu : abs_bits(xr[u], t + u * kThreads);
         if ((b & mask) == prefix && b != 0xFFFFFFFFu) atomicAdd(&hist[(b >> shift) & (bins - 1)], 1u);
       }
       __syncthreads();
@@ -105,12 +114,12 @@
     const int t2 = opaque_tid();
 #pragma unroll
     for (int u = 0; u < kPer; ++u) {
-      const unsigned b = abs_bits(xr[u], t2 + u * kThreads);
+      const unsigned b = (kKnown && (skip >> u & 1)) ? 0xFFFFFFFFu : abs_bits(xr[u], t2 + u * kThreads);
       if (b == 0xFFFFFFFFu) continue;
       if (b <= prefix) cnt += 1.f;
       else mg = fminf(mg, __builtin_bit_cast(float, b));
     }
-    cnt = block_sum(cnt, red);
+    cnt = block_sum(cnt, red) + (kKnown ? static_cast<float>(zeros_out) : 0.f);
     {
       for (int d = 32; d >= 1; d >>= 1) mg = fminf(mg, __shfl_xor(mg, d, 64));
       __syncthreads();
@@ -190,6 +199,7 @@
   int64_t out_stride;
   int64_t n;
   SrcView view;
+  int known;
 };
 
 constexpr int kEqClips = 8;
@@ -235,9 +245,21 @@
       p1 = *reinterpret_cast<const float4*>(xl + t + 32 + 4 * lq);
     }
   };
-  load_tile(0);
+  const bool zero_out = b0 > 0.0 && __builtin_isfinite(b0) && __builtin_isfinite(b1) && __builtin_isfinite(b2) &&
+                        __builtin_isfinite(a1) && __builtin_isfinite(a2);
+  int t_start = pre_l < 0 ? 0 : (n_l > 0 ? pre_l : kT);
+  for (int d = 8; d < 64; d <<= 1) t_start = min(t_start, __shfl_xor(t_start, d, 64));
+  t_start = (a.known && __all(zero_out)) ? min(t_start & ~(kEqTile - 1), kT - kEqTile) : 0;
+  t_start = __builtin_amdgcn_readfirstlane(t_start);
+  if (t_start > 0) {
+    s2 = (__builtin_signbit(b2) && !__builtin_signbit(a2)) ? -0.0 : 0.0;
+    s1 = (__builtin_signbit(b1) && !__builtin_signbit(a1) && __builtin_signbit(s2)) ? -0.0 : 0.0;
+  }
+  if (store_l)
+    for (int t = 4 * lq; t < t_start; t += 32) *reinterpret_cast<float4*>(ol + t) = float4{0.f, 0.f, 0.f, 0.f};
+  load_tile(t_start);
   float prev = 0.f;
-  for (int t0 = 0; t0 <= kT; t0 += kEqTile) {
+  for (int t0 = t_start; t0 <= kT; t0 += kEqTile) {
     tin[lc][4 * lq] = p0.x;
     tin[lc][4 * lq + 1] = p0.y;
     tin[lc][4 * lq + 2] = p0.z;
@@ -283,6 +305,11 @@
     }
     __syncthreads();
   }
+}
+
+bool known_silence() {
+  const char* s = getenv("HBK_KNOWN_SILENCE");
+  return !(s && s[0] == '0');
 }
 
 }
@@ -337,7 +364,8 @@
   if (st != HBK_OK) return st;
   if (a.n_entries <= 0) return n_entries < 0 ? arg_error("negative n_entries") : HBK_OK;
   const int64_t blocks = std::min<int64_t>(a.n_entries, persistent_blocks(2, stream));
-  hipLaunchKernelGGL(tanh_distortion_kernel, dim3(unsigned(blocks)), dim3(kThreads), 0, as_stream(stream), a);
+  hipLaunchKernelGGL(known_silence() ? tanh_distortion_kernel<true> : tanh_distortion_kernel<false>,
+                     dim3(unsigned(blocks)), dim3(kThreads), 0, as_stream(stream), a);
   HBK_LAUNCH_CHECK("tanh_distortion_kernel");
   return HBK_OK;
 }
@@ -369,6 +397,7 @@
   a.n = n_entries;
   const int st = src_view(src, src_stride, src_len, src_pre, a.view);
   if (st != HBK_OK) return st;
+  a.known = known_silence() ? 1 : 0;
   hipLaunchKernelGGL(eq_kernel, dim3(unsigned((n_entries + kEqClips - 1) / kEqClips)), dim3(64), 0,
                      as_stream(stream), a);
   HBK_LAUNCH_CHECK("eq_kernel");
diff --git a/hey-buddy_amd/csrc/hbk_mlp_fused.hip b/hey-buddy_amd/csrc/hbk_mlp_fused.hip
--- a/hey-buddy_amd/csrc/hbk_mlp_fused.hip
+++ b/hey-buddy_amd/csrc/hbk_mlp_fused.hip
@@ -50,6 +50,18 @@
   } while (0)
 #define HBK_MTB(kern, id, blk) \
   do {                         \
+  } while (0)
+#endif
+
+#if defined(HBK_TRACE) || defined(HBK_K2_ARRIVALS)
+__device__ unsigned long long g_k2_arrive[1024][2];
+#define HBK_K2_ARRIVE(slot)                                                                        \
+  do {                                                                                             \
+    if (threadIdx.x == 0 && blockIdx.x < 1024) g_k2_arrive[blockIdx.x][slot] = __builtin_amdgcn_s_memrealtime(); \
+  } while (0)
+#else
+#define HBK_K2_ARRIVE(slot) \
+  do {                      \
   } while (0)
 #endif
 
@@ -643,6 +655,7 @@
   const int64_t B = a.B;
   const int64_t Bp = a.Bp;
   K2_MARK(1);
+  HBK_K2_ARRIVE(0);
   const int step = step_of(a.state, a.parity);
   float y_pre = 0.f, nw_pre = a.neg_weight;
   if (kTrain) {
@@ -885,6 +898,7 @@
   if constexpr (!kTrain) return;
   __syncthreads();
   K2_MARK(41);
+  HBK_K2_ARRIVE(1);
   if (tid < kStats && red[tid] != 0.f) atomicAdd(BCK(a.stats + tid, 4), red[tid]);
   if (!HBK_K2_ABLATE && red[0] == 0.f) {
     const f4 z4 = {0.f, 0.f, 0.f, 0.f};
@@ -2441,6 +2455,15 @@
   (void)hipMemcpyToSymbol(HIP_SYMBOL(hbk::g_mlp_trace_n), z, sizeof(z));
   return 0;
 }
+#endif
+#if defined(HBK_TRACE) || defined(HBK_K2_ARRIVALS)
+extern "C" int hbk_debug_k2_arrivals(unsigned long long* out) {
+  if (hipMemcpyFromSymbol(out, HIP_SYMBOL(hbk::g_k2_arrive), sizeof(hbk::g_k2_arrive)) != hipSuccess) return -2;
+  static unsigned long long z[1024][2];
+  return hipMemcpyToSymbol(HIP_SYMBOL(hbk::g_k2_arrive), z, sizeof(z)) == hipSuccess ? 0 : -2;
+}
+#endif
+#ifdef HBK_TRACE
 extern "C" int hbk_debug_spans(unsigned long long* out) {
   return hipMemcpyFromSymbol(out, HIP_SYMBOL(hbk::g_span), sizeof(hbk::g_span)) == hipSuccess ? 0 : -2;
 }
diff --git a/hey-buddy_amd/csrc/hbk_pitch.hip b/hey-buddy_amd/csrc/hbk_pitch.hip
--- a/hey-buddy_amd/csrc/hbk_pitch.hip
+++ b/hey-buddy_amd/csrc/hbk_pitch.hip
@@ -47,6 +47,9 @@
   uint64_t* key;
   int32_t* ord;
   int32_t* gord;
+  const int32_t* pl_len;
+  const int32_t* pl_pre;
+  const int32_t* pl_eq;
 };
 
 __device__ __forceinline__ int ps_i0(const PitchArgs& a, int t, float& alpha) {
@@ -213,15 +216,21 @@
 __global__ void __launch_bounds__(256) ps_span_kernel(PitchArgs a) {
   const int lane = threadIdx.x & 63, e = blockIdx.x * 4 + (threadIdx.x >> 6);
   if (e >= a.n) return;
-  const float* xr = a.x + static_cast<int64_t>(a.idx[e]) * a.x_stride;
+  const int row = a.idx[e];
+  const float* xr = a.x + static_cast<int64_t>(row) * a.x_stride;
   constexpr int kChunk = 64 * 8;
+  int begin = 0, end = a.L;
+  if (a.pl_pre) {
+    begin = min(max(a.pl_pre[row], 0), a.L);
+    if (a.pl_eq[row] < 0) end = min(begin + max(a.pl_len[row], 0), a.L);
+  }
   int lo = INT_MAX, hi = -1;
-  for (int p0 = 0; p0 < a.L; p0 += kChunk) {
+  for (int p0 = begin; p0 < end; p0 += kChunk) {
     float v[8];
 #pragma unroll
     for (int j = 0; j < 8; ++j) {
       const int p = p0 + 64 * j + lane;
-      v[j] = p < a.L ? xr[p] : 0.f;
+      v[j] = p < end ? xr[p] : 0.f;
     }
 #pragma unroll
     for (int j = 0; j < 8; ++j)
@@ -236,13 +245,13 @@
     hi = max(hi, __shfl_xor(hi, o, 64));
   }
   if (hi >= 0) {
-    for (int p1 = a.L; p1 > hi + 1; p1 -= kChunk) {
+    for (int p1 = end; p1 > hi + 1; p1 -= kChunk) {
       float v[8];
       int h = -1;
 #pragma unroll
       for (int j = 0; j < 8; ++j) {
         const int p = p1 - kChunk + 64 * j + lane;
-        v[j] = (p > hi && p < a.L) ? xr[max(p, 0)] : 0.f;
+        v[j] = (p > hi && p < end) ? xr[max(p, 0)] : 0.f;
       }
 #pragma unroll
       for (int j = 0; j < 8; ++j)
@@ -837,6 +846,8 @@
   s = getenv("HBK_PS_PAIR");
   k.pair = !(s && s[0] == '0');
   k.resample_valu = getenv("HBK_PS_RESAMPLE_VALU") != nullptr;
+  s = getenv("HBK_KNOWN_SILENCE");
+  k.known_silence = !(s && s[0] == '0');
   return k;
 }
 
@@ -883,11 +894,21 @@
 int hbk_pitch_shift(const float* x, int64_t x_stride, int64_t n, const int32_t* idx, int64_t T, int32_t sample_rate,
                     int32_t num, int32_t den, float* out, int64_t out_stride, void* workspace,
                     int64_t workspace_bytes, void* stream) {
+  return hbk_pitch_shift_placed(x, x_stride, n, idx, T, sample_rate, num, den, out, out_stride, workspace,
+                                workspace_bytes, nullptr, nullptr, nullptr, stream);
+}
+
+int hbk_pitch_shift_placed(const float* x, int64_t x_stride, int64_t n, const int32_t* idx, int64_t T,
+                           int32_t sample_rate, int32_t num, int32_t den, float* out, int64_t out_stride,
+                           void* workspace, int64_t workspace_bytes, const int32_t* src_len, const int32_t* src_pre,
+                           const int32_t* eq_pre, void* stream) {
   using namespace hbk;
   if (n < 0) return arg_error("negative n");
   if (n == 0) return HBK_OK;
   if (n > 65535) return arg_error("n > 65535 per call");
   if (!x || !idx || !out || !workspace) return arg_error("NULL pointer");
+  if ((src_len || src_pre || eq_pre) && !(src_len && src_pre && eq_pre))
+    return arg_error("the placement needs src_len, src_pre and eq_pre");
   PitchGeometry g;
   std::string err;
   const int rc = pitch_geometry(T, sample_rate, num, den, g, err);
@@ -915,6 +936,7 @@
   a.taps = reinterpret_cast<float*>(w + off.taps);
   a.yr = reinterpret_cast<int2*>(w + off.yr);
   a.span = knobs.span ? 1 : 0;
+  if (knobs.known_silence) a.pl_len = src_len, a.pl_pre = src_pre, a.pl_eq = eq_pre;
   if (L.pair) {
     a.sp = reinterpret_cast<int2*>(w + off.sp);
     a.key = reinterpret_cast<uint64_t*>(w + off.key);
diff --git a/hey-buddy_amd/heybuddy/_native.py b/hey-buddy_amd/heybuddy/_native.py
--- a/hey-buddy_amd/heybuddy/_native.py
+++ b/hey-buddy_amd/heybuddy/_native.py
@@ -85,6 +85,8 @@
                                                   ctypes.c_int32]),
     "hbk_pitch_shift": (_c_int, [_vp, _c_int64, _c_int64, _vp, _c_int64, ctypes.c_int32, ctypes.c_int32,
                                  ctypes.c_int32, _vp, _c_int64, _vp, _c_int64, _vp]),
+    "hbk_pitch_shift_placed": (_c_int, [_vp, _c_int64, _c_int64, _vp, _c_int64, ctypes.c_int32, ctypes.c_int32,
+                                        ctypes.c_int32, _vp, _c_int64, _vp, _c_int64, _vp, _vp, _vp, _vp]),
     "hbk_seven_band_eq": (_c_int, [_vp, _c_int64, _c_int64, _vp, _vp, _c_int64, _vp, _c_int64, _vp]),
     "hbk_place_clips": (_c_int, [_vp, _c_int64, _c_int64, _vp, _vp, _vp, _c_int64, _c_int64, _vp]),
     "hbk_place_clips_idx": (_c_int, [_vp, _c_int64, _c_int64, _vp, _vp, _vp, _c_int64, _vp, _c_int64, _c_int64,
diff --git a/hey-buddy_amd/heybuddy/dataset/augmented.py b/hey-buddy_amd/heybuddy/dataset/augmented.py
--- a/hey-buddy_amd/heybuddy/dataset/augmented.py
+++ b/hey-buddy_amd/heybuddy/dataset/augmented.py
@@ -128,6 +128,14 @@
 
 def first_touch_enabled() -> bool:
     return os.environ.get("HBK_PLACE_FIRST_TOUCH", "1") != "0"
+
+
+def known_silence_enabled() -> bool:
+    return os.environ.get("HBK_KNOWN_SILENCE", "1") != "0"
+
+
+def eq_entry_order(eq_idx: np.ndarray, pre: np.ndarray) -> np.ndarray:
+    return np.argsort(np.asarray(pre)[np.asarray(eq_idx)], kind="stable")
 
 
 def first_touch_routes(eq_on: np.ndarray, tanh_on: np.ndarray, placed_first: np.ndarray) -> np.ndarray:
@@ -296,7 +304,8 @@
             self._tanh = np.where(t_on, t_amt, np.nan).astype(np.float32)
         return noise_off, spec_idx, gain_db
 
-    def prepare(self, n: int, coins: Optional[np.ndarray] = None) -> Dict[str, Any]:
+    def prepare(self, n: int, coins: Optional[np.ndarray] = None, pre: Optional[np.ndarray] = None
+                ) -> Dict[str, Any]:
         noise_off, spec_idx, gain_db = self.plan_batches(n, coins)
         ring_len = 0 if self.ring is None else self.ring.numel()
         if ring_len:
@@ -309,7 +318,12 @@
             gain = torch.pow(10.0, torch.from_numpy(gain_db) / 20.0)
         eq_idx, eq_coef = self._eq
         eq = None
-        if eq_idx.size:
+        if eq_idx.size and pre is not None and known_silence_enabled():
+            order = eq_entry_order(eq_idx, pre)
+            coef = torch.empty(eq_coef.shape, dtype=torch.float64, pin_memory=torch.cuda.is_available())
+            np.take(eq_coef, order, axis=0, out=coef.numpy())
+            eq = (coef, _pinned(torch.from_numpy(eq_idx[order])))
+        elif eq_idx.size:
             eq = (_pinned(torch.from_numpy(eq_coef)), _pinned(torch.from_numpy(eq_idx)))
         tanh = None if np.isnan(self._tanh).all() else torch.from_numpy(self._tanh)
         bs_idx, bs_lo, bs_hi = self._bandstop
@@ -352,8 +366,8 @@
         return first_touch_routes(eq_on, tanh_on, placed_first)
 
     def __call__(self, x: torch.Tensor, out: Optional[torch.Tensor] = None,
-                 prepared: Optional[Dict[str, Any]] = None, source: Optional[Dict[int, SourceView]] = None
-                 ) -> torch.Tensor:
+                 prepared: Optional[Dict[str, Any]] = None, source: Optional[Dict[int, SourceView]] = None,
+                 placement: Optional[tuple] = None) -> torch.Tensor:
         n = x.shape[0]
         pr = self.prepare(n) if prepared is None else prepared
         if pr["n"] != n:
@@ -376,7 +390,7 @@
         for num, den, clips in pr.get("pitch") or []:
             if out is None:
                 out = torch.empty((n, T), dtype=torch.float32, device=x.device)
-            x = pitch_shift(x, clips, num, den, out=out, sample_rate=self.sample_rate)
+            x = pitch_shift(x, clips, num, den, out=out, sample_rate=self.sample_rate, placement=placement)
             ev = self._tick("pitch", ev)
         if pr.get("bandstop") is not None:
             if out is None:
@@ -591,7 +605,7 @@
         n = clips.shape[0]
         lens = np.full(n, clips.shape[1], dtype=np.int32) if lengths is None else np.asarray(lengths, np.int32)
         pre, coins = self.plan_batches(lens)
-        return {"lens": lens, "pre": pre, "chain": self.augmenter.prepare(n, coins)}
+        return {"lens": lens, "pre": pre, "chain": self.augmenter.prepare(n, coins, pre=pre)}
 
     def augment_device(self, clips: torch.Tensor, lengths: Optional[Sequence[int]] = None,
                        prepared: Optional[Dict[str, Any]] = None) -> torch.Tensor:
@@ -613,7 +627,15 @@
         self.placed_rows = np.flatnonzero(route == ROUTE_PLACE).astype(np.int32)
         placed = place_clips(clips, dev[0], dev[1], T, idx=torch.from_numpy(self.placed_rows))
         source = {r: SourceView(clips, dev[0], dev[2 + i]) for i, r in enumerate(routes)}
-        return self.augmenter(placed, out=placed, prepared=pr["chain"], source=source)
+        chain = pr["chain"]
+        eq_rows = chain["eq"][1].numpy() if chain.get("eq") is not None else np.zeros(0, np.int32)
+        if not (route[eq_rows] == ROUTE_EQ).all() or int((route == ROUTE_EQ).sum()) != np.unique(eq_rows).size:
+            raise ValueError("prepared['route'] does not match prepared['eq'] (BatchAugmenter.routes)")
+        shifted = [c.numpy() for _, _, c in chain.get("pitch") or []]
+        if shifted and np.unique(np.concatenate(shifted)).size != sum(c.size for c in shifted):
+            raise ValueError("a clip is listed in more than one pitch shift")
+        return self.augmenter(placed, out=placed, prepared=pr["chain"], source=source,
+                              placement=(dev[0], dev[1], dev[2]))
 
     def __call__(self, num_samples: int, **kwargs: Any) -> Iterator[Dict[str, Any]]:
         total_batches = int(np.ceil(num_samples / self.batch_size))
diff --git a/hey-buddy_amd/heybuddy/dataset/features.py b/hey-buddy_amd/heybuddy/dataset/features.py
--- a/hey-buddy_amd/heybuddy/dataset/features.py
+++ b/hey-buddy_amd/heybuddy/dataset/features.py
@@ -307,7 +307,7 @@
         lens = np.asarray(lengths)[rows].astype(np.int32)
         same = num_samples == n_tts and np.array_equal(rows, np.arange(n_tts))
         src = clips if same else clips.index_select(0, torch.from_numpy(rows).to(clips.device))
-        prepared = {"lens": lens, "pre": pre, "chain": aug.augmenter.prepare(num_samples, coins)}
+        prepared = {"lens": lens, "pre": pre, "chain": aug.augmenter.prepare(num_samples, coins, pre=pre)}
         return aug.augment_device(src, lens, prepared=prepared)
 
     def generate_device(self, num_samples: int, testing: bool = False, validation: bool = False) -> torch.Tensor:
diff --git a/hey-buddy_amd/heybuddy/kernels.py b/hey-buddy_amd/heybuddy/kernels.py
--- a/hey-buddy_amd/heybuddy/kernels.py
+++ b/hey-buddy_amd/heybuddy/kernels.py
@@ -789,7 +789,7 @@
 
 
 def pitch_shift(x: torch.Tensor, idx: torch.Tensor, num: int, den: int, out: torch.Tensor | None = None,
-                sample_rate: int = 16000) -> torch.Tensor:
+                sample_rate: int = 16000, placement: tuple | None = None) -> torch.Tensor:
     T = ReverbPlan.T
     dev = _native.require_device(x.device)
     if x.dim() != 2 or x.shape[1] < T or x.stride(1) != 1 or x.dtype != torch.float32:
@@ -816,17 +816,23 @@
     if ws is None or ws.numel() < need:
         ws = torch.empty(need, dtype=torch.uint8, device=dev)
         _PS_WS[key] = ws
+    if placement is not None:
+        for t in placement:
+            if t.dtype != torch.int32 or t.shape != (n,) or t.device != dev or not t.is_contiguous():
+                raise ValueError("placement must be three [n] int32 tensors on x's device")
     for c0 in range(0, idx.numel(), chunk):
-        torch.ops.hbk.pitch_shift_(x, idx[c0:c0 + chunk], num, den, sample_rate, out, ws)
+        torch.ops.hbk.pitch_shift_(x, idx[c0:c0 + chunk], num, den, sample_rate, out, ws, *(placement or ()))
     return out
 
 
 @torch.library.custom_op("hbk::pitch_shift_", mutates_args=("out", "workspace"))
 def _pitch_shift_op(x: torch.Tensor, idx: torch.Tensor, num: int, den: int, sample_rate: int, out: torch.Tensor,
-                    workspace: torch.Tensor) -> None:
-    check(lib().hbk_pitch_shift(ptr(x), x.stride(0), idx.numel(), ptr(idx), ReverbPlan.T, sample_rate, num, den,
-                                ptr(out), out.stride(0), ptr(workspace), workspace.numel(), stream_ptr(x.device)),
-          "hbk_pitch_shift")
+                    workspace: torch.Tensor, src_len: torch.Tensor | None = None,
+                    src_pre: torch.Tensor | None = None, eq_pre: torch.Tensor | None = None) -> None:
+    pl = (None, None, None) if src_len is None else (ptr(src_len), ptr(src_pre), ptr(eq_pre))
+    check(lib().hbk_pitch_shift_placed(ptr(x), x.stride(0), idx.numel(), ptr(idx), ReverbPlan.T, sample_rate, num,
+                                       den, ptr(out), out.stride(0), ptr(workspace), workspace.numel(), *pl,
+                                       stream_ptr(x.device)), "hbk_pitch_shift_placed")
 
 
 def _view_args(src: torch.Tensor | None, src_len: torch.Tensor | None, src_pre: torch.Tensor | None) -> tuple:
diff --git a/include/hbk.h b/include/hbk.h
--- a/include/hbk.h
+++ b/include/hbk.h
@@ -218,6 +218,11 @@
 int hbk_reverb_plan_set_source(hbk_reverb_plan* plan, const float* src, int64_t src_stride,
                                const int32_t* src_len, const int32_t* src_pre);
 
+int hbk_pitch_shift_placed(const float* x, int64_t x_stride, int64_t n, const int32_t* idx, int64_t T,
+                           int32_t sample_rate, int32_t num, int32_t den, float* out, int64_t out_stride,
+                           void* workspace, int64_t workspace_bytes, const int32_t* src_len,
+                           const int32_t* src_pre, const int32_t* eq_pre, void* stream);
+
 #ifdef __cplusplus
 }
 #endif
```

New measurement: 1.158 million (median of 6 runs). +1.2%, better.
